# Lumina-Group/libzkp

Measured on AMD Instinct MI355X. Metric: proofs/sec (whole node) + ms/proof p50, 4096-proof mixed batch (range / equality / membership / improvement) per MI355X, higher is better.
Workload: dtype u32/u64 integer limbs (10x25.5-bit GF(2^255-19), BN254 Fq on 9x29-bit limbs in the MSM loops and 10x26-bit elsewhere, 8x32-bit Fr and scalars mod l, 2x64-bit f128)

## Files before the change

libzkp_amd/csrc/bn254_g.h:

```cpp
#pragma once
#include "bn254_fq.h"
#include "bn254_fq9.h"

namespace zkp {

struct fq2 { fq c0, c1; };

ZKP_HD inline fq f_add(const fq& a, const fq& b) { return fq_add(a, b); }
ZKP_HD inline fq f_sub(const fq& a, const fq& b) { return fq_sub(a, b); }
ZKP_HD inline fq f_mul(const fq& a, const fq& b) { return fq_mul(a, b); }
ZKP_HD inline fq f_sq(const fq& a) { return fq_sq(a); }
ZKP_HD inline fq f_neg(const fq& a) { return fq_neg(a); }
ZKP_HD inline fq f_dbl(const fq& a) { return fq_dbl(a); }
ZKP_HD inline bool f_is_zero(const fq& a) { return fq_is_zero(a); }
ZKP_HD inline fq f_select(bool c, const fq& a, const fq& b) { return fq_select(c, a, b); }
ZKP_HD inline void f_set_zero(fq& a) { a = fq_zero(); }
ZKP_HD inline void f_set_one(fq& a) { a = fq_one(); }
ZKP_HD inline fq f_inv(const fq& a) { return fq_inv(a); }

ZKP_HD inline fq2 f_add(const fq2& a, const fq2& b) { return fq2{fq_add(a.c0, b.c0), fq_add(a.c1, b.c1)}; }
ZKP_HD inline fq2 f_sub(const fq2& a, const fq2& b) { return fq2{fq_sub(a.c0, b.c0), fq_sub(a.c1, b.c1)}; }
ZKP_HD inline fq2 f_neg(const fq2& a) { return fq2{fq_neg(a.c0), fq_neg(a.c1)}; }
ZKP_HD inline fq2 f_dbl(const fq2& a) { return fq2{fq_dbl(a.c0), fq_dbl(a.c1)}; }
ZKP_HD inline fq2 f_mul(const fq2& a, const fq2& b) {
    const fq t0 = fq_mul(a.c0, b.c0), t1 = fq_mul(a.c1, b.c1);
    const fq t2 = fq_mul(fq_add_l(a.c0, a.c1), fq_add_l(b.c0, b.c1));
    return fq2{fq_reduce_weak(fq_sub_k4(t0, t1)), fq_reduce_weak(fq_sub_k8(t2, fq_add_l(t0, t1)))};
}
ZKP_HD inline fq2 f_sq(const fq2& a) {
    const fq t = fq_mul(a.c0, a.c1);
    return fq2{fq_reduce_weak(fq_mul(fq_add_l(a.c0, a.c1), fq_sub_k4(a.c0, a.c1))), fq_reduce_weak(fq_dbl_l(t))};
}
ZKP_HD inline bool f_is_zero(const fq2& a) { return fq_is_zero(a.c0) && fq_is_zero(a.c1); }
ZKP_HD inline fq2 f_select(bool c, const fq2& a, const fq2& b) { return fq2{fq_select(c, a.c0, b.c0), fq_select(c, a.c1, b.c1)}; }
ZKP_HD inline void f_set_zero(fq2& a) { a.c0 = fq_zero(); a.c1 = fq_zero(); }
ZKP_HD inline void f_set_one(fq2& a) { a.c0 = fq_one(); a.c1 = fq_zero(); }
ZKP_HD inline fq2 f_inv(const fq2& a) {
    const fq d = fq_inv(fq_add(fq_sq(a.c0), fq_sq(a.c1)));
    return fq2{fq_reduce_weak(fq_mul(a.c0, d)), fq_neg(fq_reduce_weak(fq_mul(a.c1, d)))};
}

template <class F> struct Aff { F x, y; };
template <class F> struct Jac { F X, Y, Z; };
using g1_aff = Aff<fq>; using g1_jac = Jac<fq>;
using g2_aff = Aff<fq2>; using g2_jac = Jac<fq2>;

template <class F> ZKP_HD inline Jac<F> jac_infinity() { Jac<F> r; f_set_one(r.X); f_set_one(r.Y); f_set_zero(r.Z); return r; }
template <class F> ZKP_HD inline Jac<F> jac_from_aff(const Aff<F>& p) { Jac<F> r; r.X = p.x; r.Y = p.y; f_set_one(r.Z); return r; }
template <class F> ZKP_HD inline bool jac_is_inf(const Jac<F>& p) { return f_is_zero(p.Z); }

template <class F> ZKP_HD inline Jac<F> jac_dbl(const Jac<F>& p) {
    const F A = f_sq(p.X), B = f_sq(p.Y), C = f_sq(B);
    const F D = f_dbl(f_sub(f_sub(f_sq(f_add(p.X, B)), A), C));
    const F E = f_add(f_dbl(A), A), Fq_ = f_sq(E);
    Jac<F> r;
    r.X = f_sub(Fq_, f_dbl(D));
    r.Y = f_sub(f_mul(E, f_sub(D, r.X)), f_dbl(f_dbl(f_dbl(C))));
    r.Z = f_dbl(f_mul(p.Y, p.Z));
    return r;
}

template <class F> ZKP_HD inline Jac<F> jac_madd(const Jac<F>& p, const Aff<F>& q) {
    if (jac_is_inf(p)) return jac_from_aff(q);
    const F Z1Z1 = f_sq(p.Z);
    const F U2 = f_mul(q.x, Z1Z1), S2 = f_mul(f_mul(q.y, p.Z), Z1Z1);
    const F H = f_sub(U2, p.X), rr = f_dbl(f_sub(S2, p.Y));
    if (f_is_zero(H)) return f_is_zero(rr) ? jac_dbl(p) : jac_infinity<F>();
    const F HH = f_sq(H), I = f_dbl(f_dbl(HH)), J = f_mul(H, I), V = f_mul(p.X, I);
    Jac<F> r;
    r.X = f_sub(f_sub(f_sq(rr), J), f_dbl(V));
    r.Y = f_sub(f_mul(rr, f_sub(V, r.X)), f_dbl(f_mul(p.Y, J)));
    r.Z = f_sub(f_sub(f_sq(f_add(p.Z, H)), Z1Z1), HH);
    return r;
}


ZKP_HD inline Jac<fq> g1_madd_lazy(const Jac<fq>& p, const Aff<fq>& q) {
    const fq Z1Z1 = fq_sq(p.Z);
    const fq U2 = fq_mul(q.x, Z1Z1), S2 = fq_mul(fq_mul(q.y, p.Z), Z1Z1);
    const fq H = fq_sub_k4(U2, p.X), sv = fq_sub_k4(S2, p.Y);
    const fq HH = fq_sq(H);
    const fq I = fq_dbl_l(fq_dbl_l(HH));
    const fq J = fq_mul(H, I), V = fq_mul(p.X, I);
    const fq ss = fq_sq(sv);
    Jac<fq> r;
    r.X = fq_reduce_weak(fq_sub_k8(fq_sub_k4(fq_dbl_l(fq_dbl_l(ss)), J), fq_dbl_l(V)));
    const fq t = fq_sub_k4(fq_mul(sv, fq_sub_k4(V, r.X)), fq_mul(p.Y, J));
    r.Y = fq_reduce_weak(fq_dbl_l(t));
    r.Z = fq_reduce_weak(fq_sub_k4(fq_sub_k4(fq_sq(fq_add_l(p.Z, H)), Z1Z1), HH));
    return r;
}

struct g1_xyzz { fq X, Y, ZZ, ZZZ; };
ZKP_HD inline g1_xyzz g1_mmadd_lazy(const g1_xyzz& p, const Aff<fq>& q) {
    const fq U2 = fq_mul(q.x, p.ZZ), S2 = fq_mul(q.y, p.ZZZ);
    const fq P = fq_sub_k4(U2, p.X), Rv = fq_sub_k4(S2, p.Y);
    const fq PP = fq_sq(P);
    const fq PPP = fq_mul(P, PP), Q = fq_mul(p.X, PP);
    const fq RR = fq_sq(Rv);
    g1_xyzz r;
    r.X = fq_reduce_weak(fq_sub_k8(fq_sub_k4(RR, PPP), fq_dbl_l(Q)));
    r.Y = fq_mul_add2(Rv, fq_sub_k4(Q, r.X), fq_sub_k4(fq_zero(), p.Y), PPP);
    r.ZZ = fq_mul(p.ZZ, PP);
    r.ZZZ = fq_mul(p.ZZZ, PPP);
    return r;
}
struct g1_xyzz9 { fq9 X, Y, ZZ, ZZZ; };
struct g1_aff9 { fq9 x, y; };
ZKP_HD inline g1_xyzz9 g1_mmadd9(const g1_xyzz9& p, const g1_aff9& q) {
    const fq9 U2 = fq9_mul(q.x, p.ZZ), S2 = fq9_mul(q.y, p.ZZZ);
    const fq9 P = fq9_sub_k<8>(U2, p.X), Rv = fq9_sub_k<4>(S2, p.Y);
    const fq9 PP = fq9_sq(P);
    const fq9 PPP = fq9_mul(P, PP), Q = fq9_mul(p.X, PP);
    const fq9 RR = fq9_sq(Rv);
    g1_xyzz9 r;
    r.X = fq9_sub2_k4(RR, PPP, Q);
    r.Y = fq9_mul_add2(Rv, fq9_sub_loose<8>(Q, r.X), fq9_neg_loose<4>(p.Y), PPP);
    r.ZZ = fq9_mul(p.ZZ, PP);
    r.ZZZ = fq9_mul(p.ZZZ, PPP);
    return r;
}
ZKP_HD inline g1_xyzz9 xyzz9_from_jac(const Jac<fq>& p) {
    const fq zz = fq_sq(p.Z);
    return g1_xyzz9{fq9_from_fq(p.X), fq9_from_fq(p.Y), fq9_from_fq(zz), fq9_from_fq(fq_mul(zz, p.Z))};
}
ZKP_HD inline Jac<fq> jac_from_xyzz9(const g1_xyzz9& p) { return Jac<fq>{fq9_to_fq(fq9_mul(p.X, p.ZZ)), fq9_to_fq(fq9_mul(p.Y, p.ZZZ)), fq9_to_fq(p.ZZ)}; }
ZKP_HD inline g1_xyzz xyzz_from_jac(const Jac<fq>& p) { const fq zz = fq_sq(p.Z); return g1_xyzz{p.X, p.Y, zz, fq_mul(zz, p.Z)}; }
ZKP_HD inline Jac<fq> jac_from_xyzz(const g1_xyzz& p) { return Jac<fq>{fq_reduce_weak(fq_mul(p.X, p.ZZ)), fq_reduce_weak(fq_mul(p.Y, p.ZZZ)), fq_reduce_weak(p.ZZ)}; }

struct fq2k { fq t0, t1, t2; };
struct fq2s { fq c0, m; };
ZKP_HD inline fq2k fq2_kara(const fq2& a, const fq2& b) { return fq2k{fq_mul(a.c0, b.c0), fq_mul(a.c1, b.c1), fq_mul(fq_add_l(a.c0, a.c1), fq_add_l(b.c0, b.c1))}; }
ZKP_HD inline fq2 fq2_join(const fq2k& k) { return fq2{fq_sub_k4(k.t0, k.t1), fq_sub_k8(k.t2, fq_add_l(k.t0, k.t1))}; }
ZKP_HD inline fq2s fq2_sq_l(const fq2& a) { return fq2s{fq_mul(fq_add_l(a.c0, a.c1), fq_sub_k4(a.c0, a.c1)), fq_mul(a.c0, a.c1)}; }
ZKP_HD inline Jac<fq2> g2_madd_lazy(const Jac<fq2>& p, const Aff<fq2>& q, bool negate) {
    const fq zero = fq_zero();
    const fq2 y2{fq_select(negate, fq_sub_k4(zero, q.y.c0), q.y.c0), fq_select(negate, fq_sub_k4(zero, q.y.c1), q.y.c1)};
    const fq2s zz = fq2_sq_l(p.Z);
    const fq2 Z1Z1{zz.c0, fq_dbl_l(zz.m)};
    const fq2 U2 = fq2_join(fq2_kara(q.x, Z1Z1));
    const fq2 S2 = fq2_join(fq2_kara(fq2_join(fq2_kara(y2, p.Z)), Z1Z1));
    const fq2 H{fq_reduce_weak(fq_sub_k4(U2.c0, p.X.c0)), fq_reduce_weak(fq_sub_k4(U2.c1, p.X.c1))};
    const fq2 sv{fq_reduce_weak(fq_sub_k4(S2.c0, p.Y.c0)), fq_reduce_weak(fq_sub_k4(S2.c1, p.Y.c1))};
    const fq2s hh = fq2_sq_l(H);
    const fq2 I{fq_dbl_l(fq_dbl_l(hh.c0)), fq_dbl_l(fq_dbl_l(fq_dbl_l(hh.m)))};
    const fq2k J = fq2_kara(H, I), V = fq2_kara(p.X, I);
    const fq2s ss = fq2_sq_l(sv);
    Jac<fq2> r;
    r.X.c0 = fq_reduce_weak(fq_sub_k16(fq_add_l(fq_dbl_l(fq_dbl_l(ss.c0)), fq_add_l(J.t1, fq_dbl_l(V.t1))), fq_add_l(J.t0, fq_dbl_l(V.t0))));
    r.X.c1 = fq_reduce_weak(fq_sub_k16(fq_add_l(fq_dbl_l(fq_dbl_l(fq_dbl_l(ss.m))), fq_add_l(fq_add_l(J.t0, J.t1), fq_dbl_l(fq_add_l(V.t0, V.t1)))),
                                       fq_add_l(J.t2, fq_dbl_l(V.t2))));
    const fq2 W{fq_sub_k8(V.t0, fq_add_l(V.t1, r.X.c0)), fq_sub_k16(V.t2, fq_add_l(fq_add_l(V.t0, V.t1), r.X.c1))};
    const fq2k P1 = fq2_kara(sv, W), P2 = fq2_kara(p.Y, fq2_join(J));
    r.Y.c0 = fq_reduce_weak(fq_dbl_l(fq_sub_k8(fq_add_l(P1.t0, P2.t1), fq_add_l(P1.t1, P2.t0))));
    r.Y.c1 = fq_reduce_weak(fq_dbl_l(fq_sub_k16(fq_add_l(P1.t2, fq_add_l(P2.t0, P2.t1)), fq_add_l(fq_add_l(P1.t0, P1.t1), P2.t2))));
    const fq2 zh{fq_add_l(p.Z.c0, H.c0), fq_add_l(p.Z.c1, H.c1)};
    const fq zq0 = fq_mul(fq_add_l(zh.c0, zh.c1), fq_sub_k8(zh.c0, zh.c1)), zqm = fq_mul(zh.c0, zh.c1);
    r.Z.c0 = fq_reduce_weak(fq_sub_k8(zq0, fq_add_l(zz.c0, hh.c0)));
    r.Z.c1 = fq_reduce_weak(fq_dbl_l(fq_sub_k8(zqm, fq_add_l(zz.m, hh.m))));
    return r;
}

struct fq2_9 { fq9 c0, c1; };
struct g2_xyzz9 { fq2_9 X, Y, ZZ, ZZZ; };
struct g2_aff9 { fq2_9 x, y; };
ZKP_HD inline fq2_9 fq2_9_mul(const fq2_9& a, const fq2_9& b, const fq9& nb1) {
    return fq2_9{fq9_mul_add2(a.c0, b.c0, a.c1, nb1), fq9_mul_add2(a.c0, b.c1, a.c1, b.c0)};
}
ZKP_HD inline fq2_9 fq2_9_sq(const fq2_9& a, const fq9& na1) { return fq2_9{fq9_mul_add2(a.c0, a.c0, a.c1, na1), fq9_mul(fq9_dbl_l(a.c0), a.c1)}; }
ZKP_HD inline g2_xyzz9 g2_mmadd9(const g2_xyzz9& p, const g2_aff9& q, bool negate) {
    const fq9 nZZ1 = fq9_neg_k<4>(p.ZZ.c1), nZZZ1 = fq9_neg_k<4>(p.ZZZ.c1);
    const fq2_9 U2 = fq2_9_mul(q.x, p.ZZ, nZZ1), S2 = fq2_9_mul(q.y, p.ZZZ, nZZZ1);
    const fq2_9 P{fq9_sub_k<16>(U2.c0, p.X.c0), fq9_sub_k<16>(U2.c1, p.X.c1)};
    const fq2_9 Rv{fq9_sgn_sub_k<8>(negate, S2.c0, p.Y.c0), fq9_sgn_sub_k<8>(negate, S2.c1, p.Y.c1)};
    const fq2_9 PP = fq2_9_sq(P, fq9_neg_k<32>(P.c1));
    const fq9 nPP1 = fq9_neg_k<8>(PP.c1);
    const fq2_9 PPP = fq2_9_mul(P, PP, nPP1), Q = fq2_9_mul(p.X, PP, nPP1);
    const fq9 nR1 = fq9_neg_k<16>(Rv.c1);
    const fq2_9 RR = fq2_9_sq(Rv, nR1);
    g2_xyzz9 r;
    r.X = fq2_9{fq9_sub2_k<8>(RR.c0, PPP.c0, Q.c0), fq9_sub2_k<8>(RR.c1, PPP.c1, Q.c1)};
    const fq2_9 W{fq9_sub_k<16>(Q.c0, r.X.c0), fq9_sub_k<16>(Q.c1, r.X.c1)};
    const fq9 nY0 = fq9_neg_k<4>(p.Y.c0), nY1 = fq9_neg_k<4>(p.Y.c1);
    r.Y = fq2_9{fq9_mul_add4(Rv.c0, W.c0, nR1, W.c1, nY0, PPP.c0, p.Y.c1, PPP.c1),
                fq9_mul_add4(Rv.c0, W.c1, Rv.c1, W.c0, nY0, PPP.c1, nY1, PPP.c0)};
    r.ZZ = fq2_9_mul(PP, p.ZZ, nZZ1);
    r.ZZZ = fq2_9_mul(PPP, p.ZZZ, nZZZ1);
    return r;
}
ZKP_HD inline fq2_9 fq2_9_from_fq2(const fq2& a) { return fq2_9{fq9_from_fq(a.c0), fq9_from_fq(a.c1)}; }
ZKP_HD inline fq2 fq2_9_to_fq2(const fq2_9& a) { return fq2{fq9_to_fq(a.c0), fq9_to_fq(a.c1)}; }
ZKP_HD inline g2_xyzz9 g2_xyzz9_from_jac(const Jac<fq2>& p) {
    const fq2 zz = f_sq(p.Z);
    return g2_xyzz9{fq2_9_from_fq2(p.X), fq2_9_from_fq2(p.Y), fq2_9_from_fq2(zz), fq2_9_from_fq2(f_mul(zz, p.Z))};
}
ZKP_HD inline Jac<fq2> jac_from_g2_xyzz9(const g2_xyzz9& p) {
    return Jac<fq2>{fq2_9_to_fq2(fq2_9_mul(p.X, p.ZZ, fq9_neg_k<4>(p.ZZ.c1))), fq2_9_to_fq2(fq2_9_mul(p.Y, p.ZZZ, fq9_neg_k<4>(p.ZZZ.c1))), fq2_9_to_fq2(p.ZZ)};
}

template <class F> ZKP_HD inline Jac<F> jac_add(const Jac<F>& p, const Jac<F>& q) {
    if (jac_is_inf(p)) return q;
    if (jac_is_inf(q)) return p;
    const F Z1Z1 = f_sq(p.Z), Z2Z2 = f_sq(q.Z);
    const F U1 = f_mul(p.X, Z2Z2), U2 = f_mul(q.X, Z1Z1);
    const F S1 = f_mul(f_mul(p.Y, q.Z), Z2Z2), S2 = f_mul(f_mul(q.Y, p.Z), Z1Z1);
    const F H = f_sub(U2, U1), rr = f_dbl(f_sub(S2, S1));
    if (f_is_zero(H)) return f_is_zero(rr) ? jac_dbl(p) : jac_infinity<F>();
    const F I = f_sq(f_dbl(H)), J = f_mul(H, I), V = f_mul(U1, I);
    Jac<F> r;
    r.X = f_sub(f_sub(f_sq(rr), J), f_dbl(V));
    r.Y = f_sub(f_mul(rr, f_sub(V, r.X)), f_dbl(f_mul(S1, J)));
    r.Z = f_mul(f_sub(f_sub(f_sq(f_add(p.Z, q.Z)), Z1Z1), Z2Z2), H);
    return r;
}
template <class F> ZKP_HD inline Aff<F> aff_neg(const Aff<F>& p) { return Aff<F>{p.x, f_neg(p.y)}; }
template <class F> ZKP_HD inline Jac<F> jac_neg(const Jac<F>& p) { return Jac<F>{p.X, f_neg(p.Y), p.Z}; }

template <class F> ZKP_HD inline Jac<F> jac_mul_raw(const Jac<F>& p, const uint32_t k[8]) {
    Jac<F> tbl[16];
    tbl[0] = jac_infinity<F>(); tbl[1] = p;
    for (int i = 2; i < 16; i++) tbl[i] = jac_add(tbl[i - 1], p);
    Jac<F> acc = jac_infinity<F>();
    for (int nib = 63; nib >= 0; nib--) {
        acc = jac_dbl(jac_dbl(jac_dbl(jac_dbl(acc))));
        const uint32_t d = (k[nib >> 3] >> ((nib & 7) * 4)) & 15u;
        if (d) acc = jac_add(acc, tbl[d]);
    }
    return acc;
}

template <int NA, int NB, int NO> ZKP_HD inline void mp_mul_lo(uint32_t* out, const uint32_t* a, const uint32_t* b) {
    uint64_t acc = 0, hi = 0;
    ZKP_UNROLL for (int k = 0; k < NO; k++) {
        ZKP_UNROLL for (int i = 0; i < NA; i++) {
            const int j = k - i;
            if (j < 0 || j >= NB) continue;
            const uint64_t t = (uint64_t)a[i] * b[j];
            acc += (uint32_t)t; hi += t >> 32;
        }
        out[k] = (uint32_t)acc;
        acc = (acc >> 32) + (uint32_t)hi; hi >>= 32;
    }
}
struct glv_half { uint32_t mag[4]; bool neg; };
ZKP_HD inline glv_half glv_from_160(const uint32_t w[5]) {
    glv_half h; h.neg = (w[4] >> 31) != 0;
    uint32_t c = h.neg ? 1u : 0u;
    ZKP_UNROLL for (int i = 0; i < 4; i++) { const uint32_t x = h.neg ? ~w[i] : w[i]; const uint32_t t = x + c; c = (c && t == 0) ? 1u : 0u; h.mag[i] = t; }
    return h;
}
ZKP_HD inline void fr_glv_split(const uint32_t k[8], glv_half& h1, glv_half& h2) {
    const uint32_t G1[3] = {0xc7e0b3d7u, 0xd91d232eu, 0x00000002u}, G2[5] = {0x391eb18du, 0x7a7bd9d4u, 0xa773d2cfu, 0x4ccef014u, 0x00000002u};
    const uint32_t A1[2] = {0x94d213e3u, 0x89d32568u}, A2[4] = {0x1221250bu, 0x0be4e154u, 0xeeb859fdu, 0x6f4d8248u};
    const uint32_t NB1[4] = {0x7d4f1128u, 0x8211bbebu, 0xeeb859fcu, 0x6f4d8248u}, B2[2] = {0x94d213e3u, 0x89d32568u};
    uint32_t t1[11], t2[13];
    mp_mul_lo<8, 3, 11>(t1, k, G1); mp_mul_lo<8, 5, 13>(t2, k, G2);
    const uint32_t* c1 = t1 + 8;
    const uint32_t* c2 = t2 + 8;
    uint32_t p11[5], p22[5], p12[5], p21[5];
    mp_mul_lo<3, 2, 5>(p11, c1, A1); mp_mul_lo<5, 4, 5>(p22, c2, A2); mp_mul_lo<3, 4, 5>(p12, c1, NB1); mp_mul_lo<5, 2, 5>(p21, c2, B2);
    uint32_t k1[5], k2[5]; int64_t b1 = 0, b2 = 0;
    ZKP_UNROLL for (int i = 0; i < 5; i++) {
        b1 += (int64_t)k[i] - (int64_t)p11[i] - (int64_t)p22[i]; k1[i] = (uint32_t)b1; b1 >>= 32;
        b2 += (int64_t)p12[i] - (int64_t)p21[i]; k2[i] = (uint32_t)b2; b2 >>= 32;
    }
    h1 = glv_from_160(k1); h2 = glv_from_160(k2);
}
ZKP_HD inline fq fq_glv_beta() {
    const uint32_t w[8] = {0x77fffffeu, 0x57634731u, 0xacdb5c4fu, 0xd4f263f1u, 0xa0d48bacu, 0x59e26bceu, 0x00000000u, 0x00000000u};
    return fq_from_raw(w);
}
template <class F> ZKP_HD inline Jac<F> jac_mul_u128_signed(const Jac<F>& p, const uint32_t mag[4], bool neg) {
    Jac<F> tbl[8];
    tbl[0] = p; tbl[1] = jac_dbl(p);
    for (int i = 2; i < 8; i++) tbl[i] = jac_add(tbl[i - 1], p);
    int dig[33]; int carry = 0;
    for (int i = 0; i < 32; i++) {
        int v = (int)((mag[i >> 3] >> ((i & 7) * 4)) & 15u) + carry;
        carry = v > 8 ? 1 : 0; if (carry) v -= 16;
        dig[i] = v;
    }
    dig[32] = carry;
    Jac<F> acc = jac_infinity<F>();
    for (int i = 32; i >= 0; i--) {
        if (i != 32) acc = jac_dbl(jac_dbl(jac_dbl(jac_dbl(acc))));
        const int d = dig[i];
        if (d > 0) acc = jac_add(acc, tbl[d - 1]);
        else if (d < 0) acc = jac_add(acc, jac_neg(tbl[-d - 1]));
    }
    return neg ? jac_neg(acc) : acc;
}

template <class F> ZKP_HD inline bool jac_to_aff(Aff<F>& out, const Jac<F>& p) {
    if (jac_is_inf(p)) return false;
    const F zi = f_inv(p.Z), zi2 = f_sq(zi);
    out.x = f_mul(p.X, zi2); out.y = f_mul(f_mul(p.Y, zi2), zi);
    return true;
}

ZKP_HD inline bool fq_raw_gt_half(const uint32_t w[8]) {
    const uint32_t half[8] = {0x6c3e7ea3u, 0x9e10460bu, 0xb438e546u, 0xcbc0b548u, 0x40c0ac2eu, 0xdc2822dbu, 0x7098d014u, 0x18322739u};
    for (int i = 7; i >= 0; i--) { if (w[i] > half[i]) return true; if (w[i] < half[i]) return false; }
    return false;
}
ZKP_HD inline void g1_serialize(uint32_t out[16], const g1_jac& p) {
    g1_aff a;
    if (!jac_to_aff(a, p)) { for (int i = 0; i < 16; i++) out[i] = 0; out[15] = 0x40000000u; return; }
    fq_to_raw(out, a.x); fq_to_raw(out + 8, a.y);
    if (fq_raw_gt_half(out + 8)) out[15] |= 0x80000000u;
}
ZKP_HD inline void g2_serialize(uint32_t out[32], const g2_jac& p) {
    g2_aff a;
    if (!jac_to_aff(a, p)) { for (int i = 0; i < 32; i++) out[i] = 0; out[31] = 0x40000000u; return; }
    fq_to_raw(out, a.x.c0); fq_to_raw(out + 8, a.x.c1); fq_to_raw(out + 16, a.y.c0); fq_to_raw(out + 24, a.y.c1);
    uint32_t nz = 0; for (int i = 0; i < 8; i++) nz |= out[24 + i];
    const bool larger = nz ? fq_raw_gt_half(out + 24) : fq_raw_gt_half(out + 16);
    if (larger) out[31] |= 0x80000000u;
}

}
```

libzkp_amd/csrc/bp_layout.h:

```cpp
#pragma once
#include <vector>
#include <utility>
#include <cstring>
#include "bp_steps.h"

namespace zkp {

inline void host_sponge(uint8_t* out, size_t outlen, const uint8_t* in, size_t inlen, size_t rate, uint8_t suffix) {
    uint64_t a[25]; memset(a, 0, sizeof a);
    uint8_t* b = reinterpret_cast<uint8_t*>(a);
    size_t pos = 0;
    for (size_t i = 0; i < inlen; i++) { b[pos++] ^= in[i]; if (pos == rate) { keccak_f1600(a); pos = 0; } }
    b[pos] ^= suffix; b[rate - 1] ^= 0x80;
    keccak_f1600(a);
    size_t done = 0;
    while (done < outlen) {
        size_t n = outlen - done < rate ? outlen - done : rate;
        memcpy(out + done, b, n); done += n;
        if (done < outlen) keccak_f1600(a);
    }
}

inline ge host_from_uniform(const uint8_t b[64]) { uint32_t w[16]; memcpy(w, b, 64); return ge_from_uniform_words(w); }

inline ge host_basepoint() {
    const uint32_t yw[8] = {0x66666658u, 0x66666666u, 0x66666666u, 0x66666666u, 0x66666666u, 0x66666666u, 0x66666666u, 0x66666666u};
    const uint32_t xw[8] = {0x8f25d51au, 0xc9562d60u, 0x9525a7b2u, 0x692cc760u, 0xfdd6dc5cu, 0xc0a4e231u, 0xcd6e53feu, 0x216936d3u};
    ge p; p.X = fe_fromwords(xw); p.Y = fe_fromwords(yw); p.Z = fe_one(); p.T = fe_mul(p.X, p.Y);
    return p;
}

inline void host_generators(ge out[NBASE]) {
    out[BASE_B] = host_basepoint();
    uint32_t enc[8]; ge_ristretto_encode(enc, out[BASE_B]);
    uint8_t h[64]; host_sponge(h, 64, reinterpret_cast<uint8_t*>(enc), 32, 72, 0x06);
    out[BASE_BB] = host_from_uniform(h);
    for (int which = 0; which < 2; which++) {
        uint8_t in[20]; memcpy(in, "GeneratorsChain", 15);
        in[15] = which ? 'H' : 'G'; in[16] = in[17] = in[18] = in[19] = 0;
        std::vector<uint8_t> stream(64 * BP_N);
        host_sponge(stream.data(), stream.size(), in, 20, 136, 0x1F);
        for (uint32_t i = 0; i < BP_N; i++) out[(which ? BASE_H : BASE_G) + i] = host_from_uniform(stream.data() + 64 * i);
    }
}

inline fe host_fe_invert(const fe& z) {
    fe t = fe_pow22523(z);
    t = fe_sq(fe_sq(fe_sq(t)));
    return fe_mul(t, fe_mul(fe_sq(z), z));
}

inline void host_build_table_for_base(uint32_t* dst, const ge& base) {
    std::vector<ge> pts(NWIN * NENT);
    ge pw = base;
    for (uint32_t w = 0; w < NWIN; w++) {
        ge acc = pw;
        for (uint32_t e = 0; e < NENT; e++) { pts[w * NENT + e] = acc; acc = ge_add(acc, pw); }
        for (uint32_t k = 0; k < WBITS; k++) pw = ge_dbl(pw);
    }
    const size_t n = pts.size();
    std::vector<fe> pre(n);
    fe run = fe_one();
    for (size_t i = 0; i < n; i++) { pre[i] = run; run = fe_mul(run, pts[i].Z); }
    fe inv = host_fe_invert(run);
    const fe d2 = fe_const_d2();
    for (size_t i = n; i-- > 0;) {
        const fe zi = fe_mul(inv, pre[i]);
        inv = fe_mul(inv, pts[i].Z);
        const fe x = fe_mul(pts[i].X, zi), y = fe_mul(pts[i].Y, zi);
        uint32_t w8[8];
        fe_towords(w8, fe_add(y, x)); const fe ypx = fe_fromwords(w8);
        fe_towords(w8, fe_sub(y, x)); const fe ymx = fe_fromwords(w8);
        fe_towords(w8, fe_mul(fe_mul(x, y), d2)); const fe xy2d = fe_fromwords(w8);
        uint32_t* q = dst + i * NIELS_W;
        for (int k = 0; k < 10; k++) { q[k] = ypx.v[k]; q[10 + k] = ymx.v[k]; q[20 + k] = xy2d.v[k]; }
    }
}

struct MsmLayout {
    std::vector<uint16_t> slot_base, chunk_begin, chunk_win0, chunk_nwin, target_chunk_begin;
    std::vector<uint8_t> slot_nwin;
    uint32_t nslots() const { return (uint32_t)slot_base.size(); }
    uint32_t nchunks() const { return (uint32_t)chunk_begin.size(); }
    uint32_t ntargets() const { return (uint32_t)target_chunk_begin.size() - 1; }
};
using SlotList = std::vector<std::pair<uint16_t, uint8_t>>;

inline MsmLayout make_layout(const std::vector<SlotList>& targets, uint32_t win_budget) {
    MsmLayout L;
    L.target_chunk_begin.push_back(0);
    for (const auto& t : targets) {
        uint32_t used = 0; bool open = false;
        for (const auto& s : t) {
            if (open && used + s.second > win_budget) { L.chunk_nwin.push_back((uint16_t)used); used = 0; open = false; }
            if (!open) { L.chunk_begin.push_back((uint16_t)L.slot_base.size()); L.chunk_win0.push_back(0); open = true; }
            L.slot_base.push_back(s.first); L.slot_nwin.push_back(s.second); used += s.second;
        }
        if (open) L.chunk_nwin.push_back((uint16_t)used);
        L.target_chunk_begin.push_back((uint16_t)L.chunk_begin.size());
    }
    return L;
}
inline MsmLayout make_layout_even(const std::vector<SlotList>& targets, uint32_t total_chunks) {
    MsmLayout L;
    uint64_t W = 0; for (const auto& t : targets) for (const auto& s : t) W += s.second;
    L.target_chunk_begin.push_back(0);
    for (const auto& t : targets) {
        uint32_t wt = 0; for (const auto& s : t) wt += s.second;
        uint32_t k = (uint32_t)((uint64_t)total_chunks * wt / (W ? W : 1));
        if (k < 1) k = 1;
        if (k > wt && wt) k = wt;
        const uint32_t slot0 = (uint32_t)L.slot_base.size();
        for (const auto& s : t) { L.slot_base.push_back(s.first); L.slot_nwin.push_back(s.second); }
        uint32_t slot = slot0, win = 0, done = 0;
        for (uint32_t c = 0; c < k; c++) {
            const uint32_t upto = (uint32_t)((uint64_t)wt * (c + 1) / k), n = upto - done;
            if (n == 0) continue;
            L.chunk_begin.push_back((uint16_t)slot); L.chunk_win0.push_back((uint16_t)win); L.chunk_nwin.push_back((uint16_t)n);
            uint32_t left = n;
            while (left) { const uint32_t room = L.slot_nwin[slot] - win, step = left < room ? left : room; win += step; left -= step; if (win == L.slot_nwin[slot]) { slot++; win = 0; } }
            done = upto;
        }
        L.target_chunk_begin.push_back((uint16_t)L.chunk_begin.size());
    }
    return L;
}
struct GatherShape { uint32_t nent, slot_ent, uneven, digw; };
inline bool make_gather_steps(const MsmLayout& L, const uint16_t* slot_scalar, const GatherShape& g, std::vector<uint32_t>& steps, std::vector<uint32_t>& chunk_step0) {
    steps.clear(); chunk_step0.clear();
    for (uint32_t c = 0; c < L.nchunks(); c++) {
        chunk_step0.push_back((uint32_t)(steps.size() / 2));
        uint32_t s = L.chunk_begin[c], w = L.chunk_win0[c];
        for (uint32_t left = L.chunk_nwin[c]; left > 0; left--) {
            const uint64_t first = (uint64_t)L.slot_base[s] * g.slot_ent + (uint64_t)(w + (g.uneven && w == 17u ? 1u : 0u)) * g.nent;
            const uint64_t word = (uint64_t)(slot_scalar ? slot_scalar[s] : s) * g.digw + w / 2;
            if (first + g.nent > 0xffffffffull || word > 0x7fffffffull) return false;
            steps.push_back((uint32_t)first); steps.push_back((uint32_t)(word << 1) | (w & 1u));
            if (++w == L.slot_nwin[s]) { s++; w = 0; }
        }
    }
    chunk_step0.push_back((uint32_t)(steps.size() / 2));
    for (int pad = 0; pad < 8; pad++) { steps.push_back(0); steps.push_back(0); }
    return true;
}

inline std::vector<SlotList> targets_phase1(uint32_t n = BP_N, uint8_t nw = NWIN, uint8_t nw64 = NWIN_U64) {
    const uint8_t NWIN = nw, NWIN_U64 = nw64;
    SlotList v = {{BASE_B, NWIN_U64}, {BASE_BB, NWIN}}, a = {{BASE_BB, NWIN}}, s = {{BASE_BB, NWIN}};
    for (uint32_t i = 0; i < n; i++) a.push_back({(uint16_t)(BASE_G + i), 1});
    for (uint32_t i = 0; i < n; i++) a.push_back({(uint16_t)(BASE_H + i), 1});
    for (uint32_t i = 0; i < n; i++) s.push_back({(uint16_t)(BASE_G + i), NWIN});
    for (uint32_t i = 0; i < n; i++) s.push_back({(uint16_t)(BASE_H + i), NWIN});
    return {v, a, s};
}
inline std::vector<SlotList> targets_phase2(uint8_t nw = NWIN) { SlotList t = {{BASE_B, nw}, {BASE_BB, nw}}; return {t, t}; }
inline std::vector<SlotList> targets_round(uint32_t r, uint32_t n = BP_N, uint8_t nw = NWIN) {
    const uint8_t NWIN = nw;
    uint32_t lg = 0; while ((1u << lg) < n) lg++;
    const uint32_t p = lg - 1 - r, k = 1u << p, half = n / 2;
    auto idx = [&](uint32_t rank, uint32_t bit) { return ((rank >> p) << (p + 1)) | (bit << p) | (rank & (k - 1)); };
    SlotList l = {{BASE_B, NWIN}}, rr = {{BASE_B, NWIN}};
    for (uint32_t q = 0; q < half; q++) l.push_back({(uint16_t)(BASE_G + idx(q, 1)), NWIN});
    for (uint32_t q = 0; q < half; q++) l.push_back({(uint16_t)(BASE_H + idx(q, 0)), NWIN});
    for (uint32_t q = 0; q < half; q++) rr.push_back({(uint16_t)(BASE_G + idx(q, 0)), NWIN});
    for (uint32_t q = 0; q < half; q++) rr.push_back({(uint16_t)(BASE_H + idx(q, 1)), NWIN});
    return {l, rr};
}
inline std::vector<SlotList> targets_ctask(uint8_t nw = NWIN, uint8_t nw64 = NWIN_U64) { return {SlotList{{BASE_B, nw64}, {BASE_BB, nw}}}; }
inline std::vector<SlotList> targets_verify(uint8_t nw = NWIN) {
    const uint8_t NWIN = nw;
    SlotList t = {{BASE_B, NWIN}, {BASE_BB, NWIN}};
    for (uint32_t i = 0; i < BP_N; i++) t.push_back({(uint16_t)(BASE_G + i), NWIN});
    for (uint32_t i = 0; i < BP_N; i++) t.push_back({(uint16_t)(BASE_H + i), NWIN});
    return {t};
}
inline MsmLayout layout_phase1(uint32_t budget, uint32_t n = BP_N) { return make_layout(targets_phase1(n), budget); }
inline MsmLayout layout_phase2(uint32_t budget) { return make_layout(targets_phase2(), budget); }
inline MsmLayout layout_round(uint32_t r, uint32_t budget, uint32_t n = BP_N) { return make_layout(targets_round(r, n), budget); }
inline MsmLayout layout_ctask(uint32_t budget) { return make_layout(targets_ctask(), budget); }

}
```

libzkp_amd/csrc/bp_steps.h:

```cpp
#pragma once
#include "fe25519.h"
#include "sc25519.h"
#include "ge25519.h"
#include "keccak.h"

namespace zkp {

constexpr uint32_t BP_N = 64;
constexpr uint32_t BASE_B = 0, BASE_BB = 1, BASE_G = 2, BASE_H = 66, NBASE = 130;
constexpr uint32_t WBITS = 10, NWIN = 26, NENT = 512, DIGW = 13, NWIN_U64 = 7, NIELS_W = 30, SUBTAB_W = NENT * NIELS_W;
constexpr uint32_t TAPE_SLOTS = 132;
constexpr uint32_t P1_V = 0, P1_A = 2, P1_NSLOTS = 260;
constexpr uint32_t P2_NSLOTS = 4;
constexpr uint32_t PR_NSLOTS = 130;
ZKP_HD constexpr uint32_t p1_s(uint32_t n) { return 3 + 2 * n; }
ZKP_HD constexpr uint32_t tape_slots(uint32_t n) { return 2 * n + 4; }
ZKP_HD constexpr uint32_t rp_bytes(uint32_t lg) { return 32 * (9 + 2 * lg); }
constexpr uint32_t GE_W = 40;
enum { SC_Y = 0, SC_Z, SC_X, SC_W, SC_U, SC_UINV, SC_T0, SC_T1, SC_T2, SC_NUM };
enum { KIND_RANGE_MIN = 0, KIND_RANGE_MAX, KIND_THRESHOLD, KIND_CONSISTENCY, KIND_BULLETPROOF, KIND_NUM };

struct BpView {
    uint32_t M;
    uint32_t n, lg;
    uint32_t wbits = 0;
    const uint64_t* v;
    const uint32_t* seed_ix;
    const uint32_t* proof_ix;
    const int32_t* bl_plus;
    const int32_t* bl_minus;
    const uint8_t* kind;
    const uint32_t* seeds;
    const uint64_t* proof_off;
    const uint64_t* commit_off;
    uint8_t* out;
    uint32_t* tape;
    uint32_t* gamma;
    uint32_t* d1;
    uint32_t* d2;
    uint32_t* dr;
    uint32_t* yinvpow;
    uint32_t* ypq;
    uint32_t* r0;
    uint32_t* r1;
    uint32_t* pp;
    uint32_t* ab;
    uint32_t* gh;
    uint32_t* scal;
    uint32_t* tstate;
    uint32_t* enc;
};

ZKP_HD inline sc ld_sc(const uint32_t* p, uint32_t idx, uint32_t row, uint32_t rows) {
    sc r; const uint32_t* q = p + (size_t)idx * 8 * rows + row;
    ZKP_UNROLL for (int k = 0; k < 8; k++) r.v[k] = q[(size_t)k * rows];
    return r;
}
ZKP_HD inline void st_sc(uint32_t* p, uint32_t idx, uint32_t row, uint32_t rows, const sc& s) {
    uint32_t* q = p + (size_t)idx * 8 * rows + row;
    ZKP_UNROLL for (int k = 0; k < 8; k++) q[(size_t)k * rows] = s.v[k];
}
ZKP_HD inline void st_digits_raw(uint32_t* d, uint32_t slot, uint32_t row, uint32_t rows, const sc& raw, uint32_t wbits = 0) {
    uint32_t* q = d + (size_t)slot * DIGW * rows + row;
    if (wbits == 16) {
        uint32_t pk[8]; sc_recode_signed65536(pk, raw);
        ZKP_UNROLL for (uint32_t k = 0; k < 8; k++) q[(size_t)k * rows] = pk[k];
        return;
    }
    if (wbits > 10) { sc_recode_signed_rt(q, rows, raw, wbits, sc_signed_ndigits(wbits, 254)); return; }
    uint32_t pk[DIGW]; sc_recode_signed1024(pk, raw);
    ZKP_UNROLL for (uint32_t k = 0; k < DIGW; k++) q[(size_t)k * rows] = pk[k];
}
ZKP_HD inline void st_digits(uint32_t* d, uint32_t slot, uint32_t row, uint32_t rows, const sc& mont, uint32_t wbits = 0) { st_digits_raw(d, slot, row, rows, sc_to_raw(mont), wbits); }
ZKP_HD inline int32_t ld_digit(const uint32_t* d, uint32_t srow, uint32_t w, uint32_t row, uint32_t rows) {
    return (int32_t)(int16_t)(d[((size_t)srow * DIGW + (w >> 1)) * rows + row] >> (16 * (w & 1u)));
}
ZKP_HD inline void put_bytes(uint8_t* dst, const uint32_t* w, int nwords) {
    for (int i = 0; i < nwords; i++) { dst[4 * i] = (uint8_t)w[i]; dst[4 * i + 1] = (uint8_t)(w[i] >> 8); dst[4 * i + 2] = (uint8_t)(w[i] >> 16); dst[4 * i + 3] = (uint8_t)(w[i] >> 24); }
}
ZKP_HD inline void ld_seed(uint32_t s[8], const BpView& V, uint32_t job) {
    const uint32_t* p = V.seeds + (size_t)V.seed_ix[job] * 8;
    ZKP_UNROLL for (int k = 0; k < 8; k++) s[k] = p[k];
}
ZKP_HD inline sc tape_blinding(const uint32_t seed[8], uint32_t i) {
    uint32_t w[16]; tape_draw64(w, seed, 0xFFFFFFFFu, i);
    sc raw; ZKP_UNROLL for (int k = 0; k < 8; k++) raw.v[k] = w[k];
    return sc_from_raw256(raw);
}

ZKP_HD inline void step_tape(const BpView& V, uint32_t slot, uint32_t job) {
    const uint32_t M = V.M, n = V.n, P1_S = p1_s(V.n);
    uint32_t seed[8]; ld_seed(seed, V, job);
    if (slot < tape_slots(n)) {
        uint32_t w[16]; tape_draw64(w, seed, V.proof_ix[job], slot);
        const sc x = sc_from_wide(w);
        st_sc(V.tape, slot, job, M, x);
        if (slot == 0) st_digits(V.d1, P1_A + 0, job, M, x, V.wbits);
        else if (slot == 1) st_digits(V.d1, P1_S + 0, job, M, x, V.wbits);
        else if (slot < 2 + n) st_digits(V.d1, P1_S + 1 + (slot - 2), job, M, x, V.wbits);
        else if (slot < 2 + 2 * n) st_digits(V.d1, P1_S + 1 + n + (slot - 2 - n), job, M, x, V.wbits);
        else if (slot == 2 + 2 * n) st_digits(V.d2, 1, job, M, x, V.wbits);
        else st_digits(V.d2, 3, job, M, x, V.wbits);
    } else {
        sc g = sc_zero();
        if (V.bl_plus[job] >= 0) g = tape_blinding(seed, (uint32_t)V.bl_plus[job]);
        if (V.bl_minus[job] >= 0) g = sc_sub(g, tape_blinding(seed, (uint32_t)V.bl_minus[job]));
        st_sc(V.gamma, 0, job, M, g);
        st_digits(V.d1, P1_V + 1, job, M, g, V.wbits);
        const uint64_t v = V.v[job];
        st_digits_raw(V.d1, P1_V + 0, job, M, sc_words((uint32_t)v, (uint32_t)(v >> 32), 0, 0, 0, 0, 0, 0), V.wbits);
        for (uint32_t i = 0; i < n; i++) {
            const uint32_t bit = (uint32_t)(v >> i) & 1u;
            V.d1[(size_t)(P1_A + 1 + i) * DIGW * M + job] = bit;
            V.d1[(size_t)(P1_A + 1 + n + i) * DIGW * M + job] = bit ? 0u : 0xFFFFu;
        }
    }
}

ZKP_HD inline ge_niels ld_niels(const uint32_t* p) {
    ge_niels n;
    ZKP_UNROLL for (int k = 0; k < 10; k++) { n.ypx.v[k] = p[k]; n.ymx.v[k] = p[10 + k]; n.xy2d.v[k] = p[20 + k]; }
    return n;
}
ZKP_HD inline ge msm_accumulate_digit(const ge& acc, int32_t d, const uint32_t* subtab) {
    const uint32_t mag = (uint32_t)(d < 0 ? -d : d);
    ge_niels n = ld_niels(subtab + (size_t)(mag - 1) * NIELS_W);
    n = ge_niels_select(d < 0, ge_niels_neg(n), n);
    return ge_madd(acc, n);
}
ZKP_HD inline void st_ge(uint32_t* p, uint32_t idx, uint32_t row, uint32_t rows, const ge& g) {
    uint32_t* q = p + (size_t)idx * GE_W * rows + row;
    ZKP_UNROLL for (int k = 0; k < 10; k++) {
        q[(size_t)k * rows] = g.X.v[k]; q[(size_t)(10 + k) * rows] = g.Y.v[k];
        q[(size_t)(20 + k) * rows] = g.Z.v[k]; q[(size_t)(30 + k) * rows] = g.T.v[k];
    }
}
ZKP_HD inline ge ld_ge(const uint32_t* p, uint32_t idx, uint32_t row, uint32_t rows) {
    ge g; const uint32_t* q = p + (size_t)idx * GE_W * rows + row;
    ZKP_UNROLL for (int k = 0; k < 10; k++) {
        g.X.v[k] = q[(size_t)k * rows]; g.Y.v[k] = q[(size_t)(10 + k) * rows];
        g.Z.v[k] = q[(size_t)(20 + k) * rows]; g.T.v[k] = q[(size_t)(30 + k) * rows];
    }
    return g;
}
struct MsmView {
    uint32_t rows, nslots, nchunks;
    const uint32_t* table;
    const uint32_t* digits;
    const uint16_t* slot_base;
    const uint16_t* slot_scalar;
    const uint8_t* slot_nwin;
    const uint16_t* chunk_begin;
    const uint16_t* chunk_win0;
    const uint16_t* chunk_nwin;
    uint32_t* partial;
    const uint32_t* acc_init;
    uint32_t nwin = 0, nent = 0, digw = 0;
    uint32_t slot_ent = 0, uneven = 0;
    const uint32_t* steps = nullptr; const uint32_t* chunk_step0 = nullptr;
};
ZKP_HD inline void msm_chunk_ref(const MsmView& m, uint32_t chunk, uint32_t row) {
    ge acc = ge_identity();
    uint32_t s = m.chunk_begin[chunk], w = m.chunk_win0[chunk];
    for (uint32_t left = m.chunk_nwin[chunk]; left > 0; left--) {
        const uint32_t srow = m.slot_scalar ? m.slot_scalar[s] : s;
        const int32_t d = ld_digit(m.digits, srow, w, row, m.rows);
        if (d != 0) acc = msm_accumulate_digit(acc, d, m.table + ((size_t)m.slot_base[s] * NWIN + w) * SUBTAB_W);
        if (++w == m.slot_nwin[s]) { s++; w = 0; }
    }
    st_ge(m.partial, chunk, row, m.rows, acc);
}
struct ReduceView {
    uint32_t rows, ntargets;
    const uint32_t* partial;
    const uint16_t* target_chunk_begin;
    uint32_t* enc;
    const uint64_t* out_off;
    uint8_t* out;
    const uint32_t* corr;
    const uint16_t* target_chunk_end = nullptr;
};
ZKP_HD inline uint32_t reduce_chunk_end(const ReduceView& r, uint32_t target) { return r.target_chunk_end ? r.target_chunk_end[target] : r.target_chunk_begin[target + 1]; }
ZKP_HD inline void reduce_encode_thread(const ReduceView& r, uint32_t target, uint32_t row) {
    const uint32_t c0 = r.target_chunk_begin[target], c1 = reduce_chunk_end(r, target);
    ge acc = ld_ge(r.partial, c0, row, r.rows);
    for (uint32_t c = c0 + 1; c < c1; c++) acc = ge_add(acc, ld_ge(r.partial, c, row, r.rows));
    sc e; ge_ristretto_encode(e.v, acc);
    st_sc(r.enc, target, row, r.rows, e);
    if (r.out_off != nullptr && target == 0) put_bytes(r.out + r.out_off[row], e.v, 8);
}

ZKP_HD inline void strobe_save(const BpView& V, uint32_t job, const Strobe& s) {
    for (int i = 0; i < 50; i++) V.tstate[(size_t)i * V.M + job] = s.base[i * s.stride];
    V.tstate[(size_t)50 * V.M + job] = s.pos; V.tstate[(size_t)51 * V.M + job] = s.pos_begin;
}
ZKP_HD inline void strobe_load(const BpView& V, uint32_t job, Strobe& s) {
    for (int i = 0; i < 50; i++) s.base[i * s.stride] = V.tstate[(size_t)i * V.M + job];
    s.pos = V.tstate[(size_t)50 * V.M + job]; s.pos_begin = V.tstate[(size_t)51 * V.M + job];
}
ZKP_HD inline sc merlin_challenge_scalar(Strobe& s, const char* label, uint32_t label_len) {
    uint32_t w[16]; merlin_challenge_words(s, label, label_len, w, 16);
    return sc_from_wide(w);
}
ZKP_HD inline void merlin_append_scalar(Strobe& s, const char* label, uint32_t label_len, const sc& raw) { merlin_append_words(s, label, label_len, raw.v, 8); }

ZKP_HD inline void step_transcript1(const BpView& V, uint32_t job, Strobe& s) {
    const uint32_t M = V.M;
    switch (V.kind[job]) {
        case KIND_RANGE_MIN: merlin_init(s, "libzkp_range_min", 16); break;
        case KIND_RANGE_MAX: merlin_init(s, "libzkp_range_max", 16); break;
        case KIND_THRESHOLD: merlin_init(s, "libzkp_threshold", 16); break;
        case KIND_CONSISTENCY: merlin_init(s, "libzkp_consistency", 18); break;
        default: merlin_init(s, "libzkp_bulletproof", 18); break;
    }
    merlin_append_bytes(s, "dom-sep", 7, "rangeproof v1", 13);
    merlin_append_u64(s, "n", 1, V.n);
    merlin_append_u64(s, "m", 1, 1);
    const sc Ve = ld_sc(V.enc, 0, job, M), Ae = ld_sc(V.enc, 1, job, M), Se = ld_sc(V.enc, 2, job, M);
    merlin_append_words(s, "V", 1, Ve.v, 8);
    merlin_append_words(s, "A", 1, Ae.v, 8);
    merlin_append_words(s, "S", 1, Se.v, 8);
    const sc y = merlin_challenge_scalar(s, "y", 1);
    const sc z = merlin_challenge_scalar(s, "z", 1);
    strobe_save(V, job, s);
    st_sc(V.scal, SC_Y, job, M, y);
    st_sc(V.scal, SC_Z, job, M, z);
    const sc yinv = sc_invert(y);
    for (uint32_t h = 0; h < 2; h++) {
        const sc base = h ? yinv : y;
        sc p = sc_one();
        for (uint32_t b = 0; b < 8; b++) { st_sc(V.ypq, 16 * h + b, job, M, p); p = sc_mul(p, base); }
        sc q = sc_one();
        for (uint32_t a = 0; a < 8; a++) { st_sc(V.ypq, 16 * h + 8 + a, job, M, q); q = sc_mul(q, p); }
    }
    uint8_t* pr = V.out + V.proof_off[job];
    put_bytes(pr, Ae.v, 8); put_bytes(pr + 32, Se.v, 8);
    put_bytes(V.out + V.commit_off[job], Ve.v, 8);
}

ZKP_HD inline void step_poly(const BpView& V, uint32_t i, uint32_t job) {
    const uint32_t M = V.M;
    const sc yi = sc_mul(ld_sc(V.ypq, 8 + (i >> 3), job, M), ld_sc(V.ypq, i & 7u, job, M));
    st_sc(V.yinvpow, i, job, M, sc_mul(ld_sc(V.ypq, 24 + (i >> 3), job, M), ld_sc(V.ypq, 16 + (i & 7u), job, M)));
    const sc z = ld_sc(V.scal, SC_Z, job, M);
    const sc zz = sc_mul(z, z);
    const uint32_t bit = (uint32_t)(V.v[job] >> i) & 1u;
    const sc one = sc_one();
    const sc l0 = bit ? sc_sub(one, z) : sc_neg(z);
    const sc arz = bit ? z : sc_sub(z, one);
    const sc two_i = sc_from_u64(1ull << i);
    const sc r0 = sc_add(sc_mul(yi, arz), sc_mul(zz, two_i));
    const sc l1 = ld_sc(V.tape, 2 + i, job, M);
    const sc r1 = sc_mul(yi, ld_sc(V.tape, 2 + V.n + i, job, M));
    st_sc(V.r0, i, job, M, r0); st_sc(V.r1, i, job, M, r1);
    st_sc(V.pp, i, job, M, sc_mul(l0, r0));
    st_sc(V.pp, 64 + i, job, M, sc_mul(sc_add(l0, l1), sc_add(r0, r1)));
    st_sc(V.pp, 128 + i, job, M, sc_mul(l1, r1));
}
struct ScTriple { sc a, b, c; };
ZKP_HD inline ScTriple triple_add(const ScTriple& x, const ScTriple& y) { return ScTriple{sc_add(x.a, y.a), sc_add(x.b, y.b), sc_add(x.c, y.c)}; }
ZKP_HD inline ScTriple step_poly_sum_part(const BpView& V, uint32_t part, uint32_t job) {
    const uint32_t M = V.M;
    ScTriple t{sc_zero(), sc_zero(), sc_zero()};
    for (uint32_t i = part; i < V.n; i += 8) {
        t.a = sc_add(t.a, ld_sc(V.pp, i, job, M));
        t.b = sc_add(t.b, ld_sc(V.pp, 64 + i, job, M));
        t.c = sc_add(t.c, ld_sc(V.pp, 128 + i, job, M));
    }
    return t;
}
ZKP_HD inline void step_poly_sum_finish(const BpView& V, uint32_t job, const ScTriple& t) {
    const uint32_t M = V.M;
    const sc t0 = t.a, t2 = t.c, t1 = sc_sub(sc_sub(t.b, t0), t2);
    st_sc(V.scal, SC_T0, job, M, t0); st_sc(V.scal, SC_T1, job, M, t1); st_sc(V.scal, SC_T2, job, M, t2);
    st_digits(V.d2, 0, job, M, t1, V.wbits);
    st_digits(V.d2, 2, job, M, t2, V.wbits);
}
ZKP_HD inline void step_poly_sum(const BpView& V, uint32_t job) {
    ScTriple t = step_poly_sum_part(V, 0, job);
    for (uint32_t p = 1; p < 8; p++) t = triple_add(t, step_poly_sum_part(V, p, job));
    step_poly_sum_finish(V, job, t);
}
ZKP_HD inline void step_transcript2(const BpView& V, uint32_t job, Strobe& s) {
    const uint32_t M = V.M;
    strobe_load(V, job, s);
    const sc T1e = ld_sc(V.enc, 0, job, M), T2e = ld_sc(V.enc, 1, job, M);
    merlin_append_words(s, "T_1", 3, T1e.v, 8);
    merlin_append_words(s, "T_2", 3, T2e.v, 8);
    const sc x = merlin_challenge_scalar(s, "x", 1);
    const sc xx = sc_mul(x, x);
    const sc z = ld_sc(V.scal, SC_Z, job, M), zz = sc_mul(z, z);
    const sc t0 = ld_sc(V.scal, SC_T0, job, M), t1 = ld_sc(V.scal, SC_T1, job, M), t2 = ld_sc(V.scal, SC_T2, job, M);
    const sc t_x = sc_add(sc_add(t0, sc_mul(t1, x)), sc_mul(t2, xx));
    const sc t1_bl = ld_sc(V.tape, 2 + 2 * V.n, job, M), t2_bl = ld_sc(V.tape, 3 + 2 * V.n, job, M);
    const sc t_x_bl = sc_add(sc_add(sc_mul(zz, ld_sc(V.gamma, 0, job, M)), sc_mul(t1_bl, x)), sc_mul(t2_bl, xx));
    const sc e_bl = sc_add(ld_sc(V.tape, 0, job, M), sc_mul(ld_sc(V.tape, 1, job, M), x));
    const sc r_tx = sc_to_raw(t_x), r_txb = sc_to_raw(t_x_bl), r_eb = sc_to_raw(e_bl);
    merlin_append_scalar(s, "t_x", 3, r_tx);
    merlin_append_scalar(s, "t_x_blinding", 12, r_txb);
    merlin_append_scalar(s, "e_blinding", 10, r_eb);
    const sc w = merlin_challenge_scalar(s, "w", 1);
    merlin_append_bytes(s, "dom-sep", 7, "ipp v1", 6);
    merlin_append_u64(s, "n", 1, V.n);
    strobe_save(V, job, s);
    st_sc(V.scal, SC_X, job, M, x); st_sc(V.scal, SC_W, job, M, w);
    uint8_t* pr = V.out + V.proof_off[job];
    put_bytes(pr + 64, T1e.v, 8); put_bytes(pr + 96, T2e.v, 8);
    put_bytes(pr + 128, r_tx.v, 8); put_bytes(pr + 160, r_txb.v, 8); put_bytes(pr + 192, r_eb.v, 8);
}
ZKP_HD inline void step_lr_init(const BpView& V, uint32_t i, uint32_t job) {
    const uint32_t M = V.M;
    const sc z = ld_sc(V.scal, SC_Z, job, M), x = ld_sc(V.scal, SC_X, job, M);
    const uint32_t bit = (uint32_t)(V.v[job] >> i) & 1u;
    const sc l0 = bit ? sc_sub(sc_one(), z) : sc_neg(z);
    const sc a = sc_add(l0, sc_mul(ld_sc(V.tape, 2 + i, job, M), x));
    const sc b = sc_add(ld_sc(V.r0, i, job, M), sc_mul(ld_sc(V.r1, i, job, M), x));
    st_sc(V.ab, i, job, M, a); st_sc(V.ab, 64 + i, job, M, b);
}

ZKP_HD inline void step_round_prep(const BpView& V, uint32_t r, uint32_t i, uint32_t job) {
    const uint32_t M = V.M, p = V.lg - 1 - r, k = 1u << p, half = V.n >> 1;
    const uint32_t* abp = V.ab + (size_t)(r & 1) * (2 * 64 * 8) * M;
    uint32_t* abn = V.ab + (size_t)((r + 1) & 1) * (2 * 64 * 8) * M;
    sc u = sc_one(), uinv = sc_one();
    if (r > 0) { u = ld_sc(V.scal, SC_U, job, M); uinv = ld_sc(V.scal, SC_UINV, job, M); }
    auto cur_a = [&](uint32_t x) -> sc {
        if (r == 0) return ld_sc(abp, x, job, M);
        return sc_add(sc_mul(ld_sc(abp, x, job, M), u), sc_mul(ld_sc(abp, x + 2 * k, job, M), uinv));
    };
    auto cur_b = [&](uint32_t x) -> sc {
        if (r == 0) return ld_sc(abp, 64 + x, job, M);
        return sc_add(sc_mul(ld_sc(abp, 64 + x, job, M), uinv), sc_mul(ld_sc(abp, 64 + x + 2 * k, job, M), u));
    };
    sc g, h;
    if (r == 0) { g = sc_one(); h = ld_sc(V.yinvpow, i, job, M); }
    else {
        const bool hi = (i >> (p + 1)) & 1u;
        g = sc_mul(ld_sc(V.gh, i, job, M), hi ? u : uinv);
        h = sc_mul(ld_sc(V.gh, 64 + i, job, M), hi ? uinv : u);
    }
    st_sc(V.gh, i, job, M, g); st_sc(V.gh, 64 + i, job, M, h);
    const uint32_t x = (i & (2 * k - 1)) ^ k;
    const sc ax = cur_a(x), bx = cur_b(x);
    if (i < 2 * k) { st_sc(abn, x, job, M, ax); st_sc(abn, 64 + x, job, M, bx); }
    const uint32_t bit = (i >> p) & 1u, rank = ((i >> (p + 1)) << p) | (i & (k - 1));
    st_digits(V.dr, bit ? 1 + rank : V.n + 2 + rank, job, M, sc_mul(ax, g), V.wbits);
    st_digits(V.dr, bit ? V.n + 2 + half + rank : 1 + half + rank, job, M, sc_mul(bx, h), V.wbits);
    if (i < k) {
        const sc ai = cur_a(i), bi = cur_b(i);
        st_sc(V.pp, i, job, M, sc_mul(ai, bx));
        st_sc(V.pp, 32 + i, job, M, sc_mul(ax, bi));
    }
}
ZKP_HD inline void step_round_sum(const BpView& V, uint32_t r, uint32_t job) {
    const uint32_t M = V.M, k = (V.n >> 1) >> r;
    sc cL = sc_zero(), cR = sc_zero();
    for (uint32_t j = 0; j < k; j++) { cL = sc_add(cL, ld_sc(V.pp, j, job, M)); cR = sc_add(cR, ld_sc(V.pp, 32 + j, job, M)); }
    const sc w = ld_sc(V.scal, SC_W, job, M);
    st_digits(V.dr, 0, job, M, sc_mul(cL, w), V.wbits);
    st_digits(V.dr, V.n + 1, job, M, sc_mul(cR, w), V.wbits);
}
ZKP_HD inline void step_transcript_round(const BpView& V, uint32_t r, uint32_t job, Strobe& s) {
    const uint32_t M = V.M;
    strobe_load(V, job, s);
    const sc Le = ld_sc(V.enc, 0, job, M), Re = ld_sc(V.enc, 1, job, M);
    merlin_append_words(s, "L", 1, Le.v, 8);
    merlin_append_words(s, "R", 1, Re.v, 8);
    const sc u = merlin_challenge_scalar(s, "u", 1);
    const sc uinv = sc_invert(u);
    uint8_t* pr = V.out + V.proof_off[job];
    put_bytes(pr + 224 + 64 * r, Le.v, 8); put_bytes(pr + 256 + 64 * r, Re.v, 8);
    if (r + 1 < V.lg) {
        strobe_save(V, job, s);
        st_sc(V.scal, SC_U, job, M, u); st_sc(V.scal, SC_UINV, job, M, uinv);
    } else {
        const uint32_t* abp = V.ab + (size_t)(V.lg & 1u) * (2 * 64 * 8) * M;
        const sc a = sc_add(sc_mul(ld_sc(abp, 0, job, M), u), sc_mul(ld_sc(abp, 1, job, M), uinv));
        const sc b = sc_add(sc_mul(ld_sc(abp, 64, job, M), uinv), sc_mul(ld_sc(abp, 65, job, M), u));
        const sc ra = sc_to_raw(a), rb = sc_to_raw(b);
        put_bytes(pr + 224 + 64 * V.lg, ra.v, 8); put_bytes(pr + 256 + 64 * V.lg, rb.v, 8);
    }
}

struct CtView {
    uint32_t C;
    const uint64_t* v; const uint32_t* seed_ix; const uint32_t* bl_ix; const uint32_t* seeds;
    uint32_t* digits;
    uint32_t wbits = 0;
};
ZKP_HD inline void step_ctask(const CtView& T, uint32_t c) {
    uint32_t seed[8]; const uint32_t* p = T.seeds + (size_t)T.seed_ix[c] * 8;
    ZKP_UNROLL for (int k = 0; k < 8; k++) seed[k] = p[k];
    const uint64_t v = T.v[c];
    st_digits_raw(T.digits, 0, c, T.C, sc_words((uint32_t)v, (uint32_t)(v >> 32), 0, 0, 0, 0, 0, 0), T.wbits);
    st_digits(T.digits, 1, c, T.C, tape_blinding(seed, T.bl_ix[c]), T.wbits);
}

struct JobBuf {
    uint64_t* v; uint32_t* seed_ix; uint32_t* proof_ix; int32_t* bl_plus; int32_t* bl_minus; uint8_t* kind;
    uint64_t* proof_off; uint64_t* commit_off;
    uint64_t* ct_v; uint32_t* ct_seed_ix; uint32_t* ct_bl_ix; uint64_t* ct_off;
};
constexpr uint32_t RANGE_PROOF_BYTES = 1478, RP_BYTES = 672;
enum { ZKP_ST_OK = 0, ZKP_ST_INVALID_INPUT = 1 };
ZKP_HD inline void put_le(uint8_t* p, uint64_t x, int n) { for (int i = 0; i < n; i++) p[i] = (uint8_t)(x >> (8 * i)); }
ZKP_HD constexpr uint32_t range_body_bytes(uint32_t lg) { return 20 + 2 * (4 + rp_bytes(lg)) + 64; }
ZKP_HD constexpr uint32_t range_envelope_bytes(uint32_t lg) { return 10 + range_body_bytes(lg) + 32; }
ZKP_HD inline void step_build_range(const JobBuf& J, uint32_t op, const uint64_t* value, const uint64_t* mn, const uint64_t* mx, uint32_t lg,
                                    uint8_t* out, uint64_t stride, uint32_t* out_len, int32_t* status) {
    const uint64_t val = value[op], lo = mn[op], hi = mx[op];
    const uint64_t max_diff = lg >= 6 ? ~0ull : (1ull << (1u << lg)) - 1;
    const bool ok = lo <= hi && val >= lo && val <= hi
                    && val - lo <= max_diff && hi - val <= max_diff;
    const uint32_t RP_BYTES = rp_bytes(lg), body = range_body_bytes(lg);
    status[op] = ok ? ZKP_ST_OK : ZKP_ST_INVALID_INPUT;
    out_len[op] = ok ? range_envelope_bytes(lg) : 0;
    const uint64_t base = (uint64_t)op * stride;
    for (uint32_t j = 0; j < 2; j++) {
        const uint32_t job = 2 * op + j;
        J.v[job] = ok ? (j == 0 ? val - lo : hi - val) : 0;
        J.seed_ix[job] = op; J.proof_ix[job] = j;
        J.bl_plus[job] = j == 0 ? 0 : -1; J.bl_minus[job] = j == 0 ? -1 : 0;
        J.kind[job] = (uint8_t)(j == 0 ? KIND_RANGE_MIN : KIND_RANGE_MAX);
        J.proof_off[job] = base + 34 + (uint64_t)j * (4 + RP_BYTES);
        J.commit_off[job] = base + 10 + 20 + 2 * (4 + RP_BYTES) + 32 * j;
    }
    J.ct_v[op] = ok ? val : 0; J.ct_seed_ix[op] = op; J.ct_bl_ix[op] = 0;
    J.ct_off[op] = base + 10 + body;
    uint8_t* o = out + base;
    o[0] = 2; o[1] = 1; put_le(o + 2, body, 4); put_le(o + 6, 32, 4);
    put_le(o + 10, lo, 8); put_le(o + 18, hi, 8); put_le(o + 26, 1u << lg, 4);
    put_le(o + 30, RP_BYTES, 4); put_le(o + 34 + RP_BYTES, RP_BYTES, 4);
}

}
```

libzkp_amd/csrc/g16_impl.inc:

```

namespace {

struct G16Key {
    bool loaded = false;
    uint32_t n_inst = 0, n_wit = 0, nv = 0, n_rows = 0, m = 0, logm = 0;
    G16Circuit C{};
    std::vector<void*> allocs;
    uint32_t *table_g1 = nullptr, *table_g2 = nullptr;
    G16Radix rx = g16_radix(G16_WBITS_DEFAULT);
    int shared_tables = -1;
    uint64_t table_bytes = 0;
    struct Chunking { DevLayout lay; const uint32_t* corr = nullptr; const uint16_t* scal = nullptr; };
    std::vector<SlotList> targets_g1, targets_g2;
    std::vector<uint16_t> hscal_g1, hscal_g2;
    std::map<uint64_t, Chunking> lays_g1, lays_g2;
    uint64_t win_g1 = 0, win_g2 = 0;
    const uint32_t *init_g1 = nullptr, *init_g2 = nullptr;
    G16Vk vk{}; bool vk_ready = false;
    uint64_t vk_table_bytes = 0;
    bool verifier_only() const { return vk_ready && !loaded; }
    const uint32_t *vm_kconst = nullptr, *vm_lines = nullptr;
};
struct G16Run {
    void* buf = nullptr; size_t cap = 0; hipStream_t side = nullptr, side2 = nullptr; hipEvent_t ev[4] = {nullptr, nullptr, nullptr, nullptr};
    hipEvent_t last = nullptr; bool used = false;
};
struct G16State {
    G16Key key[2];
    uint32_t* mimc_dev = nullptr;
    G16Run run[2][2];
    bool attr_set = false;
    G16VmTables vm;
};
G16State& g16s() {
    if (!dev().g16) dev().g16 = new G16State();
    return *dev().g16;
}

template <class Tv> int dev_upload(G16Key& K, Tv** dst, const std::vector<typename std::remove_const<Tv>::type>& src) {
    typename std::remove_const<Tv>::type* p = nullptr;
    HIP_TRY(hipMalloc(&p, src.size() * sizeof(src[0]) + 16));
    if (!src.empty()) HIP_TRY(hipMemcpy(p, src.data(), src.size() * sizeof(src[0]), hipMemcpyHostToDevice));
    K.allocs.push_back(p); *dst = p;
    return 0;
}

int upload_circuit(G16Key& K, const HostR1CS& cs) {
    const HostCircuitTables T = build_circuit_tables(cs);
    K.n_inst = T.n_inst; K.n_wit = T.n_wit; K.nv = T.nv; K.n_rows = T.n_rows; K.m = T.m; K.logm = T.logm;
    G16Circuit& C = K.C;
    C.n_rows = T.n_rows; C.m = T.m; C.logm = T.logm;
    int rc;
    if ((rc = dev_upload(K, &C.a_ptr, T.ptr[0])) || (rc = dev_upload(K, &C.a_col, T.col[0])) || (rc = dev_upload(K, &C.a_coef, T.coef[0]))) return rc;
    if ((rc = dev_upload(K, &C.b_ptr, T.ptr[1])) || (rc = dev_upload(K, &C.b_col, T.col[1])) || (rc = dev_upload(K, &C.b_coef, T.coef[1]))) return rc;
    if ((rc = dev_upload(K, &C.c_ptr, T.ptr[2])) || (rc = dev_upload(K, &C.c_col, T.col[2])) || (rc = dev_upload(K, &C.c_coef, T.coef[2]))) return rc;
    if ((rc = dev_upload(K, &C.tw, T.tw)) || (rc = dev_upload(K, &C.tw_inv, T.tw_inv)) || (rc = dev_upload(K, &C.coset, T.coset)) ||
        (rc = dev_upload(K, &C.coset_inv, T.coset_inv)) || (rc = dev_upload(K, &C.zinv, T.zinv))) return rc;
    return 0;
}


g2_aff host_g2_generator() {
    static const char* dec[4] = {"10857046999023057135944570762232829481370756359578518086990519993285655852781",
                                 "11559732032986387107991004021392285783925812861821192530917403151452391805634",
                                 "8495653923123431417604973247489272438418190587263600148770280649306958101930",
                                 "4082367875863433681332203403145435568316851327593401208105741076214120093531"};
    fq c[4];
    for (int k = 0; k < 4; k++) {
        fq acc = fq_zero(); const fq ten = fq_from_u64(10);
        for (const char* q = dec[k]; *q; q++) acc = fq_add(fq_mul(acc, ten), fq_from_u64((uint64_t)(*q - '0')));
        c[k] = acc;
    }
    return g2_aff{fq2{c[0], c[1]}, fq2{c[2], c[3]}};
}
g1_aff host_g1_generator() { return g1_aff{fq_from_u64(1), fq_from_u64(2)}; }
struct MsmOffsets { g1_jac o1; g2_jac o2; };
const MsmOffsets& msm_offsets() {
    static const MsmOffsets off = [] {
        uint8_t h[32]; const char* tag = "libzkp-amd msm offset"; sha256_host(h, (const uint8_t*)tag, strlen(tag));
        uint32_t k[8]; memcpy(k, h, 32); k[7] &= 0x0fffffffu;
        return MsmOffsets{jac_mul_raw(jac_from_aff(host_g1_generator()), k), jac_mul_raw(jac_from_aff(host_g2_generator()), k)};
    }();
    return off;
}
template <class J> void append_words(std::vector<uint32_t>& v, const J& p) { const uint32_t* w = reinterpret_cast<const uint32_t*>(&p); for (size_t i = 0; i < sizeof(J) / 4; i++) v.push_back(w[i]); }
template <class J> J host_neg_multiple(const J& o, uint32_t k) {
    J acc = o; for (uint32_t i = 1; i < k; i++) acc = jac_add(acc, o);
    return jac_neg(acc);
}
void append_offset(std::vector<uint32_t>& v, bool g2, uint32_t k) {
    const MsmOffsets& o = msm_offsets();
    if (!g2) append_words(v, k ? host_neg_multiple(o.o1, k) : o.o1); else append_words(v, k ? host_neg_multiple(o.o2, k) : o.o2);
}
int upload_offset_point(G16Key& K, bool g2, const uint32_t** d_init) { std::vector<uint32_t> init; append_offset(init, g2, 0); return dev_upload(K, d_init, init); }
uint32_t choose_chunks(uint64_t windows, uint32_t ntargets, uint32_t rows, uint32_t resident, uint32_t tb) {
    const uint32_t groups = (rows + tb - 1) / tb;
    uint32_t hi = (uint32_t)(windows / 8); if (hi > 2048) hi = 2048; if (hi < ntargets) hi = ntargets;
    uint32_t best = ntargets; double best_cost = 1e300;
    for (uint32_t c = ntargets; c <= hi; c++) {
        const double rounds = std::ceil((double)c * groups / resident);
        const double cost = rounds * (std::ceil((double)windows / c) + 2.5) + 0.25 * c / 8.0;
        if (cost < best_cost) { best_cost = cost; best = c; }
    }
    return best;
}
int get_chunking(G16Key& K, bool g2, int part, uint32_t rows, const G16Key::Chunking** out) {
    const uint32_t resident = (uint32_t)dev().num_cu * g16_msm_blocks_per_cu(g2);
    if (part == G16_PART_ALL && !g2) return fail(ZKP_HIP_E_ARGUMENT, "G16_PART_ALL is the G2 launch");
    const std::vector<SlotList> targets = g16_part_targets(g2 ? K.targets_g2 : K.targets_g1, part);
    uint32_t c = choose_chunks(g16_windows(targets), (uint32_t)targets.size(), rows, resident, g16_msm_rows_per_block(g2));
    if (g_budget_request >= 10000) c = g_budget_request - 10000;
    auto& cache = g2 ? K.lays_g2 : K.lays_g1;
    const uint64_t key = (uint64_t)part << 32 | c;
    auto it = cache.find(key);
    if (it == cache.end()) {
        const G16Chunks P = g16_plan_chunks(targets, g2 ? K.hscal_g2 : K.hscal_g1, part, c);
        G16Key::Chunking ch; int rc;
        const GatherShape shape{K.rx.nent, K.rx.slot_ent, K.rx.uneven ? 1u : 0u, K.rx.digw};
        if ((rc = upload_layout(ch.lay, P.L, &shape, P.scal.data()))) return rc;
        std::vector<uint32_t> corr;
        for (uint32_t k : P.offsets) append_offset(corr, g2, k);
        if ((rc = dev_upload(K, &ch.corr, corr))) return rc;
        if ((rc = dev_upload(K, &ch.scal, P.scal))) return rc;
        it = cache.emplace(key, ch).first;
    }
    *out = &it->second;
    return 0;
}


uint64_t key_table_bytes(size_t n1, size_t n2, uint32_t wbits, bool uneven = false) {
    const G16Radix rx = g16_radix(wbits, uneven);
    return ((uint64_t)n1 * g16_table_entry_words(false, true) + (uint64_t)n2 * g16_table_entry_words(true, true)) * 4ull * rx.slot_ent;
}
int choose_radix(size_t n1, size_t n2, uint32_t* wbits_out, bool* uneven_out) {
    *uneven_out = false;
    const int forced = env_int("ZKP_HIP_G16_WBITS", 0);
    if (forced) {
        if (forced < (int)G16_WBITS_MIN || forced > (int)G16_WBITS_MAX) return fail(ZKP_HIP_E_ARGUMENT, "ZKP_HIP_G16_WBITS must be 8..15");
        *wbits_out = (uint32_t)forced; *uneven_out = forced == 14 && env_int("ZKP_HIP_G16_UNEVEN", 1) != 0; return 0;
    }
    size_t free_b = 0, total_b = 0;
    HIP_TRY(hipMemGetInfo(&free_b, &total_b));
    const int budget_mb = env_int("ZKP_HIP_G16_TABLE_BUDGET_MB", 0);
    const uint64_t reserve = 8ull << 30;
    const uint64_t fits = free_b > reserve ? (uint64_t)((free_b - reserve) * 0.45) : 0;
    uint64_t budget = budget_mb > 0 ? (uint64_t)budget_mb << 20 : fits;
    uint32_t first = G16_WBITS_KNEE;
    if (budget_mb > 0) {
        first = G16_WBITS_DEFAULT;
        if (G16_WBITS_DEFAULT == 14 && env_int("ZKP_HIP_G16_UNEVEN", 1) != 0 && key_table_bytes(n1, n2, 14, true) <= budget) { *wbits_out = 14; *uneven_out = true; return 0; }
    }
    for (uint32_t w = first; w >= G16_WBITS_MIN; w--)
        if (key_table_bytes(n1, n2, w) <= budget) { *wbits_out = w; return 0; }
    char msg[256];
    snprintf(msg, sizeof msg, "not enough device memory for the proving key's window tables: %llu MB at the smallest radix (2^%u), budget %llu MB (%llu MB free)",
             (unsigned long long)(key_table_bytes(n1, n2, G16_WBITS_MIN) >> 20), G16_WBITS_MIN, (unsigned long long)(budget >> 20), (unsigned long long)(free_b >> 20));
    return fail(ZKP_HIP_E_RUNTIME, msg);
}
struct SharedTables { int hip_dev, kind; uint8_t digest[32]; uint32_t wbits; bool share_ab; uint32_t *g1, *g2; int refs; };
struct TableRegistry { std::mutex mu; std::vector<SharedTables> v; std::map<int, std::mutex> build_mu; };
TableRegistry& table_registry() { static TableRegistry* r = new TableRegistry(); return *r; }
std::mutex& table_build_mutex(int hip_dev) { TableRegistry& R = table_registry(); std::lock_guard<std::mutex> lk(R.mu); return R.build_mu[hip_dev]; }
bool acquire_tables(G16Key& K, const SharedTables& want, bool any_radix) {
    TableRegistry& R = table_registry();
    std::lock_guard<std::mutex> lk(R.mu);
    for (size_t i = 0; i < R.v.size(); i++) {
        SharedTables& e = R.v[i];
        if (e.refs <= 0 || e.hip_dev != want.hip_dev || e.kind != want.kind || e.share_ab != want.share_ab || memcmp(e.digest, want.digest, 32) || (!any_radix && e.wbits != want.wbits)) continue;
        e.refs++; K.shared_tables = (int)i; K.table_g1 = e.g1; K.table_g2 = e.g2; K.rx = g16_radix(e.wbits & 0xffu, (e.wbits >> 8) != 0);
        return true;
    }
    return false;
}
void register_tables(G16Key& K, SharedTables e) {
    TableRegistry& R = table_registry();
    std::lock_guard<std::mutex> lk(R.mu);
    e.refs = 1; R.v.push_back(e);
    K.shared_tables = (int)R.v.size() - 1; K.table_g1 = e.g1; K.table_g2 = e.g2;
}
template <uint32_t AW, class Pt>
int build_tables(G16Key& K, const std::vector<Pt>& bases, uint32_t** table, bool msm_form, const G16Radix& rx, bool owned = true) {
    std::vector<uint32_t> flat; flat.reserve(bases.size() * AW);
    for (auto& b : bases) { const uint32_t* w = reinterpret_cast<const uint32_t*>(&b); for (uint32_t k = 0; k < AW; k++) flat.push_back(w[k]); }
    uint32_t* d_bases = nullptr; int rc;
    if ((rc = dev_upload(K, &d_bases, flat))) return rc;
    const size_t words = bases.size() * (size_t)rx.slot_ent * g16_table_entry_words(AW == 40, msm_form);
    uint32_t* tab = nullptr;
    if (hipMalloc(&tab, words * 4 + 64) != hipSuccess) {
        (void)hipGetLastError();
        char msg[200]; snprintf(msg, sizeof msg, "out of device memory allocating %llu MB of key tables (radix 2^%u)", (unsigned long long)((words * 4) >> 20), rx.wbits);
        return fail(ZKP_HIP_E_RUNTIME, msg);
    }
    if (owned) K.allocs.push_back(tab);
    g16_launch_build_table(AW == 40, d_bases, (uint32_t)bases.size(), tab, dev().stream, msm_form, rx);
    HIP_TRY(hipGetLastError());
    HIP_TRY(hipStreamSynchronize(dev().stream));
    *table = tab;
    return 0;
}

void release_key(G16Key& K) {
    (void)hipDeviceSynchronize();
    if (K.shared_tables >= 0) {
        TableRegistry& R = table_registry();
        std::lock_guard<std::mutex> lk(R.mu);
        SharedTables& e = R.v[(size_t)K.shared_tables];
        if (--e.refs == 0) { (void)hipFree(e.g1); (void)hipFree(e.g2); e.g1 = e.g2 = nullptr; }
    }
    for (void* p : K.allocs) (void)hipFree(p);
    for (auto& e : K.lays_g1) free_layout(e.second.lay);
    for (auto& e : K.lays_g2) free_layout(e.second.lay);
    K = G16Key();
}
int load_key_body(int kind, const uint8_t* pk, uint64_t len);
int no_proving_key(const G16Key& K) {
    return fail(ZKP_HIP_E_ARGUMENT, K.verifier_only() ? "only a verifying key is loaded for this circuit: proving needs the proving key (zkp_hip_groth16_load_key)"
                                                      : "no proving key loaded for this circuit (zkp_hip_groth16_load_key)");
}
int load_key_locked(int kind, const uint8_t* pk, uint64_t len) {
    if (kind != G16_EQUALITY && kind != G16_MEMBERSHIP) return fail(ZKP_HIP_E_ARGUMENT, "unknown circuit kind");
    G16Key& K = g16s().key[kind];
    if (K.loaded || K.shared_tables >= 0 || !K.allocs.empty()) release_key(K);
    int rc;
    try { rc = load_key_body(kind, pk, len); }
    catch (...) { release_key(K); throw; }
    if (rc) { const std::string keep = t_err; release_key(K); t_err = keep; }
    return rc;
}
int install_verifying_key(G16Key& K, const G16VkBlob& B) {
    int rc;
    K.vk_ready = false;
    std::vector<g1_aff> ic_pts; for (auto& e : B.abc) ic_pts.push_back(e.p);
    ic_pts.push_back(B.alpha_g1.p);
    std::vector<uint32_t> icw; for (auto& p : ic_pts) append_words(icw, p);
    const uint32_t* d_ic = nullptr;
    if ((rc = dev_upload(K, &d_ic, icw))) return rc;
    uint32_t* d_ic_tab = nullptr;
    const G16Radix vrx = g16_radix(G16V_WBITS);
    if ((rc = build_tables<20>(K, ic_pts, &d_ic_tab, false, vrx))) return rc;
    K.vk_table_bytes = (uint64_t)ic_pts.size() * vrx.slot_ent * g16_table_entry_words(false, false) * 4ull;
    K.vk.gamma = B.gamma_g2.p; K.vk.delta = B.delta_g2.p; K.vk.beta = B.beta_g2.p; K.vk.n_ic = (uint32_t)B.abc.size(); K.vk.ic = d_ic; K.vk.ic_table = d_ic_tab;
    K.vk.ml_alpha_beta = miller_loop(B.beta_g2.p, aff_neg(B.alpha_g1.p));
    std::vector<uint32_t> kc(6 * 20), lines;
    g16_vm_key_constants(B.beta_g2.p, aff_neg(B.alpha_g1.p), B.gamma_g2.p, B.delta_g2.p, kc.data(), lines);
    if ((rc = dev_upload(K, &K.vm_kconst, kc)) || (rc = dev_upload(K, &K.vm_lines, lines))) return rc;
    K.vk_ready = true;
    return 0;
}
int ensure_mimc_dev() {
    if (g16s().mimc_dev) return 0;
    ensure_mimc_constants();
    std::vector<uint32_t> mc; for (auto& c : g_mimc_host) put_fr(mc, c);
    HIP_TRY(hipMalloc(&g16s().mimc_dev, mc.size() * 4)); HIP_TRY(hipMemcpy(g16s().mimc_dev, mc.data(), mc.size() * 4, hipMemcpyHostToDevice));
    return 0;
}
int load_key_body(int kind, const uint8_t* pk, uint64_t len) {
    G16Key& K = g16s().key[kind];
    const HostR1CS cs = kind == G16_EQUALITY ? build_equality_r1cs() : build_membership_r1cs();
    int rc;
    KeyReader R{pk, len};
    G16VkBlob B; G16PkBlob Q;
    const int format = g16_read_key_prefix(R, B);
    if (format == G16_BLOB_MALFORMED)
        return fail(ZKP_HIP_E_ARGUMENT, "malformed proving key or verifying key (expected ark-serialize uncompressed ProvingKey<Bn254>, or its VerifyingKey<Bn254> alone)");
    if (format == G16_BLOB_VERIFYING_KEY) {
        if (const char* why = g16_check_verifying_key(B, cs.n_inst)) return fail(ZKP_HIP_E_ARGUMENT, why);
        return install_verifying_key(K, B);
    }
    if (const char* why = g16_read_proving_key(R, B, g16_key_shape(cs), Q)) return fail(ZKP_HIP_E_ARGUMENT, why);
    const bool share_ab = env_int("ZKP_HIP_G16_SHARE_AB", 1) != 0;
    G16KeyPlan P;
    if (const char* why = g16_plan_key(P, B, Q, cs, share_ab)) return fail(ZKP_HIP_E_UNSUPPORTED, why);
    SharedTables want{}; want.hip_dev = dev().hip_dev; want.kind = kind; want.share_ab = share_ab; sha256_host(want.digest, pk, len);
    std::lock_guard<std::mutex> build_lock(table_build_mutex(want.hip_dev));
    if (env_int("ZKP_HIP_G16_WBITS", 0) != 0 || !acquire_tables(K, want, true)) {
        uint32_t wb = 0; bool uneven = false;
        if ((rc = choose_radix(P.radix_points_g1, P.radix_points_g2, &wb, &uneven))) return rc;
        K.rx = g16_radix(wb, uneven); want.wbits = K.rx.wbits | K.rx.uneven << 8;
        if (!acquire_tables(K, want, false)) {
            if ((rc = build_tables<20>(K, P.bases_g1, &want.g1, true, K.rx, false))) return rc;
            if ((rc = build_tables<40>(K, P.bases_g2, &want.g2, true, K.rx, false))) { (void)hipFree(want.g1); return rc; }
            register_tables(K, want);
        }
    }
    K.table_bytes = key_table_bytes(P.bases_g1.size(), P.bases_g2.size(), K.rx.wbits, K.rx.uneven);
    if ((rc = upload_circuit(K, cs)) || (rc = ensure_mimc_dev())) return rc;
    K.targets_g1 = g16_plan_targets(P.cls_g1, K.rx); K.targets_g2 = g16_plan_targets(P.cls_g2, K.rx);
    K.win_g1 = g16_windows(K.targets_g1); K.win_g2 = g16_windows(K.targets_g2);
    K.hscal_g1 = P.row_g1; K.hscal_g2 = P.row_g2;
    if ((rc = upload_offset_point(K, false, &K.init_g1)) || (rc = upload_offset_point(K, true, &K.init_g2))) return rc;
    if (!g16_check_verifying_key(B, K.n_inst) && (rc = install_verifying_key(K, B))) return rc;
    K.loaded = true;
    return 0;
}


fr tape_fr(const uint32_t seed[8], uint32_t idx, uint32_t slot) { uint32_t w[16]; tape_draw64(w, seed, idx, slot); return fp_from_wide<FrParams>(w); }

MsmView g16_msm_view(const G16Radix& rx, const DevLayout& D, const uint16_t* slot_scalar, const uint32_t* table, const uint32_t* acc_init, uint32_t rows, const uint32_t* digits, uint32_t* partial) {
    MsmView m; m.nwin = rx.nwin; m.nent = rx.nent; m.digw = rx.digw; m.slot_ent = rx.slot_ent; m.uneven = rx.uneven; m.rows = rows; m.nslots = D.nslots; m.nchunks = D.nchunks; m.table = table; m.digits = digits;
    m.slot_base = D.slot_base; m.slot_scalar = slot_scalar; m.slot_nwin = D.slot_nwin; m.chunk_begin = D.chunk_begin; m.chunk_win0 = D.chunk_win0; m.chunk_nwin = D.chunk_nwin; m.partial = partial; m.acc_init = acc_init;
    m.steps = D.steps; m.chunk_step0 = D.chunk_step0;
    return m;
}

int gpu_scalar_mults(bool g2, const std::vector<fr>& scalars, std::vector<uint8_t>& out_bytes) {
    const uint32_t rows = (uint32_t)scalars.size(), AW = g2 ? 40 : 20, JW = g2 ? G2_JAC_W : G1_JAC_W, PB = g2 ? 128 : 64;
    std::vector<uint32_t> base;
    if (!g2) append_words(base, host_g1_generator()); else append_words(base, host_g2_generator());
    std::vector<uint32_t> offs; append_offset(offs, g2, 0); append_offset(offs, g2, 1);
    const G16Radix rx = g16_radix(10);
    std::vector<uint32_t> dig((size_t)rx.digw * rows);
    for (uint32_t i = 0; i < rows; i++) {
        sc raw; fp_to_raw(raw.v, scalars[i]); uint32_t pk[G16_DIGW_MAX]; g16_recode(pk, raw, rx);
        for (uint32_t k = 0; k < rx.digw; k++) dig[(size_t)k * rows + i] = pk[k];
    }
    uint32_t *d_base = nullptr, *d_tab = nullptr, *d_dig = nullptr, *d_part = nullptr, *d_offs = nullptr, *d_sums = nullptr; uint8_t* d_out = nullptr;
    DevScope mem;
    HIP_TRY(mem.alloc(&d_base, AW * 4)); HIP_TRY(mem.alloc(&d_tab, (size_t)rx.slot_ent * g16_table_entry_words(g2, true) * 4 + 64)); HIP_TRY(mem.alloc(&d_dig, dig.size() * 4));
    HIP_TRY(mem.alloc(&d_part, (size_t)JW * 4 * rows)); HIP_TRY(mem.alloc(&d_sums, (size_t)JW * 4 * rows)); HIP_TRY(mem.alloc(&d_offs, offs.size() * 4));
    HIP_TRY(hipMemcpy(d_offs, offs.data(), offs.size() * 4, hipMemcpyHostToDevice)); HIP_TRY(mem.alloc(&d_out, (size_t)PB * rows));
    HIP_TRY(hipMemcpy(d_base, base.data(), AW * 4, hipMemcpyHostToDevice));
    HIP_TRY(hipMemcpy(d_dig, dig.data(), dig.size() * 4, hipMemcpyHostToDevice));
    struct OneSlot { DevLayout d; ~OneSlot() { free_layout(d); } } lay;
    const GatherShape shape{rx.nent, rx.slot_ent, rx.uneven ? 1u : 0u, rx.digw};
    if (int rc = upload_layout(lay.d, make_layout_even({SlotList{{0, (uint8_t)rx.nwin}}}, 1), &shape)) return rc;
    g16_launch_build_table(g2, d_base, 1, d_tab, dev().stream, true, rx);
    g16_launch_msm(g2, g16_msm_view(rx, lay.d, nullptr, d_tab, d_offs, rows, d_dig, d_part), dev().stream);
    ReduceView R{}; R.rows = rows; R.ntargets = 1; R.partial = d_part; R.target_chunk_begin = lay.d.target_chunk_begin; R.corr = d_offs + JW;
    g16_launch_sum(g2, R, d_sums, dev().stream);
    g16_launch_serialize(g2, d_sums, rows, d_out, dev().stream);
    out_bytes.resize((size_t)PB * rows);
    HIP_TRY(hipMemcpyAsync(out_bytes.data(), d_out, out_bytes.size(), hipMemcpyDeviceToHost, dev().stream));
    HIP_TRY(hipStreamSynchronize(dev().stream));
    return 0;
}

int generate_key_locked(int kind, const uint8_t* setup_seed, std::vector<uint8_t>& pk, std::vector<uint8_t>& vk) {
    if (kind != G16_EQUALITY && kind != G16_MEMBERSHIP) return fail(ZKP_HIP_E_ARGUMENT, "unknown circuit kind");
    const HostR1CS cs = kind == G16_EQUALITY ? build_equality_r1cs() : build_membership_r1cs();
    const HostCircuitTables T = build_circuit_tables(cs);
    uint32_t seed[8];
    if (setup_seed) memcpy(seed, setup_seed, 32);
    else { std::vector<uint8_t> f; int rc0 = fresh_seeds(f, 1); if (rc0) return rc0; memcpy(seed, f.data(), 32); }
    const char* tagname = kind == G16_EQUALITY ? "equality_mimc" : "membership_mimc";
    uint8_t th[32]; sha256_host(th, (const uint8_t*)tagname, strlen(tagname));
    const uint32_t tag = (uint32_t)th[0] | ((uint32_t)th[1] << 8) | ((uint32_t)th[2] << 16);
    fr tw[5];
    for (uint32_t k = 0; k < 5; k++) { tw[k] = tape_fr(seed, 0x47313601u, 8 * tag + k); if (fp_is_zero(tw[k])) tw[k] = fp_one<FrParams>(); }
    const fr alpha = tw[0], beta = tw[1], gamma = tw[2], delta = tw[3], tau = tw[4];
    const uint32_t m = T.m, nv = T.nv;
    const fr one = fp_one<FrParams>();
    fr taum = one; for (uint32_t i = 0; i < m; i++) taum = fp_mul(taum, tau);
    const fr zt = fp_sub(taum, one), minv = fp_inv(fp_from_u64<FrParams>(m));
    const fr w = fr9_to_fr<FrParams>(ld_fr9_c(T.tw.data(), 1));
    std::vector<fr> lag(m);
    fr wj = one;
    for (uint32_t j = 0; j < m; j++) { lag[j] = fp_mul(fp_mul(fp_mul(zt, minv), wj), fp_inv(fp_sub(tau, wj))); wj = fp_mul(wj, w); }
    std::vector<fr> At(nv, fp_zero<FrParams>()), Bt = At, Ct = At;
    std::vector<fr>* dst[3] = {&At, &Bt, &Ct};
    for (int q = 0; q < 3; q++)
        for (uint32_t j = 0; j < T.n_rows; j++)
            for (uint32_t e = T.ptr[q][j]; e < T.ptr[q][j + 1]; e++)
                (*dst[q])[T.col[q][e]] = fp_add((*dst[q])[T.col[q][e]], fp_mul(ld_fr_c(T.coef[q].data(), e), lag[j]));
    for (uint32_t i = 0; i < T.n_inst; i++) At[i] = fp_add(At[i], lag[T.n_rows + i]);
    const fr ginv = fp_inv(gamma), dinv = fp_inv(delta);
    auto mix = [&](uint32_t k) { return fp_add(fp_add(fp_mul(beta, At[k]), fp_mul(alpha, Bt[k])), Ct[k]); };
    std::vector<fr> s1 = {alpha, beta, delta}, s2 = {beta, gamma, delta};
    for (uint32_t i = 0; i < T.n_inst; i++) s1.push_back(fp_mul(mix(i), ginv));
    for (uint32_t k = 0; k < nv; k++) s1.push_back(At[k]);
    for (uint32_t k = 0; k < nv; k++) s1.push_back(Bt[k]);
    { fr tp = fp_mul(zt, dinv); for (uint32_t i = 0; i + 1 < m; i++) { s1.push_back(tp); tp = fp_mul(tp, tau); } }
    for (uint32_t k = T.n_inst; k < nv; k++) s1.push_back(fp_mul(mix(k), dinv));
    for (uint32_t k = 0; k < nv; k++) s2.push_back(Bt[k]);
    std::vector<uint8_t> b1, b2; int rc;
    if ((rc = gpu_scalar_mults(false, s1, b1)) || (rc = gpu_scalar_mults(true, s2, b2))) return rc;
    auto g1at = [&](size_t i) { return b1.data() + 64 * i; };
    auto g2at = [&](size_t i) { return b2.data() + 128 * i; };
    auto put = [](std::vector<uint8_t>& v, const uint8_t* p, size_t n) { v.insert(v.end(), p, p + n); };
    auto put_len = [](std::vector<uint8_t>& v, uint64_t n) { for (int i = 0; i < 8; i++) v.push_back((uint8_t)(n >> (8 * i))); };
    size_t o_abc = 3, o_a = o_abc + T.n_inst, o_b = o_a + nv, o_h = o_b + nv, o_l = o_h + (m - 1);
    vk.clear();
    put(vk, g1at(0), 64); put(vk, g2at(0), 128); put(vk, g2at(1), 128); put(vk, g2at(2), 128);
    put_len(vk, T.n_inst); put(vk, g1at(o_abc), 64ull * T.n_inst);
    pk = vk;
    put(pk, g1at(1), 64); put(pk, g1at(2), 64);
    put_len(pk, nv); put(pk, g1at(o_a), 64ull * nv);
    put_len(pk, nv); put(pk, g1at(o_b), 64ull * nv);
    put_len(pk, nv); put(pk, g2at(3), 128ull * nv);
    put_len(pk, m - 1); put(pk, g1at(o_h), 64ull * (m - 1));
    put_len(pk, T.n_wit); put(pk, g1at(o_l), 64ull * T.n_wit);
    return load_key_locked(kind, pk.data(), pk.size());
}

int launch_msm_key(bool g2, const G16Radix& rx, const G16Key::Chunking& ch, const uint32_t* table, const uint32_t* acc_init, uint32_t rows, const uint32_t* digits, uint32_t* partial, hipStream_t st) {
    const DevLayout& D = ch.lay;
    const MsmView m = g16_msm_view(rx, D, ch.scal, table, acc_init, rows, digits, partial);
    Device::KProf& K = dev().prof[g2 ? 2 : 1];
    hipEvent_t e1 = nullptr;
    int rc = prof_begin(K, st, &e1);
    if (rc) return rc;
    ZKP_TRACED(g2 ? "k_msm_gather<G2Msm>" : "k_msm_gather<G1Msm>", st, g16_launch_msm(g2, m, st));
    prof_end(K, st, e1, D.adds_per_row * rows);
    return 0;
}


int run_g16(int kind, uint32_t rows, const uint64_t* d_value, const uint64_t* d_set_vals, const uint32_t* d_set_len, const uint8_t* d_seeds,
            uint8_t* d_out, uint64_t stride, hipStream_t st, uint32_t lane = 0) {
    G16Key& K = g16s().key[kind];
    if (!K.loaded) return no_proving_key(K);
    const uint32_t nsc = g16_nscalars(K.nv, K.m);
    const G16Key::Chunking *c1 = nullptr, *c1c = nullptr, *c2 = nullptr;
    int rc;
    if ((rc = get_chunking(K, false, G16_PART_AB, rows, &c1)) || (rc = get_chunking(K, true, G16_PART_ALL, rows, &c2))) return rc;
    if ((rc = get_chunking(K, false, G16_PART_C, rows, &c1c))) return rc;
    size_t off = 0;
    auto sz = [&](size_t bytes) { size_t o = off; off += align_up(bytes); return o; };
    const size_t W = (size_t)32 * rows;
    const size_t o_z = sz(W * K.nv), o_sd = sz((size_t)K.rx.digw * 4 * rows * nsc), o_rs = sz(W * 2), o_p1 = sz((size_t)c1->lay.nchunks * G1_JAC_W * 4 * rows),
                 o_p1c = sz((size_t)c1c->lay.nchunks * G1_JAC_W * 4 * rows), o_p2 = sz((size_t)c2->lay.nchunks * G2_JAC_W * 4 * rows),
                 o_s1 = sz((size_t)3 * G1_JAC_W * 4 * rows), o_s2 = sz((size_t)G2_JAC_W * 4 * rows), o_t1 = sz((size_t)G16_CPARTS * G1_JAC_W * 4 * rows),
                 o_qe = sz((size_t)2 * 9 * K.m * 4 * rows);
    G16Run& RW = g16s().run[kind][lane & 1u];
    if (off > RW.cap) {
        if (RW.buf) { HIP_TRY(hipDeviceSynchronize()); HIP_TRY(hipFree(RW.buf)); RW.buf = nullptr; RW.cap = 0; }
        HIP_TRY(hipMalloc(&RW.buf, off)); RW.cap = off;
    }
    uint8_t* base = (uint8_t*)RW.buf;
    G16View V{}; V.rx = K.rx; V.rows = rows; V.kind = (uint32_t)kind; V.n_inst = K.n_inst; V.n_wit = K.n_wit; V.nv = K.nv; V.m = K.m;
    V.value = d_value; V.set_vals = d_set_vals; V.set_len = d_set_len; V.seeds = reinterpret_cast<const uint32_t*>(d_seeds); V.mimc_c = g16s().mimc_dev;
    V.z = (uint32_t*)(base + o_z); V.sdig = (uint32_t*)(base + o_sd); V.rs = (uint32_t*)(base + o_rs); V.out = d_out; V.stride = stride;
    V.qap_evals = (uint32_t*)(base + o_qe);
    uint32_t *p1 = (uint32_t*)(base + o_p1), *p1c = (uint32_t*)(base + o_p1c), *p2 = (uint32_t*)(base + o_p2), *s1 = (uint32_t*)(base + o_s1), *s2 = (uint32_t*)(base + o_s2), *t1 = (uint32_t*)(base + o_t1);
    if (!RW.last) {
        for (auto& e : RW.ev) HIP_TRY(hipEventCreateWithFlags(&e, hipEventDisableTiming));
        HIP_TRY(hipEventCreateWithFlags(&RW.last, hipEventDisableTiming));
    }
    G16Run& R0 = g16s().run[kind][0];
    if (!R0.side) {
        static const int side_level = env_int("ZKP_HIP_G16_SIDE_PRIORITY", 2), side2_level = env_int("ZKP_HIP_G16_SIDE2_PRIORITY", 0);
        HIP_TRY(hipStreamCreateWithPriority(&R0.side, hipStreamNonBlocking, stream_priority(side_level)));
        HIP_TRY(hipStreamCreateWithPriority(&R0.side2, hipStreamNonBlocking, stream_priority(side2_level)));
    }
    hipStream_t const side = R0.side, side2 = R0.side2;
    hipEvent_t ev_wit = RW.ev[0], ev_ab = RW.ev[1], ev_c = RW.ev[2], ev_cp = RW.ev[3];
    ReduceView R2{}; R2.rows = rows; R2.ntargets = 1; R2.partial = p2; R2.target_chunk_begin = c2->lay.target_chunk_begin; R2.corr = c2->corr;
    if (RW.used) HIP_TRY(hipStreamWaitEvent(st, RW.last, 0));
    ZKP_TRACED("k_g16_witness", st, g16_launch_witness(V, st));
    ZKP_TRACED("k_g16_zdigits", st, g16_launch_zdigits(V, st));
    HIP_TRY(hipEventRecord(ev_wit, st));
    HIP_TRY(hipStreamWaitEvent(side, ev_wit, 0));
    { TraceMark tm_("k_g16_qap", side); HIP_TRY(g16_launch_qap(V, K.C, side)); }
    if ((rc = launch_msm_key(false, K.rx, *c1c, K.table_g1, K.init_g1, rows, V.sdig, p1c, side))) return rc;
    ReduceView Rc{}; Rc.rows = rows; Rc.ntargets = 1; Rc.partial = p1c; Rc.target_chunk_begin = c1c->lay.target_chunk_begin; Rc.corr = c1c->corr;
    ZKP_TRACED("k_sum_t<G1Msm>", side, g16_launch_sum(false, Rc, s1 + (size_t)2 * G1_JAC_W * rows, side));
    HIP_TRY(hipEventRecord(ev_c, side));
    if ((rc = launch_msm_key(false, K.rx, *c1, K.table_g1, K.init_g1, rows, V.sdig, p1, st))) return rc;
    ReduceView Rab{}; Rab.rows = rows; Rab.ntargets = 2; Rab.partial = p1; Rab.target_chunk_begin = c1->lay.target_chunk_begin; Rab.corr = c1->corr;
    if (c1->lay.ntargets == 3) Rab.target_chunk_end = c1->lay.target_chunk_begin + 2;
    HIP_TRY(hipEventRecord(ev_ab, st));
    HIP_TRY(hipStreamWaitEvent(side2, ev_ab, 0));
    ZKP_TRACED("k_sum_t<G1Msm>", side2, g16_launch_sum(false, Rab, s1, side2));
    ZKP_TRACED("k_g16_cparts", side2, g16_launch_cparts(V, s1, t1, side2));
    HIP_TRY(hipEventRecord(ev_cp, side2));
    if ((rc = launch_msm_key(true, K.rx, *c2, K.table_g2, K.init_g2, rows, V.sdig, p2, st))) return rc;
    ZKP_TRACED("k_sum_t<G2Msm>", st, g16_launch_sum(true, R2, s2, st));
    HIP_TRY(hipStreamWaitEvent(st, ev_c, 0));
    HIP_TRY(hipStreamWaitEvent(st, ev_cp, 0));
    ZKP_TRACED("k_g16_final", st, g16_launch_final(V, s1, s2, t1, st));
    HIP_TRY(hipGetLastError());
    HIP_TRY(hipEventRecord(RW.last, st)); RW.used = true;
    return 0;
}

int prove_g16_host(int kind, uint64_t n, const uint64_t* values, const uint64_t* sets_flat, const uint32_t* set_counts, const std::vector<uint8_t>& valid,
                   const uint8_t* seeds, uint8_t* out, uint64_t stride, uint32_t* out_len, int32_t* status) {
    if (g16s().key[kind].verifier_only()) return no_proving_key(g16s().key[kind]);
    std::vector<uint64_t> v, sv; std::vector<uint32_t> sl, idx; std::vector<uint8_t> sd;
    size_t pos = 0; int any = 0;
    memset(out, 0, stride * n);
    for (uint64_t i = 0; i < n; i++) {
        const uint32_t cnt = set_counts ? set_counts[i] : 0;
        if (valid[i]) {
            idx.push_back((uint32_t)i); v.push_back(values[i]);
            sd.insert(sd.end(), seeds + 32 * i, seeds + 32 * i + 32);
            if (kind == G16_MEMBERSHIP) { sl.push_back(cnt); for (uint32_t k = 0; k < G16_MAX_SET; k++) sv.push_back(k < cnt ? sets_flat[pos + k] : 0); }
            const uint32_t plen = kind == G16_EQUALITY ? EQUALITY_ENVELOPE_BYTES : (uint32_t)membership_envelope_bytes(cnt);
            if (plen > stride) return fail(ZKP_HIP_E_ARGUMENT, "stride too small for the proof envelope");
            out_len[i] = plen; status[i] = ZKP_HIP_OK;
        } else { out_len[i] = 0; status[i] = ZKP_HIP_INVALID_INPUT; any = 1; }
        pos += cnt;
    }
    const uint32_t rows = (uint32_t)idx.size();
    if (rows == 0) return any;
    hipStream_t st = dev().stream;
    uint64_t *d_v = nullptr, *d_sv = nullptr; uint32_t* d_sl = nullptr; uint8_t *d_sd = nullptr, *d_out = nullptr;
    DevScope mem;
    HIP_TRY(mem.alloc(&d_v, 8ull * rows)); HIP_TRY(mem.alloc(&d_sd, 32ull * rows)); HIP_TRY(mem.alloc(&d_out, stride * rows));
    HIP_TRY(hipMemcpyAsync(d_v, v.data(), 8ull * rows, hipMemcpyHostToDevice, st));
    HIP_TRY(hipMemcpyAsync(d_sd, sd.data(), 32ull * rows, hipMemcpyHostToDevice, st));
    HIP_TRY(hipMemsetAsync(d_out, 0, stride * rows, st));
    if (kind == G16_MEMBERSHIP) {
        HIP_TRY(mem.alloc(&d_sv, 8ull * sv.size())); HIP_TRY(mem.alloc(&d_sl, 4ull * rows));
        HIP_TRY(hipMemcpyAsync(d_sv, sv.data(), 8ull * sv.size(), hipMemcpyHostToDevice, st));
        HIP_TRY(hipMemcpyAsync(d_sl, sl.data(), 4ull * rows, hipMemcpyHostToDevice, st));
    }
    int rc = run_g16(kind, rows, d_v, d_sv, d_sl, d_sd, d_out, stride, st);
    std::vector<uint8_t> tmp;
    if (rc == 0) {
        tmp.resize(stride * rows);
        HIP_TRY(hipMemcpyAsync(tmp.data(), d_out, stride * rows, hipMemcpyDeviceToHost, st));
        HIP_TRY(hipStreamSynchronize(st));
        for (uint32_t k = 0; k < rows; k++) memcpy(out + (uint64_t)idx[k] * stride, tmp.data() + (uint64_t)k * stride, stride);
    }
    if (rc) return rc;
    return any;
}

void g16_release_all() {
    G16State* S = dev().g16;
    if (!S) return;
    for (auto& circuit : S->run) for (auto& W : circuit) {
        if (W.side) { (void)hipStreamDestroy(W.side); (void)hipStreamDestroy(W.side2); }
        if (W.last) { for (auto e : W.ev) (void)hipEventDestroy(e); (void)hipEventDestroy(W.last); }
        if (W.buf) (void)hipFree(W.buf);
    }
    for (auto& K : S->key) release_key(K);
    if (S->mimc_dev) (void)hipFree(S->mimc_dev);
    g16_vm_free(S->vm);
    delete S; dev().g16 = nullptr;
}

int verify_g16_device(int kind, G16Key& K, const uint8_t* d_in, uint64_t stride, const uint32_t* d_len, uint32_t n, uint8_t* d_ok, uint8_t* ok, bool use_vm, DevScope& mem) {
    hipStream_t st = dev().stream;
    if (use_vm) {
        uint8_t* d_scratch = nullptr; uint32_t* d_special = nullptr; uint32_t special = 0;
        HIP_TRY(mem.alloc(&d_scratch, g16_vm_scratch_bytes(n))); HIP_TRY(mem.alloc(&d_special, 4));
        HIP_TRY(hipMemsetAsync(d_special, 0, 4, st));
        g16_launch_verify_vm(kind, d_in, stride, d_len, n, K.vk, g16s().vm, K.vm_kconst, K.vm_lines, d_scratch, d_ok, d_special, st);
        HIP_TRY(hipGetLastError());
        if (ok) HIP_TRY(hipMemcpyAsync(ok, d_ok, n, hipMemcpyDeviceToHost, st));
        HIP_TRY(hipMemcpyAsync(&special, d_special, 4, hipMemcpyDeviceToHost, st));
        HIP_TRY(hipStreamSynchronize(st));
        if (!special) return 0;
    }
    uint8_t* d_scratch2 = nullptr;
    HIP_TRY(mem.alloc(&d_scratch2, g16_verify_scratch_bytes(n)));
    g16_launch_verify(kind, d_in, stride, d_len, n, K.vk, d_scratch2, d_ok, st);
    HIP_TRY(hipGetLastError());
    if (ok) HIP_TRY(hipMemcpyAsync(ok, d_ok, n, hipMemcpyDeviceToHost, st));
    HIP_TRY(hipStreamSynchronize(st));
    return 0;
}

struct G16VerifyTally {
    Device& d; std::chrono::steady_clock::time_point t0 = std::chrono::steady_clock::now();
    uint64_t segment_checks = 0, envelopes = 0;
    explicit G16VerifyTally(Device& dv) : d(dv) {}
    ~G16VerifyTally() {
        Device::HostCounter& C = d.counter(ZKP_HIP_COUNTER_G16_VERIFY);
        C.a += segment_checks; C.b += envelopes;
        C.ms += std::chrono::duration<double, std::milli>(std::chrono::steady_clock::now() - t0).count();
    }
};

int localise_g16(int kind, G16Key& K, const uint8_t* d_in, uint64_t stride, const uint32_t* d_len, uint32_t n, uint8_t* d_rlc, uint8_t* d_ok, uint8_t* ok,
                 const uint32_t counters[4], DevScope& mem, G16VerifyTally& tally, bool* done) {
    *done = false;
    if (env_int("ZKP_HIP_G16_LOCALISE", 1) == 0) return 0;
    hipStream_t st = dev().stream;
    if (counters[0] == 0 && counters[1] == 0 && std::all_of(ok, ok + n, [](uint8_t v) { return v == 0; })) { *done = true; return 0; }
    const int forced = env_int("ZKP_HIP_G16_LOCALISE_SEGMENT", 0);
    const G16Segments g = g16_loc_segments(n, forced > 0 ? (uint32_t)forced : 0u);
    const uint32_t n_ic = K.vk.n_ic;
    uint8_t* d_loc = nullptr;
    HIP_TRY(mem.alloc(&d_loc, g16_loc_scratch_bytes(g.count, n_ic)));
    std::vector<uint8_t> suspect(g.count);
    g16_launch_localise(kind, d_in, stride, d_len, n, g, K.vk, g16s().vm, K.vm_kconst, K.vm_lines, d_rlc, d_ok, d_loc, st);
    HIP_TRY(hipGetLastError());
    HIP_TRY(hipMemcpyAsync(suspect.data(), d_loc, g.count, hipMemcpyDeviceToHost, st));
    HIP_TRY(hipStreamSynchronize(st));
    tally.segment_checks += g.count;
    std::vector<uint32_t> off((size_t)g.count + 1);
    const uint32_t m = g16_loc_offsets(g, n, suspect.data(), off.data());
    if (g16_loc_whole_batch(m, n)) return 0;
    *done = true;
    if (m == 0) return 0;
    uint8_t *d_in2 = nullptr, *d_ok2 = nullptr; uint32_t* d_len2 = nullptr;
    uint32_t* d_off = reinterpret_cast<uint32_t*>(d_loc + g16_loc_offsets_offset(g.count, n_ic));
    HIP_TRY(mem.alloc(&d_in2, stride * m)); HIP_TRY(mem.alloc(&d_len2, 4ull * m)); HIP_TRY(mem.alloc(&d_ok2, m));
    HIP_TRY(hipMemcpyAsync(d_off, off.data(), 4 * off.size(), hipMemcpyHostToDevice, st));
    g16_launch_compact(d_in, stride, d_len, n, g, d_loc, d_off, d_in2, d_len2, st);
    HIP_TRY(hipGetLastError());
    tally.envelopes += m;
    int rc = verify_g16_device(kind, K, d_in2, stride, d_len2, m, d_ok2, nullptr, true, mem);
    if (rc) return rc;
    g16_launch_scatter(n, g, d_loc, d_off, d_ok2, d_ok, st);
    HIP_TRY(hipGetLastError());
    HIP_TRY(hipMemcpyAsync(ok, d_ok, n, hipMemcpyDeviceToHost, st));
    HIP_TRY(hipStreamSynchronize(st));
    return 0;
}

int g16_rlc_min() { static const int v = env_int("ZKP_HIP_G16_BATCH_VERIFY_MIN", 8193); return v; }

int verify_g16_core(int kind, uint64_t n, const uint8_t* d_in, uint64_t stride, const uint32_t* d_len, uint8_t* d_ok, uint8_t* ok, DevScope& mem) {
    G16Key& K = g16s().key[kind];
    if (!K.vk_ready) return fail(ZKP_HIP_E_ARGUMENT, "no (usable) key loaded for this circuit (zkp_hip_groth16_load_key)");
    hipStream_t st = dev().stream;
    static const int use_vm = env_int("ZKP_HIP_G16_VERIFY_VM", 1);
    std::unique_ptr<G16VerifyTally> tally;
    if (use_vm) {
        G16VmTables& T = g16s().vm;
        if (!T.ready) {
            const int urc = g16_vm_upload(T);
            if (urc == -2) return fail(ZKP_HIP_E_RUNTIME, "hipFuncSetAttribute: the device refused the 160 KB dynamic LDS that the Groth16 verifier's Fq2 machine needs");
            if (urc) return fail(ZKP_HIP_E_RUNTIME, "could not place the verifier's tables in device memory");
        }
        const int rlc_min = g16_rlc_min();
        if (rlc_min > 0 && n >= (uint64_t)rlc_min && !getenv("ZKP_HIP_NO_BATCH_VERIFY")) {
            const uint32_t n_ic = K.vk.n_ic;
            uint8_t* d_rlc = nullptr;
            HIP_TRY(mem.alloc(&d_rlc, g16_rlc_scratch_bytes((uint32_t)n, n_ic)));
            std::vector<uint8_t> rnd; { int rcs = fresh_seeds(rnd, (n + 1) / 2); if (rcs) return rcs; }
            for (uint64_t j = 0; j < n; j++) { bool z = true; for (int k = 0; k < 16; k++) z = z && rnd[16 * j + k] == 0; if (z) rnd[16 * j] = 1; }
            uint32_t counters[4] = {0, 0, 0, 0};
            HIP_TRY(hipMemcpyAsync(d_rlc + g16_rlc_rho_offset((uint32_t)n, n_ic), rnd.data(), 16 * n, hipMemcpyHostToDevice, st));
            HIP_TRY(hipMemsetAsync(d_rlc + g16_rlc_counters_offset((uint32_t)n, n_ic), 0, sizeof counters, st));
            g16_launch_verify_rlc(kind, d_in, stride, d_len, (uint32_t)n, K.vk, T, K.vm_kconst, K.vm_lines, d_rlc, d_ok, st);
            HIP_TRY(hipGetLastError());
            HIP_TRY(hipMemcpyAsync(counters, d_rlc + g16_rlc_counters_offset((uint32_t)n, n_ic), sizeof counters, hipMemcpyDeviceToHost, st));
            HIP_TRY(hipMemcpyAsync(ok, d_ok, n, hipMemcpyDeviceToHost, st));
            HIP_TRY(hipStreamSynchronize(st));
            if (counters[0] == 0 && counters[1] == 0 && counters[2] == 0 && counters[3] == 1) return 0;
            if (getenv("ZKP_HIP_G16_BATCH_VERIFY_ONLY")) {
                char msg[160]; snprintf(msg, sizeof msg, "the batch check did not stand (special %u, outside the subgroup %u, anomalies %u, product is one: %u)", counters[0], counters[1], counters[2], counters[3]);
                return fail(ZKP_HIP_E_RUNTIME, msg);
            }
            tally.reset(new G16VerifyTally(dev()));
            bool done = false;
            const int rc = localise_g16(kind, K, d_in, stride, d_len, (uint32_t)n, d_rlc, d_ok, ok, counters, mem, *tally, &done);
            if (rc) return rc;
            if (done) return 0;
            tally->envelopes += n;
        }
    }
    return verify_g16_device(kind, K, d_in, stride, d_len, (uint32_t)n, d_ok, ok, use_vm != 0, mem);
}

uint64_t g16_min_slice() { const int v = g16_rlc_min(); return v > 0 ? (uint64_t)v : 8193u; }
bool g16_shard_holds_vk(Device* d, int kind) { std::lock_guard<std::mutex> lk(d->mu); return d->g16 && d->g16->key[kind].vk_ready; }

int verify_g16_host(int kind, uint64_t n, const uint8_t* proofs, uint64_t stride, const uint32_t* lens, uint8_t* ok) {
    if (!g16s().key[kind].vk_ready) return fail(ZKP_HIP_E_ARGUMENT, "no (usable) key loaded for this circuit (zkp_hip_groth16_load_key)");
    EnvelopeUpload up;
    Quiesce quiesce;
    int rc = up.open(n, proofs, stride, lens);
    if (rc || (rc = verify_g16_core(kind, n, up.d_in, stride, up.d_len, up.d_ok, ok, up.mem))) return rc;
    quiesce.armed = false;
    return 0;
}
int verify_g16_call(int kind, uint64_t n, const uint8_t* proofs, uint64_t stride, const uint32_t* lens, uint8_t* ok) {
    return verify_call(n,
        [&](const std::vector<Device*>& shards, VerifyFanout& F) {
            for (Device* d : shards) F.holds.push_back(g16_shard_holds_vk(d, kind));
            F.min_jobs = g16_min_slice();
            return 0;
        },
        [&](uint64_t lo, uint64_t m) { return verify_g16_host(kind, m, proofs + stride * lo, stride, lens + lo, ok + lo); });
}

}

extern "C" {

static int load_key_all_shards(int kind, const uint8_t* pk, uint64_t len, Device* skip) {
    std::vector<Device*> todo;
    {
        Device* d0 = nullptr; int rc = find_shard(0, &d0);
        if (rc) return rc;
        Registry& R = registry(); std::lock_guard<std::mutex> lk(R.mu);
        for (Device* d : R.shards) if (d != skip) todo.push_back(d);
    }
    return for_each_device(todo, [&](size_t) { return load_key_locked(kind, pk, len); });
}

int zkp_hip_groth16_load_key(int kind, const uint8_t* pk, uint64_t len) try {
    if (!pk) return fail(ZKP_HIP_E_ARGUMENT, "null proving key");
    return load_key_all_shards(kind, pk, len, nullptr);
} ZKP_API_CATCH_INT

int zkp_hip_groth16_key_info(int kind, uint32_t* wbits, uint32_t* uneven, uint64_t* table_bytes) try {
    if (kind != G16_EQUALITY && kind != G16_MEMBERSHIP && kind != ZKP_HIP_TABLES_BP_GENERATORS) return fail(ZKP_HIP_E_ARGUMENT, "unknown circuit kind");
    Bind bind; int rc = bind.open();
    if (rc) return rc;
    if (kind == ZKP_HIP_TABLES_BP_GENERATORS) {
        const EdgGeom& g = dev().edg;
        if (wbits) *wbits = g.wbits;
        if (uneven) *uneven = 0;
        if (table_bytes) *table_bytes = dev().d_edg_table ? (uint64_t)edg_table_words(g) * 4 : 0;
        return 0;
    }
    const G16Key& K = g16s().key[kind];
    if (K.verifier_only()) {
        if (wbits) *wbits = G16V_WBITS;
        if (uneven) *uneven = 0;
        if (table_bytes) *table_bytes = K.vk_table_bytes;
        return 0;
    }
    if (!K.loaded) return fail(ZKP_HIP_E_ARGUMENT, "no proving key loaded for this circuit (zkp_hip_groth16_load_key)");
    if (wbits) *wbits = K.rx.wbits;
    if (uneven) *uneven = K.rx.uneven ? 1u : 0u;
    if (table_bytes) *table_bytes = K.table_bytes;
    return 0;
} ZKP_API_CATCH_INT

int zkp_hip_groth16_generate_key(int kind, const uint8_t* setup_seed, uint8_t* pk_out, uint64_t pk_cap, uint64_t* pk_len,
                                 uint8_t* vk_out, uint64_t vk_cap, uint64_t* vk_len) try {
    std::vector<uint8_t> pk, vk;
    Device* here = nullptr;
    {
        Bind bind; int rc = bind.open();
        if (rc) return rc;
        here = &dev();
        if ((rc = generate_key_locked(kind, setup_seed, pk, vk))) return rc;
    }
    int rc = load_key_all_shards(kind, pk.data(), pk.size(), here);
    if (rc) return rc;
    if (pk_len) *pk_len = pk.size();
    if (vk_len) *vk_len = vk.size();
    if (pk_out) { if (pk_cap < pk.size()) return fail(ZKP_HIP_E_ARGUMENT, "pk buffer too small"); memcpy(pk_out, pk.data(), pk.size()); }
    if (vk_out) { if (vk_cap < vk.size()) return fail(ZKP_HIP_E_ARGUMENT, "vk buffer too small"); memcpy(vk_out, vk.data(), vk.size()); }
    return 0;
} ZKP_API_CATCH_INT

int zkp_hip_verify_equality_batch(uint64_t n, const uint8_t* proofs, uint64_t stride, const uint32_t* lens, uint8_t* ok) try {
    if (n == 0) return 0;
    const int rc = verifier_args(n, {proofs, lens, ok}, stride);
    return rc ? rc : verify_g16_call(G16_EQUALITY, n, proofs, stride, lens, ok);
} ZKP_API_CATCH_INT
int zkp_hip_verify_membership_batch(uint64_t n, const uint8_t* proofs, uint64_t stride, const uint32_t* lens, uint8_t* ok) try {
    if (n == 0) return 0;
    const int rc = verifier_args(n, {proofs, lens, ok}, stride);
    return rc ? rc : verify_g16_call(G16_MEMBERSHIP, n, proofs, stride, lens, ok);
} ZKP_API_CATCH_INT

int zkp_hip_snark_commit_value_batch(uint64_t n, const uint64_t* values, uint8_t* out) try {
    if (n == 0) return 0;
    Bind bind; int rc = host_args(n, {values, out});
    if (rc || (rc = bind.open())) return rc;
    if ((rc = ensure_mimc_dev())) return rc;
    uint64_t* d_v = nullptr; uint8_t* d_o = nullptr;
    DevScope mem;
    HIP_TRY(mem.alloc(&d_v, 8 * n)); HIP_TRY(mem.alloc(&d_o, 32 * n));
    HIP_TRY(hipMemcpyAsync(d_v, values, 8 * n, hipMemcpyHostToDevice, dev().stream));
    g16_launch_mimc(d_v, (uint32_t)n, g16s().mimc_dev, d_o, dev().stream);
    HIP_TRY(hipMemcpyAsync(out, d_o, 32 * n, hipMemcpyDeviceToHost, dev().stream));
    HIP_TRY(hipStreamSynchronize(dev().stream));
    return 0;
} ZKP_API_CATCH_INT

int zkp_hip_prove_equality_batch(uint64_t n, const uint64_t* val1, const uint64_t* val2, const uint8_t* seeds,
                                 uint8_t* out, uint64_t stride, uint32_t* out_len, int32_t* status) try {
    if (n == 0) return 0;
    std::vector<uint8_t> fresh;
    int rc = prover_args(fresh, seeds, n, {val1, val2, out, out_len, status}, nullptr, stride, EQUALITY_ENVELOPE_BYTES, "stride must be >= 298");
    if (rc) return rc;
    std::vector<uint8_t> valid(n);
    for (uint64_t i = 0; i < n; i++) valid[i] = equality_ok(val1[i], val2[i]);
    Bind bind;
    if ((rc = bind.open())) return rc;
    return prove_g16_host(G16_EQUALITY, n, val1, nullptr, nullptr, valid, seeds, out, stride, out_len, status);
} ZKP_API_CATCH_INT

int zkp_hip_prove_membership_batch(uint64_t n, const uint64_t* values, const uint64_t* sets, const uint32_t* set_counts, const uint8_t* seeds,
                                   uint8_t* out, uint64_t stride, uint32_t* out_len, int32_t* status) try {
    if (n == 0) return 0;
    std::vector<uint8_t> fresh;
    int rc = prover_args(fresh, seeds, n, {values, sets, set_counts, out, out_len, status}, set_counts);
    if (rc) return rc;
    std::vector<uint8_t> valid(n);
    for (uint64_t i = 0, pos = 0; i < n; pos += set_counts[i++]) valid[i] = membership_ok(values[i], sets + pos, set_counts[i]);
    Bind bind;
    if ((rc = bind.open())) return rc;
    return prove_g16_host(G16_MEMBERSHIP, n, values, sets, set_counts, valid, seeds, out, stride, out_len, status);
} ZKP_API_CATCH_INT

}
```

libzkp_amd/csrc/g16_kernels.hip:

```cpp
#include "g16_launch.h"
#include "msm_kernel.h"

struct G1Msm {
    static constexpr uint32_t ACC_W = G1_JAC_W, DIG_PER_WORD = 2;
    static __device__ __forceinline__ int32_t digit(uint32_t word, uint32_t w) { return (int32_t)(int16_t)(word >> (16 * (w & 1u))); }
    using Acc = g1_jac;
    static __device__ __forceinline__ Acc identity() { return jac_infinity<fq>(); }
    static constexpr uint32_t GATHER_WAVES = 3; static constexpr int GATHER_PREFETCH = 2;
    static constexpr uint32_t GATHER_W = 16, GATHER_STRIDE = 16, GATHER_PRIO = 0;
    using GAcc = g1_xyzz9;
    static __device__ __forceinline__ GAcc to_gather(const g1_jac& a) { return xyzz9_from_jac(a); }
    static __device__ __forceinline__ g1_jac from_gather(const GAcc& a) { return jac_from_xyzz9(a); }
    static __device__ __forceinline__ GAcc accumulate_entry(const GAcc& acc, int32_t d, const uint32_t* e) {
        g1_aff9 q{fq9_unpack8(e), fq9_unpack8(e + 8)};
        q.y = fq9_select(d < 0, fq9_neg_k<4>(q.y), q.y);
        return g1_mmadd9(acc, q);
    }
    static __device__ __forceinline__ void store(uint32_t* p, uint32_t idx, uint32_t row, uint32_t rows, const Acc& a) { st_g1_jac(p, idx, row, rows, a); }
    static __device__ __forceinline__ Acc load(const uint32_t* p, uint32_t idx, uint32_t row, uint32_t rows) { return ld_g1_jac(p, idx, row, rows); }
    static __device__ __forceinline__ Acc add(const Acc& a, const Acc& b) { return jac_add(a, b); }
};
struct G2Msm {
    static constexpr uint32_t ACC_W = G2_JAC_W, DIG_PER_WORD = 2;
    static __device__ __forceinline__ int32_t digit(uint32_t word, uint32_t w) { return (int32_t)(int16_t)(word >> (16 * (w & 1u))); }
    using Acc = g2_jac;
    static __device__ __forceinline__ Acc identity() { return jac_infinity<fq2>(); }
    static constexpr uint32_t GATHER_WAVES = 2; static constexpr int GATHER_PREFETCH = -1;
    static constexpr uint32_t GATHER_W = 32, GATHER_STRIDE = 32, GATHER_PRIO = 0;
    using GAcc = g2_xyzz9;
    static __device__ __forceinline__ GAcc to_gather(const g2_jac& a) { return g2_xyzz9_from_jac(a); }
    static __device__ __forceinline__ g2_jac from_gather(const GAcc& a) { return jac_from_g2_xyzz9(a); }
    static __device__ __forceinline__ GAcc accumulate_entry(const GAcc& acc, int32_t d, const uint32_t* e) {
        const g2_aff9 q{fq2_9{fq9_unpack8(e), fq9_unpack8(e + 8)}, fq2_9{fq9_unpack8(e + 16), fq9_unpack8(e + 24)}};
        return g2_mmadd9(acc, q, d < 0);
    }
    static __device__ __forceinline__ void store(uint32_t* p, uint32_t idx, uint32_t row, uint32_t rows, const Acc& a) { st_g2_jac(p, idx, row, rows, a); }
    static __device__ __forceinline__ Acc load(const uint32_t* p, uint32_t idx, uint32_t row, uint32_t rows) { return ld_g2_jac(p, idx, row, rows); }
    static __device__ __forceinline__ Acc add(const Acc& a, const Acc& b) { return jac_add(a, b); }
};


__global__ void __launch_bounds__(TW) k_g16_witness(G16View V) {
    ZKP_RAISE_PRIO();
    const uint32_t row = blockIdx.x * TW + threadIdx.x;
    if (row < V.rows) step_g16_witness(V, row);
}
__global__ void __launch_bounds__(TB) k_g16_zdigits(G16View V) {
    ZKP_RAISE_PRIO();
    const uint32_t row = blockIdx.x * TB + threadIdx.x;
    if (row < V.rows) step_g16_zdigits(V, blockIdx.y, row);
}
struct DevSync { __device__ __forceinline__ void operator()() const { __syncthreads(); } };
static constexpr int QAP_TB_MAX = 256;
__global__ void __launch_bounds__(QAP_TB_MAX) k_g16_qap(G16View V, G16Circuit C) {
    extern __shared__ uint32_t g16_lds[];
    G16Lds L; L.base = g16_lds; L.m = C.m;
    g16_qap_proof(V, C, L, V.qap_evals + (size_t)blockIdx.x * 2 * 9 * C.m, blockIdx.x, threadIdx.x, blockDim.x, DevSync());
}
__global__ void __launch_bounds__(TW) k_g16_cparts(G16View V, const uint32_t* sum_g1, uint32_t* tmp_g1) {
    ZKP_RAISE_PRIO();
    const uint32_t row = blockIdx.x * TW + threadIdx.x;
    if (row < V.rows) step_g16_cparts(V, sum_g1, tmp_g1, blockIdx.y, row);
}
__global__ void __launch_bounds__(TW) k_g16_final(G16View V, const uint32_t* sum_g1, const uint32_t* sum_g2, const uint32_t* tmp_g1) {
    ZKP_RAISE_PRIO();
    const uint32_t row = blockIdx.x * TW + threadIdx.x;
    if (row < V.rows) step_g16_final(V, sum_g1, sum_g2, tmp_g1, blockIdx.y, row);
}
__global__ void __launch_bounds__(TW) k_mimc_commit(const uint64_t* values, uint32_t n, const uint32_t* mimc_c, uint8_t* out) {
    const uint32_t i = blockIdx.x * TW + threadIdx.x;
    if (i >= n) return;
    G16View V{}; V.mimc_c = mimc_c; V.z = nullptr;
    const fr h = g16_mimc_chain(V, 0, fp_from_u64<FrParams>(values[i]), 0);
    uint32_t w[8]; fp_to_raw(w, h);
    g16_put_bytes(out + 32ull * i, w, 8);
}
constexpr uint32_t G16_TABLE_SEG = 512;
template <class F, uint32_t AFF_W>
__global__ void __launch_bounds__(TW, 2) k_g16_build_table(const uint32_t* bases, uint32_t nslots, uint32_t* table, uint32_t fmt9, G16Radix rx) {
    const uint32_t seg_len = rx.nent < G16_TABLE_SEG ? rx.nent : G16_TABLE_SEG, nseg = rx.nent / seg_len, slot_seg = rx.slot_ent / seg_len;
    const uint32_t t = blockIdx.x * TW + threadIdx.x;
    if (t >= nslots * slot_seg) return;
    const uint32_t slot = t / slot_seg, sg = t % slot_seg;
    uint32_t win = sg / nseg, seg = sg % nseg;
    if (rx.uneven && sg >= 16u * nseg) { win = sg < 18u * nseg ? 16u : 17u; seg = sg - (win == 16u ? 16u : 18u) * nseg; }
    constexpr uint32_t FW = AFF_W / 2, BATCH = 8;
    Aff<F> base;
    {
        const uint32_t* b = bases + (size_t)slot * AFF_W;
        uint32_t* bx = reinterpret_cast<uint32_t*>(&base.x); uint32_t* by = reinterpret_cast<uint32_t*>(&base.y);
        for (uint32_t k = 0; k < FW; k++) { bx[k] = b[k]; by[k] = b[FW + k]; }
    }
    Jac<F> q = jac_from_aff(base);
    for (uint32_t i = 0; i < g16_win_bit(rx, win); i++) q = jac_dbl(q);
    Jac<F> acc = q;
    {
        const uint32_t first = seg * seg_len + 1;
        int top = 31; while (top > 0 && !((first >> top) & 1u)) top--;
        for (int b = top - 1; b >= 0; b--) { acc = jac_dbl(acc); if ((first >> b) & 1u) acc = jac_add(acc, q); }
    }
    constexpr uint32_t NC = AFF_W / 10;
    const uint32_t OW = fmt9 ? 8 * NC : AFF_W;
    uint32_t* dst = table + ((size_t)slot * rx.slot_ent + g16_win_off(rx, win) + (size_t)seg * seg_len) * OW;
    for (uint32_t e0 = 0; e0 < seg_len; e0 += BATCH) {
        Jac<F> pts[BATCH]; F zp[BATCH];
        for (uint32_t k = 0; k < BATCH; k++) {
            pts[k] = acc; acc = jac_add(acc, q);
            zp[k] = k ? f_mul(zp[k - 1], pts[k].Z) : pts[k].Z;
        }
        F inv = f_inv(zp[BATCH - 1]);
        for (int k = BATCH - 1; k >= 0; k--) {
            const F zi = k ? f_mul(inv, zp[k - 1]) : inv;
            if (k) inv = f_mul(inv, pts[k].Z);
            const F zi2 = f_sq(zi);
            Aff<F> a; a.x = f_mul(pts[k].X, zi2); a.y = f_mul(pts[k].Y, f_mul(zi2, zi));
            const uint32_t* ax = reinterpret_cast<const uint32_t*>(&a.x); const uint32_t* ay = reinterpret_cast<const uint32_t*>(&a.y);
            uint32_t* o = dst + (size_t)(e0 + k) * OW;
            if (fmt9) {
                const fq* c = reinterpret_cast<const fq*>(&a);
                for (uint32_t t2 = 0; t2 < NC; t2++) fq9_pack8(o + 8 * t2, fq9_from_fq(c[t2]));
                continue;
            }
            for (uint32_t j = 0; j < FW; j++) { o[j] = ax[j]; o[FW + j] = ay[j]; }
        }
    }
}



__global__ void __launch_bounds__(TW) k_g16_serialize(bool g2, const uint32_t* jac, uint32_t rows, uint8_t* out) {
    const uint32_t row = blockIdx.x * TW + threadIdx.x;
    if (row >= rows) return;
    if (!g2) { uint32_t w[16]; g1_serialize(w, ld_g1_jac(jac, 0, row, rows)); g16_put_bytes(out + 64ull * row, w, 16); }
    else { uint32_t w[32]; g2_serialize(w, ld_g2_jac(jac, 0, row, rows)); g16_put_bytes(out + 128ull * row, w, 32); }
}

template __global__ void k_msm_gather<G1Msm>(MsmView, uint32_t, uint32_t);
template __global__ void k_msm_gather<G2Msm>(MsmView, uint32_t, uint32_t);
static constexpr uint32_t G16_SUM_ROWS = 8, G16_SUM_TB = 256;
template __global__ void k_sum_t<G1Msm, G16_SUM_ROWS, G16_SUM_TB>(ReduceView, uint32_t*);
template __global__ void k_sum_t<G2Msm, G16_SUM_ROWS, G16_SUM_TB>(ReduceView, uint32_t*);
template __global__ void k_g16_build_table<fq, 20>(const uint32_t*, uint32_t, uint32_t*, uint32_t, G16Radix);
template __global__ void k_g16_build_table<fq2, 40>(const uint32_t*, uint32_t, uint32_t*, uint32_t, G16Radix);

void g16_launch_witness(const G16View& V, hipStream_t st) { k_g16_witness<<<(V.rows + TW - 1) / TW, TW, 0, st>>>(V); }
void g16_launch_zdigits(const G16View& V, hipStream_t st) { k_g16_zdigits<<<dim3((V.rows + TB - 1) / TB, V.nv), TB, 0, st>>>(V); }
hipError_t g16_launch_qap(const G16View& V, const G16Circuit& C, hipStream_t st) {
    const size_t lds = (size_t)9 * C.m * 4;
    const uint32_t tb = C.m / 4;
    if (tb < 64 || tb > (uint32_t)QAP_TB_MAX || (tb & 63u)) return hipErrorInvalidValue;
    k_g16_qap<<<V.rows, tb, lds, st>>>(V, C);
    return hipSuccess;
}
void g16_launch_cparts(const G16View& V, const uint32_t* sum_g1, uint32_t* tmp_g1, hipStream_t st) {
    k_g16_cparts<<<dim3((V.rows + TW - 1) / TW, G16_CPARTS), TW, 0, st>>>(V, sum_g1, tmp_g1);
}
void g16_launch_final(const G16View& V, const uint32_t* sum_g1, const uint32_t* sum_g2, const uint32_t* tmp_g1, hipStream_t st) {
    k_g16_final<<<dim3((V.rows + TW - 1) / TW, 3), TW, 0, st>>>(V, sum_g1, sum_g2, tmp_g1);
}
void g16_launch_mimc(const uint64_t* values, uint32_t n, const uint32_t* mimc_c, uint8_t* out, hipStream_t st) { k_mimc_commit<<<(n + TW - 1) / TW, TW, 0, st>>>(values, n, mimc_c, out); }
void g16_launch_build_table(bool g2, const uint32_t* bases, uint32_t nslots, uint32_t* table, hipStream_t st, bool msm_form, const G16Radix& rx) {
    const uint32_t seg_len = rx.nent < G16_TABLE_SEG ? rx.nent : G16_TABLE_SEG;
    const uint32_t threads = nslots * (rx.slot_ent / seg_len);
    if (!g2) k_g16_build_table<fq, 20><<<(threads + TW - 1) / TW, TW, 0, st>>>(bases, nslots, table, msm_form ? 1u : 0u, rx);
    else k_g16_build_table<fq2, 40><<<(threads + TW - 1) / TW, TW, 0, st>>>(bases, nslots, table, msm_form ? 1u : 0u, rx);
}
uint32_t g16_table_entry_words(bool g2, bool msm_form) { return msm_form ? (g2 ? G2Msm::GATHER_W : G1Msm::GATHER_W) : (g2 ? 40u : 20u); }
uint32_t g16_msm_rows_per_block(bool) { return 256u; }
uint32_t g16_msm_blocks_per_cu(bool g2) { return g2 ? G2Msm::GATHER_WAVES : G1Msm::GATHER_WAVES; }
void g16_launch_msm(bool g2, const MsmView& m, hipStream_t st) {
    const uint32_t ngroups = (m.rows + 255u) / 256u, nblocks = m.nchunks * ngroups, grid = ((nblocks + 7) / 8) * 8;
    if constexpr (gather_lds_bytes<G2Msm>() > 0 || gather_lds_bytes<G1Msm>() > 0) {
        if (gather_lds_bytes<G1Msm>()) (void)hipFuncSetAttribute(reinterpret_cast<const void*>(k_msm_gather<G1Msm>), hipFuncAttributeMaxDynamicSharedMemorySize, (int)gather_lds_bytes<G1Msm>());
        if (gather_lds_bytes<G2Msm>()) (void)hipFuncSetAttribute(reinterpret_cast<const void*>(k_msm_gather<G2Msm>), hipFuncAttributeMaxDynamicSharedMemorySize, (int)gather_lds_bytes<G2Msm>());
    }
    if (!g2) k_msm_gather<G1Msm><<<grid, 256, gather_lds_bytes<G1Msm>(), st>>>(m, ngroups, nblocks);
    else k_msm_gather<G2Msm><<<grid, 256, gather_lds_bytes<G2Msm>(), st>>>(m, ngroups, nblocks);
}
void g16_launch_sum(bool g2, const ReduceView& R, uint32_t* sums, hipStream_t st) {
    const dim3 grid((R.rows + G16_SUM_ROWS - 1) / G16_SUM_ROWS, R.ntargets);
    if (!g2) k_sum_t<G1Msm, G16_SUM_ROWS, G16_SUM_TB><<<grid, G16_SUM_TB, 0, st>>>(R, sums);
    else k_sum_t<G2Msm, G16_SUM_ROWS, G16_SUM_TB><<<grid, G16_SUM_TB, 0, st>>>(R, sums);
}
void g16_launch_serialize(bool g2, const uint32_t* jac, uint32_t rows, uint8_t* out, hipStream_t st) { k_g16_serialize<<<(rows + TW - 1) / TW, TW, 0, st>>>(g2, jac, rows, out); }
```

libzkp_amd/csrc/g16_launch.h:

```cpp
#pragma once
#include <hip/hip_runtime.h>
#include "g16_steps.h"
#include "bp_steps.h"

void g16_launch_witness(const zkp::G16View& V, hipStream_t st);
void g16_launch_zdigits(const zkp::G16View& V, hipStream_t st);
hipError_t g16_launch_qap(const zkp::G16View& V, const zkp::G16Circuit& C, hipStream_t st);
void g16_launch_cparts(const zkp::G16View& V, const uint32_t* sum_g1, uint32_t* tmp_g1, hipStream_t st);
void g16_launch_final(const zkp::G16View& V, const uint32_t* sum_g1, const uint32_t* sum_g2, const uint32_t* tmp_g1, hipStream_t st);
void g16_launch_mimc(const uint64_t* values, uint32_t n, const uint32_t* mimc_c, uint8_t* out, hipStream_t st);
void g16_launch_build_table(bool g2, const uint32_t* bases, uint32_t nslots, uint32_t* table, hipStream_t st, bool msm_form, const zkp::G16Radix& rx);
uint32_t g16_table_entry_words(bool g2, bool msm_form);
uint32_t g16_msm_rows_per_block(bool g2);
uint32_t g16_msm_blocks_per_cu(bool g2);
void g16_launch_msm(bool g2, const zkp::MsmView& m, hipStream_t st);
void g16_launch_sum(bool g2, const zkp::ReduceView& R, uint32_t* sums, hipStream_t st);
void g16_launch_serialize(bool g2, const uint32_t* jac, uint32_t rows, uint8_t* out, hipStream_t st);
```

libzkp_amd/csrc/g16_share.h:

```cpp
#pragma once
#include <cstdint>
#include <vector>
#include "bp_layout.h"
#include "g16_circuit.h"
#include "g16_keyblob.h"

namespace zkp {

inline bool g16_shared_point(const G1Pt& a, const G1Pt& b) { return !a.inf && !b.inf && fq_eq(a.p.x, b.p.x) && fq_eq(a.p.y, b.p.y); }

struct G16AbSlots { SlotList a, s, b; };
inline G16AbSlots g16_ab_slots(const std::vector<G1Pt>& aq, const std::vector<G1Pt>& b1q, const std::vector<uint8_t>& cls, bool share) {
    G16AbSlots out;
    const size_t n = aq.size() < b1q.size() ? aq.size() : b1q.size();
    for (size_t k = 0; k < aq.size(); k++) {
        if (aq[k].inf) continue;
        if (share && k < n && g16_shared_point(aq[k], b1q[k])) out.s.push_back({(uint16_t)k, cls[k]});
        else out.a.push_back({(uint16_t)k, cls[k]});
    }
    for (size_t k = 0; k < b1q.size(); k++) {
        if (b1q[k].inf || (share && k < n && g16_shared_point(aq[k], b1q[k]))) continue;
        out.b.push_back({(uint16_t)k, cls[k]});
    }
    return out;
}

inline std::vector<SlotList> g16_ab_targets(const SlotList& a, const SlotList& s, const SlotList& b) {
    if (s.empty()) return {a, b};
    return {a, s, b};
}
struct G16AbRanges { uint16_t begin[2], end[2]; };
inline G16AbRanges g16_ab_ranges(const MsmLayout& L) {
    const auto& t = L.target_chunk_begin;
    if (L.ntargets() == 3) return {{t[0], t[1]}, {t[2], t[3]}};
    return {{t[0], t[1]}, {t[1], t[2]}};
}

inline G16KeyShape g16_key_shape(const HostR1CS& cs) { return {cs.n_inst + cs.n_wit, 1u << g16_domain_log2(cs), cs.n_wit, cs.n_inst}; }

struct G16KeyPlan {
    std::vector<g1_aff> bases_g1; std::vector<g2_aff> bases_g2;
    std::vector<uint16_t> row_g1, row_g2;
    std::vector<SlotList> cls_g1, cls_g2;
    size_t radix_points_g1 = 0, radix_points_g2 = 0;
};
inline const char* g16_plan_key(G16KeyPlan& P, const G16VkBlob& vk, const G16PkBlob& pk, const HostR1CS& cs, bool share_ab) {
    const G16KeyShape sh = g16_key_shape(cs);
    if (sh.nv + sh.m + 3 > 65535 || 3ull * sh.nv + sh.m + 8 > 65535) return "circuit too large for 16-bit slot indices";
    const uint32_t SC_H = sh.nv, SC_R = sh.nv + sh.m - 1, SC_S = SC_R + 1, SC_NRS = SC_R + 2, SC_ONE = SC_R + 3;
    std::vector<uint8_t> cls(cs.inst_nwin); cls.insert(cls.end(), cs.wit_nwin.begin(), cs.wit_nwin.end());
    P = G16KeyPlan(); P.cls_g1.resize(4); P.cls_g2.resize(1);
    auto add1 = [&](int list, const G1Pt& pt, uint32_t row, uint8_t c) {
        if (pt.inf) return;
        P.cls_g1[list].push_back({(uint16_t)P.bases_g1.size(), c}); P.bases_g1.push_back(pt.p); P.row_g1.push_back((uint16_t)row);
    };
    auto add2 = [&](const G2Pt& pt, uint32_t row, uint8_t c) {
        if (pt.inf) return;
        P.cls_g2[0].push_back({(uint16_t)P.bases_g2.size(), c}); P.bases_g2.push_back(pt.p); P.row_g2.push_back((uint16_t)row);
    };
    const G16AbSlots ab = g16_ab_slots(pk.a_query, pk.b_g1_query, cls, share_ab);
    for (auto& sl : ab.a) add1(0, pk.a_query[sl.first], sl.first, sl.second);
    add1(0, pk.delta_g1, SC_R, G16_NW_FULL); add1(0, vk.alpha_g1, SC_ONE, 1);
    for (auto& sl : ab.s) add1(1, pk.a_query[sl.first], sl.first, sl.second);
    for (auto& sl : ab.b) add1(2, pk.b_g1_query[sl.first], sl.first, sl.second);
    add1(2, pk.delta_g1, SC_S, G16_NW_FULL); add1(2, pk.beta_g1, SC_ONE, 1);
    for (uint32_t k = 0; k < sh.n_wit; k++) add1(3, pk.l_query[k], sh.n_inst + k, cls[sh.n_inst + k]);
    for (uint32_t i = 0; i + 1 < sh.m; i++) add1(3, pk.h_query[i], SC_H + i, G16_NW_FULL);
    add1(3, pk.delta_g1, SC_NRS, G16_NW_FULL);
    for (uint32_t k = 0; k < sh.nv; k++) add2(pk.b_g2_query[k], k, cls[k]);
    add2(vk.delta_g2, SC_S, G16_NW_FULL); add2(vk.beta_g2, SC_ONE, 1);
    P.radix_points_g1 = pk.a_query.size() + pk.b_g1_query.size() - ab.s.size() + pk.l_query.size() + pk.h_query.size() + 5;
    P.radix_points_g2 = pk.b_g2_query.size() + 2;
    return nullptr;
}
inline std::vector<SlotList> g16_plan_targets(const std::vector<SlotList>& cls, const G16Radix& rx) {
    std::vector<SlotList> out = cls;
    for (auto& t : out) for (auto& sl : t) sl.second = g16_class_nwin(sl.second, rx);
    return out;
}
inline uint64_t g16_windows(const std::vector<SlotList>& targets) { uint64_t w = 0; for (auto& t : targets) for (auto& sl : t) w += sl.second; return w; }

enum { G16_PART_ALL = 0, G16_PART_AB = 1, G16_PART_C = 2 };
inline std::vector<SlotList> g16_part_targets(const std::vector<SlotList>& all, int part) {
    if (part == G16_PART_ALL) return all;
    if (part == G16_PART_AB) return g16_ab_targets(all[0], all[1], all[2]);
    return std::vector<SlotList>(all.begin() + 3, all.end());
}
struct G16Chunks { MsmLayout L; std::vector<uint16_t> scal; std::vector<uint32_t> offsets; };
inline G16Chunks g16_plan_chunks(const std::vector<SlotList>& targets, const std::vector<uint16_t>& row, int part, uint32_t chunks) {
    G16Chunks C; C.L = make_layout_even(targets, chunks);
    for (uint16_t b : C.L.slot_base) C.scal.push_back(row[b]);
    if (part == G16_PART_AB) { const G16AbRanges ab = g16_ab_ranges(C.L); for (int t = 0; t < 2; t++) C.offsets.push_back((uint32_t)ab.end[t] - ab.begin[t]); }
    else for (uint32_t t = 0; t < C.L.ntargets(); t++) C.offsets.push_back((uint32_t)C.L.target_chunk_begin[t + 1] - C.L.target_chunk_begin[t]);
    return C;
}

}
```

libzkp_amd/csrc/msm_kernel.h:

```cpp
#pragma once
#include <hip/hip_runtime.h>
#include "bp_steps.h"

using namespace zkp;
static constexpr int TW = 64;
static constexpr int TB = 256;


template <class T> constexpr size_t gather_lds_bytes() { return T::GATHER_PREFETCH < 0 ? (size_t)4 * 2 * (T::GATHER_W / 4) * 64 * 16 : 0; }
template <class T>
__global__ void __launch_bounds__(256, T::GATHER_WAVES) k_msm_gather(MsmView m, uint32_t ngroups, uint32_t nblocks) {
    constexpr uint32_t V4 = T::GATHER_W / 4;
    constexpr uint32_t SV4 = T::GATHER_STRIDE / 4;
    const uint32_t tid = threadIdx.x;
    const uint32_t per_xcd = (nblocks + 7) / 8;
    const uint32_t linear = (blockIdx.x & 7u) * per_xcd + (blockIdx.x >> 3);
    if (linear >= nblocks) return;
    const uint32_t chunk = linear / ngroups, group = linear % ngroups;
    const uint32_t row = group * 256u + tid;
    const bool active = row < m.rows;
    const uint32_t st0 = m.chunk_step0[chunk], left = m.chunk_step0[chunk + 1] - st0;
    const uint2* const steps = reinterpret_cast<const uint2*>(m.steps) + st0;
    typename T::GAcc acc = T::to_gather(m.acc_init ? T::load(m.acc_init, 0, 0, 1) : T::identity());
    const uint4* const table4 = reinterpret_cast<const uint4*>(m.table);
    auto digit_word = [&](const uint2 ds) -> uint32_t { return active ? m.digits[(size_t)(ds.y >> 1) * m.rows + row] : 0u; };
    auto entry_of = [&](const uint2 ds, int32_t d) -> const uint4* { return table4 + ((uint64_t)ds.x + (uint32_t)((d < 0 ? -d : d) - 1)) * SV4; };
    if (left == 0) { if (active) T::store(m.partial, chunk, row, m.rows, T::from_gather(acc)); return; }
    if constexpr (T::GATHER_PREFETCH < 0) {
#if defined(__HIP_DEVICE_COMPILE__)
        extern __shared__ uint4 gather_lds[];
        const uint32_t wave = tid >> 6, lane = tid & 63u;
        uint4* const wbuf = gather_lds + (size_t)wave * (2u * V4 * 64u);
        auto dma = [&](uint32_t buf, const uint2 ds, int32_t dd) {
            if (dd == 0) return;
            const uint4* src = entry_of(ds, dd);
            ZKP_UNROLL for (uint32_t k = 0; k < V4; k++) __builtin_amdgcn_global_load_lds(src + k, wbuf + (buf * V4 + k) * 64u, 16, 0, 0);
        };
        uint32_t cb = 0;
        int32_t d = T::digit(digit_word(steps[0]), steps[0].y & 1u);
        uint32_t q0 = left > 1 ? digit_word(steps[1]) : 0u, q1 = left > 2 ? digit_word(steps[2]) : 0u;
        dma(0, steps[0], d);
        for (uint32_t i = 0; i < left; i++) {
            int32_t dn = 0;
            asm volatile("s_waitcnt vmcnt(0)" ::: "memory");
            uint4 e[V4];
            if (d != 0) { ZKP_UNROLL for (uint32_t k = 0; k < V4; k++) e[k] = wbuf[(cb * V4 + k) * 64u + lane]; }
            if (i + 1 < left) { const uint2 ds = steps[i + 1]; dn = T::digit(q0, ds.y & 1u); dma(cb ^ 1u, ds, dn); }
            const uint32_t qn = i + 3 < left ? digit_word(steps[i + 3]) : 0u;
            if (d != 0) acc = T::accumulate_entry(acc, d, reinterpret_cast<const uint32_t*>(e));
            cb ^= 1u; d = dn; q0 = q1; q1 = qn;
        }
        if (active) T::store(m.partial, chunk, row, m.rows, T::from_gather(acc));
        return;
#endif
    } else {
        constexpr int LEAD = T::GATHER_PREFETCH;
        uint4 e[LEAD + 1][V4]; int32_t dd[LEAD + 1];
        auto fetch = [&](uint4* dst, const uint2 ds, int32_t d) {
            if (d == 0) return;
            const uint4* src = entry_of(ds, d);
            ZKP_UNROLL for (uint32_t k = 0; k < V4; k++) dst[k] = src[k];
        };
        uint32_t qpre[LEAD + 2];
        ZKP_UNROLL for (int k = 0; k < LEAD + 2; k++) qpre[k] = (uint32_t)k < left ? digit_word(steps[k]) : 0u;
        ZKP_UNROLL for (int k = 0; k < LEAD; k++) {
            dd[k] = 0;
            if ((uint32_t)k < left) { const uint2 ds = steps[k]; dd[k] = T::digit(qpre[k], ds.y & 1u); fetch(e[k], ds, dd[k]); }
        }
        uint32_t q0 = qpre[LEAD], q1 = qpre[LEAD + 1];
        if constexpr (T::GATHER_PRIO > 0) __builtin_amdgcn_s_setprio(T::GATHER_PRIO);
        for (uint32_t i = 0; i < left; i++) {
            dd[LEAD] = 0;
            if (i + LEAD < left) { const uint2 ds = steps[i + LEAD]; dd[LEAD] = T::digit(q0, ds.y & 1u); fetch(e[LEAD], ds, dd[LEAD]); }
            const uint32_t qn = i + LEAD + 2 < left ? digit_word(steps[i + LEAD + 2]) : 0u;
            if (dd[0] != 0) acc = T::accumulate_entry(acc, dd[0], reinterpret_cast<const uint32_t*>(e[0]));
            ZKP_UNROLL for (int k = 0; k < LEAD; k++) { ZKP_UNROLL for (uint32_t v = 0; v < V4; v++) e[k][v] = e[k + 1][v]; dd[k] = dd[k + 1]; }
            q0 = q1; q1 = qn;
        }
    }
    if (active) T::store(m.partial, chunk, row, m.rows, T::from_gather(acc));
}

template <class T, uint32_t ROWS, uint32_t NTHREADS, uint32_t MIN_WAVES = 1>
__global__ void __launch_bounds__(NTHREADS, MIN_WAVES) k_sum_t(ReduceView R, uint32_t* sums) {
    ZKP_RAISE_PRIO();
    constexpr uint32_t SLICES = NTHREADS / ROWS;
    static_assert(NTHREADS % ROWS == 0 && (SLICES & (SLICES - 1)) == 0, "slices per row: a power of two");
    __shared__ uint32_t lds[T::ACC_W * (NTHREADS / 2)];
    const uint32_t rl = threadIdx.x % ROWS, slice = threadIdx.x / ROWS;
    const uint32_t row = blockIdx.x * ROWS + rl, target = blockIdx.y;
    const bool active = row < R.rows;
    const uint32_t c0 = R.target_chunk_begin[target], c1 = reduce_chunk_end(R, target);
    typename T::Acc acc = T::identity();
    bool have = false;
    if (active) {
        for (uint32_t c = c0 + slice; c < c1; c += SLICES) {
            const typename T::Acc p = T::load(R.partial, c, row, R.rows);
            acc = have ? T::add(acc, p) : p;
            have = true;
        }
    }
    for (uint32_t stride = SLICES / 2; stride >= 1; stride >>= 1) {
        if (slice >= stride && slice < 2 * stride) T::store(lds, 0, (slice - stride) * ROWS + rl, NTHREADS / 2, acc);
        __syncthreads();
        if (slice < stride) acc = T::add(acc, T::load(lds, 0, slice * ROWS + rl, NTHREADS / 2));
        __syncthreads();
    }
    if (slice == 0 && active) {
        if (R.corr) acc = T::add(acc, T::load(R.corr, target, 0, 1));
        T::store(sums, target, row, R.rows, acc);
    }
}
```

Before: 346,100.

## Merge four chunk waves per workgroup in Groth16 MSM gather via LDS tree add

```diff
diff --git a/libzkp_amd/csrc/bn254_g.h b/libzkp_amd/csrc/bn254_g.h
--- a/libzkp_amd/csrc/bn254_g.h
+++ b/libzkp_amd/csrc/bn254_g.h
@@ -119,6 +119,27 @@
     r.ZZ = fq9_mul(p.ZZ, PP);
     r.ZZZ = fq9_mul(p.ZZZ, PPP);
     return r;
+}
+template <class Src> ZKP_HD inline g1_xyzz9 g1_add9_from(const g1_xyzz9& p, Src&& q) {
+    const fq9 zz2 = q(2);
+    const fq9 U1 = fq9_mul(p.X, zz2), zz12 = fq9_mul(p.ZZ, zz2);
+    const fq9 U2 = fq9_mul(q(0), p.ZZ);
+    const fq9 zzz2 = q(3);
+    const fq9 S1 = fq9_mul(p.Y, zzz2), zzz12 = fq9_mul(p.ZZZ, zzz2);
+    const fq9 S2 = fq9_mul(q(1), p.ZZZ);
+    const fq9 P = fq9_sub_k<2>(U2, U1), Rv = fq9_sub_k<2>(S2, S1);
+    const fq9 PP = fq9_sq(P);
+    const fq9 PPP = fq9_mul(P, PP), Q = fq9_mul(U1, PP);
+    const fq9 RR = fq9_sq(Rv);
+    g1_xyzz9 r;
+    r.X = fq9_sub2_k4(RR, PPP, Q);
+    r.Y = fq9_mul_add2(Rv, fq9_sub_loose<8>(Q, r.X), fq9_neg_loose<4>(S1), PPP);
+    r.ZZ = fq9_mul(zz12, PP);
+    r.ZZZ = fq9_mul(zzz12, PPP);
+    return r;
+}
+ZKP_HD inline g1_xyzz9 g1_add9(const g1_xyzz9& p, const g1_xyzz9& q) {
+    return g1_add9_from(p, [&](int k) -> const fq9& { return k == 0 ? q.X : k == 1 ? q.Y : k == 2 ? q.ZZ : q.ZZZ; });
 }
 ZKP_HD inline g1_xyzz9 xyzz9_from_jac(const Jac<fq>& p) {
     const fq zz = fq_sq(p.Z);
@@ -188,6 +209,40 @@
     r.ZZZ = fq2_9_mul(PPP, p.ZZZ, nZZZ1);
     return r;
 }
+template <class Src> ZKP_HD inline g2_xyzz9 g2_add9_from(const g2_xyzz9& p, Src&& q) {
+    fq2_9 U1, U2, S1, S2, zz12, zzz12;
+    {
+        const fq2_9 zz2{q(4), q(5)};
+        const fq9 nZZ2 = fq9_neg_k<4>(zz2.c1);
+        U1 = fq2_9_mul(p.X, zz2, nZZ2); zz12 = fq2_9_mul(p.ZZ, zz2, nZZ2);
+    }
+    { const fq2_9 x2{q(0), q(1)}; U2 = fq2_9_mul(x2, p.ZZ, fq9_neg_k<4>(p.ZZ.c1)); }
+    {
+        const fq2_9 zzz2{q(6), q(7)};
+        const fq9 nZZZ2 = fq9_neg_k<4>(zzz2.c1);
+        S1 = fq2_9_mul(p.Y, zzz2, nZZZ2); zzz12 = fq2_9_mul(p.ZZZ, zzz2, nZZZ2);
+    }
+    { const fq2_9 y2{q(2), q(3)}; S2 = fq2_9_mul(y2, p.ZZZ, fq9_neg_k<4>(p.ZZZ.c1)); }
+    const fq2_9 P{fq9_sub_k<2>(U2.c0, U1.c0), fq9_sub_k<2>(U2.c1, U1.c1)};
+    const fq2_9 Rv{fq9_sub_k<2>(S2.c0, S1.c0), fq9_sub_k<2>(S2.c1, S1.c1)};
+    const fq2_9 PP = fq2_9_sq(P, fq9_neg_k<4>(P.c1));
+    const fq9 nPP1 = fq9_neg_k<2>(PP.c1);
+    const fq2_9 PPP = fq2_9_mul(P, PP, nPP1), Q = fq2_9_mul(U1, PP, nPP1);
+    const fq9 nR1 = fq9_neg_k<4>(Rv.c1);
+    const fq2_9 RR = fq2_9_sq(Rv, nR1);
+    g2_xyzz9 r;
+    r.X = fq2_9{fq9_sub2_k<4>(RR.c0, PPP.c0, Q.c0), fq9_sub2_k<4>(RR.c1, PPP.c1, Q.c1)};
+    const fq2_9 W{fq9_sub_k<8>(Q.c0, r.X.c0), fq9_sub_k<8>(Q.c1, r.X.c1)};
+    const fq9 nS0 = fq9_neg_k<2>(S1.c0), nS1 = fq9_neg_k<2>(S1.c1);
+    r.Y = fq2_9{fq9_mul_add4(Rv.c0, W.c0, nR1, W.c1, nS0, PPP.c0, S1.c1, PPP.c1),
+                fq9_mul_add4(Rv.c0, W.c1, Rv.c1, W.c0, nS0, PPP.c1, nS1, PPP.c0)};
+    r.ZZ = fq2_9_mul(zz12, PP, nPP1);
+    r.ZZZ = fq2_9_mul(zzz12, PPP, fq9_neg_k<2>(PPP.c1));
+    return r;
+}
+ZKP_HD inline g2_xyzz9 g2_add9(const g2_xyzz9& p, const g2_xyzz9& q) {
+    return g2_add9_from(p, [&](int k) -> const fq9& { return k == 0 ? q.X.c0 : k == 1 ? q.X.c1 : k == 2 ? q.Y.c0 : k == 3 ? q.Y.c1 : k == 4 ? q.ZZ.c0 : k == 5 ? q.ZZ.c1 : k == 6 ? q.ZZZ.c0 : q.ZZZ.c1; });
+}
 ZKP_HD inline fq2_9 fq2_9_from_fq2(const fq2& a) { return fq2_9{fq9_from_fq(a.c0), fq9_from_fq(a.c1)}; }
 ZKP_HD inline fq2 fq2_9_to_fq2(const fq2_9& a) { return fq2{fq9_to_fq(a.c0), fq9_to_fq(a.c1)}; }
 ZKP_HD inline g2_xyzz9 g2_xyzz9_from_jac(const Jac<fq2>& p) {
diff --git a/libzkp_amd/csrc/bp_layout.h b/libzkp_amd/csrc/bp_layout.h
--- a/libzkp_amd/csrc/bp_layout.h
+++ b/libzkp_amd/csrc/bp_layout.h
@@ -101,7 +101,7 @@
     }
     return L;
 }
-inline MsmLayout make_layout_even(const std::vector<SlotList>& targets, uint32_t total_chunks) {
+inline MsmLayout make_layout_even(const std::vector<SlotList>& targets, uint32_t total_chunks, uint32_t gran = 1) {
     MsmLayout L;
     uint64_t W = 0; for (const auto& t : targets) for (const auto& s : t) W += s.second;
     L.target_chunk_begin.push_back(0);
@@ -110,12 +110,13 @@
         uint32_t k = (uint32_t)((uint64_t)total_chunks * wt / (W ? W : 1));
         if (k < 1) k = 1;
         if (k > wt && wt) k = wt;
+        if (gran > 1) k = (k + gran - 1) / gran * gran;
         const uint32_t slot0 = (uint32_t)L.slot_base.size();
         for (const auto& s : t) { L.slot_base.push_back(s.first); L.slot_nwin.push_back(s.second); }
         uint32_t slot = slot0, win = 0, done = 0;
         for (uint32_t c = 0; c < k; c++) {
             const uint32_t upto = (uint32_t)((uint64_t)wt * (c + 1) / k), n = upto - done;
-            if (n == 0) continue;
+            if (n == 0 && gran == 1) continue;
             L.chunk_begin.push_back((uint16_t)slot); L.chunk_win0.push_back((uint16_t)win); L.chunk_nwin.push_back((uint16_t)n);
             uint32_t left = n;
             while (left) { const uint32_t room = L.slot_nwin[slot] - win, step = left < room ? left : room; win += step; left -= step; if (win == L.slot_nwin[slot]) { slot++; win = 0; } }
diff --git a/libzkp_amd/csrc/bp_steps.h b/libzkp_amd/csrc/bp_steps.h
--- a/libzkp_amd/csrc/bp_steps.h
+++ b/libzkp_amd/csrc/bp_steps.h
@@ -158,6 +158,7 @@
     uint32_t nwin = 0, nent = 0, digw = 0;
     uint32_t slot_ent = 0, uneven = 0;
     const uint32_t* steps = nullptr; const uint32_t* chunk_step0 = nullptr;
+    uint32_t merge = 0;
 };
 ZKP_HD inline void msm_chunk_ref(const MsmView& m, uint32_t chunk, uint32_t row) {
     ge acc = ge_identity();
@@ -179,6 +180,7 @@
     uint8_t* out;
     const uint32_t* corr;
     const uint16_t* target_chunk_end = nullptr;
+    uint32_t few_partials = 0;
 };
 ZKP_HD inline uint32_t reduce_chunk_end(const ReduceView& r, uint32_t target) { return r.target_chunk_end ? r.target_chunk_end[target] : r.target_chunk_begin[target + 1]; }
 ZKP_HD inline void reduce_encode_thread(const ReduceView& r, uint32_t target, uint32_t row) {
diff --git a/libzkp_amd/csrc/g16_impl.inc b/libzkp_amd/csrc/g16_impl.inc
--- a/libzkp_amd/csrc/g16_impl.inc
+++ b/libzkp_amd/csrc/g16_impl.inc
@@ -16,6 +16,7 @@
     std::map<uint64_t, Chunking> lays_g1, lays_g2;
     uint64_t win_g1 = 0, win_g2 = 0;
     const uint32_t *init_g1 = nullptr, *init_g2 = nullptr;
+    uint32_t merge = G16_MERGE;
     G16Vk vk{}; bool vk_ready = false;
     uint64_t vk_table_bytes = 0;
     bool verifier_only() const { return vk_ready && !loaded; }
@@ -92,14 +93,19 @@
     const MsmOffsets& o = msm_offsets();
     if (!g2) append_words(v, k ? host_neg_multiple(o.o1, k) : o.o1); else append_words(v, k ? host_neg_multiple(o.o2, k) : o.o2);
 }
-int upload_offset_point(G16Key& K, bool g2, const uint32_t** d_init) { std::vector<uint32_t> init; append_offset(init, g2, 0); return dev_upload(K, d_init, init); }
-uint32_t choose_chunks(uint64_t windows, uint32_t ntargets, uint32_t rows, uint32_t resident, uint32_t tb) {
-    const uint32_t groups = (rows + tb - 1) / tb;
-    uint32_t hi = (uint32_t)(windows / 8); if (hi > 2048) hi = 2048; if (hi < ntargets) hi = ntargets;
-    uint32_t best = ntargets; double best_cost = 1e300;
-    for (uint32_t c = ntargets; c <= hi; c++) {
-        const double rounds = std::ceil((double)c * groups / resident);
-        const double cost = rounds * (std::ceil((double)windows / c) + 2.5) + 0.25 * c / 8.0;
+template <class J> void append_multiples(std::vector<uint32_t>& v, const J& o, uint32_t n) { J acc = o; for (uint32_t i = 0; i < n; i++) { append_words(v, acc); acc = i ? jac_add(acc, o) : jac_dbl(o); } }
+int upload_offset_point(G16Key& K, bool g2, const uint32_t** d_init) {
+    std::vector<uint32_t> init;
+    if (!g2) append_multiples(init, msm_offsets().o1, G16_MERGE); else append_multiples(init, msm_offsets().o2, G16_MERGE);
+    return dev_upload(K, d_init, init);
+}
+uint32_t choose_chunks(uint64_t windows, uint32_t ntargets, uint32_t rows, uint32_t resident, uint32_t tb, uint32_t merge = 0) {
+    const uint32_t groups = (rows + tb - 1) / tb, step = merge ? merge : 1u, lo = ntargets * step;
+    uint32_t hi = (uint32_t)(windows / 8); if (hi > 2048) hi = 2048; if (hi < lo) hi = lo;
+    uint32_t best = lo; double best_cost = 1e300;
+    for (uint32_t c = lo; c <= hi; c += step) {
+        const double rounds = std::ceil((double)(c / step) * groups / resident);
+        const double cost = rounds * (std::ceil((double)windows / c) + 2.5 + (merge ? 3.0 : 0.0)) + 0.25 * (c / step) / 8.0;
         if (cost < best_cost) { best_cost = cost; best = c; }
     }
     return best;
@@ -108,18 +114,19 @@
     const uint32_t resident = (uint32_t)dev().num_cu * g16_msm_blocks_per_cu(g2);
     if (part == G16_PART_ALL && !g2) return fail(ZKP_HIP_E_ARGUMENT, "G16_PART_ALL is the G2 launch");
     const std::vector<SlotList> targets = g16_part_targets(g2 ? K.targets_g2 : K.targets_g1, part);
-    uint32_t c = choose_chunks(g16_windows(targets), (uint32_t)targets.size(), rows, resident, g16_msm_rows_per_block(g2));
+    uint32_t c = choose_chunks(g16_windows(targets), (uint32_t)targets.size(), rows, resident, g16_msm_rows_per_block(g2, K.merge), K.merge);
     if (g_budget_request >= 10000) c = g_budget_request - 10000;
     auto& cache = g2 ? K.lays_g2 : K.lays_g1;
     const uint64_t key = (uint64_t)part << 32 | c;
     auto it = cache.find(key);
     if (it == cache.end()) {
-        const G16Chunks P = g16_plan_chunks(targets, g2 ? K.hscal_g2 : K.hscal_g1, part, c);
+        G16Chunks P = g16_plan_chunks(targets, g2 ? K.hscal_g2 : K.hscal_g1, part, c, K.merge);
         G16Key::Chunking ch; int rc;
         const GatherShape shape{K.rx.nent, K.rx.slot_ent, K.rx.uneven ? 1u : 0u, K.rx.digw};
+        P.L.target_chunk_begin = P.reduce_begin;
         if ((rc = upload_layout(ch.lay, P.L, &shape, P.scal.data()))) return rc;
         std::vector<uint32_t> corr;
-        for (uint32_t k : P.offsets) append_offset(corr, g2, k);
+        for (uint32_t t = 0; t < P.offsets.size(); t++) append_offset(corr, g2, g16_offset_points(P, K.merge, t));
         if ((rc = dev_upload(K, &ch.corr, corr))) return rc;
         if ((rc = dev_upload(K, &ch.scal, P.scal))) return rc;
         it = cache.emplace(key, ch).first;
@@ -289,6 +296,7 @@
     K.targets_g1 = g16_plan_targets(P.cls_g1, K.rx); K.targets_g2 = g16_plan_targets(P.cls_g2, K.rx);
     K.win_g1 = g16_windows(K.targets_g1); K.win_g2 = g16_windows(K.targets_g2);
     K.hscal_g1 = P.row_g1; K.hscal_g2 = P.row_g2;
+    K.merge = env_int("ZKP_HIP_G16_MERGE", (int)G16_MERGE) == 0 ? 0u : G16_MERGE;
     if ((rc = upload_offset_point(K, false, &K.init_g1)) || (rc = upload_offset_point(K, true, &K.init_g2))) return rc;
     if (!g16_check_verifying_key(B, K.n_inst) && (rc = install_verifying_key(K, B))) return rc;
     K.loaded = true;
@@ -394,9 +402,10 @@
     return load_key_locked(kind, pk.data(), pk.size());
 }
 
-int launch_msm_key(bool g2, const G16Radix& rx, const G16Key::Chunking& ch, const uint32_t* table, const uint32_t* acc_init, uint32_t rows, const uint32_t* digits, uint32_t* partial, hipStream_t st) {
+int launch_msm_key(bool g2, const G16Radix& rx, const G16Key::Chunking& ch, const uint32_t* table, const uint32_t* acc_init, uint32_t rows, const uint32_t* digits, uint32_t* partial, hipStream_t st, uint32_t merge) {
     const DevLayout& D = ch.lay;
-    const MsmView m = g16_msm_view(rx, D, ch.scal, table, acc_init, rows, digits, partial);
+    MsmView m = g16_msm_view(rx, D, ch.scal, table, acc_init, rows, digits, partial);
+    m.merge = merge;
     Device::KProf& K = dev().prof[g2 ? 2 : 1];
     hipEvent_t e1 = nullptr;
     int rc = prof_begin(K, st, &e1);
@@ -419,8 +428,9 @@
     size_t off = 0;
     auto sz = [&](size_t bytes) { size_t o = off; off += align_up(bytes); return o; };
     const size_t W = (size_t)32 * rows;
-    const size_t o_z = sz(W * K.nv), o_sd = sz((size_t)K.rx.digw * 4 * rows * nsc), o_rs = sz(W * 2), o_p1 = sz((size_t)c1->lay.nchunks * G1_JAC_W * 4 * rows),
-                 o_p1c = sz((size_t)c1c->lay.nchunks * G1_JAC_W * 4 * rows), o_p2 = sz((size_t)c2->lay.nchunks * G2_JAC_W * 4 * rows),
+    const uint32_t per = K.merge ? K.merge : 1u;
+    const size_t o_z = sz(W * K.nv), o_sd = sz((size_t)K.rx.digw * 4 * rows * nsc), o_rs = sz(W * 2), o_p1 = sz((size_t)(c1->lay.nchunks / per) * G1_JAC_W * 4 * rows),
+                 o_p1c = sz((size_t)(c1c->lay.nchunks / per) * G1_JAC_W * 4 * rows), o_p2 = sz((size_t)(c2->lay.nchunks / per) * G2_JAC_W * 4 * rows),
                  o_s1 = sz((size_t)3 * G1_JAC_W * 4 * rows), o_s2 = sz((size_t)G2_JAC_W * 4 * rows), o_t1 = sz((size_t)G16_CPARTS * G1_JAC_W * 4 * rows),
                  o_qe = sz((size_t)2 * 9 * K.m * 4 * rows);
     G16Run& RW = g16s().run[kind][lane & 1u];
@@ -446,26 +456,26 @@
     }
     hipStream_t const side = R0.side, side2 = R0.side2;
     hipEvent_t ev_wit = RW.ev[0], ev_ab = RW.ev[1], ev_c = RW.ev[2], ev_cp = RW.ev[3];
-    ReduceView R2{}; R2.rows = rows; R2.ntargets = 1; R2.partial = p2; R2.target_chunk_begin = c2->lay.target_chunk_begin; R2.corr = c2->corr;
+    ReduceView R2{}; R2.rows = rows; R2.ntargets = 1; R2.partial = p2; R2.target_chunk_begin = c2->lay.target_chunk_begin; R2.corr = c2->corr; R2.few_partials = K.merge != 0;
     if (RW.used) HIP_TRY(hipStreamWaitEvent(st, RW.last, 0));
     ZKP_TRACED("k_g16_witness", st, g16_launch_witness(V, st));
     ZKP_TRACED("k_g16_zdigits", st, g16_launch_zdigits(V, st));
     HIP_TRY(hipEventRecord(ev_wit, st));
     HIP_TRY(hipStreamWaitEvent(side, ev_wit, 0));
     { TraceMark tm_("k_g16_qap", side); HIP_TRY(g16_launch_qap(V, K.C, side)); }
-    if ((rc = launch_msm_key(false, K.rx, *c1c, K.table_g1, K.init_g1, rows, V.sdig, p1c, side))) return rc;
-    ReduceView Rc{}; Rc.rows = rows; Rc.ntargets = 1; Rc.partial = p1c; Rc.target_chunk_begin = c1c->lay.target_chunk_begin; Rc.corr = c1c->corr;
+    if ((rc = launch_msm_key(false, K.rx, *c1c, K.table_g1, K.init_g1, rows, V.sdig, p1c, side, K.merge))) return rc;
+    ReduceView Rc{}; Rc.rows = rows; Rc.ntargets = 1; Rc.partial = p1c; Rc.target_chunk_begin = c1c->lay.target_chunk_begin; Rc.corr = c1c->corr; Rc.few_partials = K.merge != 0;
     ZKP_TRACED("k_sum_t<G1Msm>", side, g16_launch_sum(false, Rc, s1 + (size_t)2 * G1_JAC_W * rows, side));
     HIP_TRY(hipEventRecord(ev_c, side));
-    if ((rc = launch_msm_key(false, K.rx, *c1, K.table_g1, K.init_g1, rows, V.sdig, p1, st))) return rc;
-    ReduceView Rab{}; Rab.rows = rows; Rab.ntargets = 2; Rab.partial = p1; Rab.target_chunk_begin = c1->lay.target_chunk_begin; Rab.corr = c1->corr;
+    if ((rc = launch_msm_key(false, K.rx, *c1, K.table_g1, K.init_g1, rows, V.sdig, p1, st, K.merge))) return rc;
+    ReduceView Rab{}; Rab.rows = rows; Rab.ntargets = 2; Rab.partial = p1; Rab.target_chunk_begin = c1->lay.target_chunk_begin; Rab.corr = c1->corr; Rab.few_partials = K.merge != 0;
     if (c1->lay.ntargets == 3) Rab.target_chunk_end = c1->lay.target_chunk_begin + 2;
     HIP_TRY(hipEventRecord(ev_ab, st));
     HIP_TRY(hipStreamWaitEvent(side2, ev_ab, 0));
     ZKP_TRACED("k_sum_t<G1Msm>", side2, g16_launch_sum(false, Rab, s1, side2));
     ZKP_TRACED("k_g16_cparts", side2, g16_launch_cparts(V, s1, t1, side2));
     HIP_TRY(hipEventRecord(ev_cp, side2));
-    if ((rc = launch_msm_key(true, K.rx, *c2, K.table_g2, K.init_g2, rows, V.sdig, p2, st))) return rc;
+    if ((rc = launch_msm_key(true, K.rx, *c2, K.table_g2, K.init_g2, rows, V.sdig, p2, st, K.merge))) return rc;
     ZKP_TRACED("k_sum_t<G2Msm>", st, g16_launch_sum(true, R2, s2, st));
     HIP_TRY(hipStreamWaitEvent(st, ev_c, 0));
     HIP_TRY(hipStreamWaitEvent(st, ev_cp, 0));
diff --git a/libzkp_amd/csrc/g16_kernels.hip b/libzkp_amd/csrc/g16_kernels.hip
--- a/libzkp_amd/csrc/g16_kernels.hip
+++ b/libzkp_amd/csrc/g16_kernels.hip
@@ -8,9 +8,11 @@
     static __device__ __forceinline__ Acc identity() { return jac_infinity<fq>(); }
     static constexpr uint32_t GATHER_WAVES = 3; static constexpr int GATHER_PREFETCH = 2;
     static constexpr uint32_t GATHER_W = 16, GATHER_STRIDE = 16, GATHER_PRIO = 0;
-    using GAcc = g1_xyzz9;
+    using GAcc = g1_xyzz9; using GCoord = fq9;
     static __device__ __forceinline__ GAcc to_gather(const g1_jac& a) { return xyzz9_from_jac(a); }
     static __device__ __forceinline__ g1_jac from_gather(const GAcc& a) { return jac_from_xyzz9(a); }
+    static constexpr uint32_t GATHER_MERGE = 4;
+    template <class Src> static __device__ __forceinline__ GAcc gather_add_from(const GAcc& a, Src&& b) { return g1_add9_from(a, b); }
     static __device__ __forceinline__ GAcc accumulate_entry(const GAcc& acc, int32_t d, const uint32_t* e) {
         g1_aff9 q{fq9_unpack8(e), fq9_unpack8(e + 8)};
         q.y = fq9_select(d < 0, fq9_neg_k<4>(q.y), q.y);
@@ -27,9 +29,11 @@
     static __device__ __forceinline__ Acc identity() { return jac_infinity<fq2>(); }
     static constexpr uint32_t GATHER_WAVES = 2; static constexpr int GATHER_PREFETCH = -1;
     static constexpr uint32_t GATHER_W = 32, GATHER_STRIDE = 32, GATHER_PRIO = 0;
-    using GAcc = g2_xyzz9;
+    using GAcc = g2_xyzz9; using GCoord = fq9;
     static __device__ __forceinline__ GAcc to_gather(const g2_jac& a) { return g2_xyzz9_from_jac(a); }
     static __device__ __forceinline__ g2_jac from_gather(const GAcc& a) { return jac_from_g2_xyzz9(a); }
+    static constexpr uint32_t GATHER_MERGE = 4;
+    template <class Src> static __device__ __forceinline__ GAcc gather_add_from(const GAcc& a, Src&& b) { return g2_add9_from(a, b); }
     static __device__ __forceinline__ GAcc accumulate_entry(const GAcc& acc, int32_t d, const uint32_t* e) {
         const g2_aff9 q{fq2_9{fq9_unpack8(e), fq9_unpack8(e + 8)}, fq2_9{fq9_unpack8(e + 16), fq9_unpack8(e + 24)}};
         return g2_mmadd9(acc, q, d < 0);
@@ -138,8 +142,11 @@
 template __global__ void k_msm_gather<G1Msm>(MsmView, uint32_t, uint32_t);
 template __global__ void k_msm_gather<G2Msm>(MsmView, uint32_t, uint32_t);
 static constexpr uint32_t G16_SUM_ROWS = 8, G16_SUM_TB = 256;
+static constexpr uint32_t G16_SUM_ROWS_FEW = 32;
 template __global__ void k_sum_t<G1Msm, G16_SUM_ROWS, G16_SUM_TB>(ReduceView, uint32_t*);
 template __global__ void k_sum_t<G2Msm, G16_SUM_ROWS, G16_SUM_TB>(ReduceView, uint32_t*);
+template __global__ void k_sum_t<G1Msm, G16_SUM_ROWS_FEW, G16_SUM_TB>(ReduceView, uint32_t*);
+template __global__ void k_sum_t<G2Msm, G16_SUM_ROWS_FEW, G16_SUM_TB>(ReduceView, uint32_t*);
 template __global__ void k_g16_build_table<fq, 20>(const uint32_t*, uint32_t, uint32_t*, uint32_t, G16Radix);
 template __global__ void k_g16_build_table<fq2, 40>(const uint32_t*, uint32_t, uint32_t*, uint32_t, G16Radix);
 
@@ -166,10 +173,11 @@
     else k_g16_build_table<fq2, 40><<<(threads + TW - 1) / TW, TW, 0, st>>>(bases, nslots, table, msm_form ? 1u : 0u, rx);
 }
 uint32_t g16_table_entry_words(bool g2, bool msm_form) { return msm_form ? (g2 ? G2Msm::GATHER_W : G1Msm::GATHER_W) : (g2 ? 40u : 20u); }
-uint32_t g16_msm_rows_per_block(bool) { return 256u; }
+uint32_t g16_msm_rows_per_block(bool, uint32_t merge) { return merge ? 64u : 256u; }
 uint32_t g16_msm_blocks_per_cu(bool g2) { return g2 ? G2Msm::GATHER_WAVES : G1Msm::GATHER_WAVES; }
 void g16_launch_msm(bool g2, const MsmView& m, hipStream_t st) {
-    const uint32_t ngroups = (m.rows + 255u) / 256u, nblocks = m.nchunks * ngroups, grid = ((nblocks + 7) / 8) * 8;
+    const uint32_t tb = g16_msm_rows_per_block(g2, m.merge), ngroups = (m.rows + tb - 1) / tb;
+    const uint32_t nblocks = (m.merge ? m.nchunks / m.merge : m.nchunks) * ngroups, grid = ((nblocks + 7) / 8) * 8;
     if constexpr (gather_lds_bytes<G2Msm>() > 0 || gather_lds_bytes<G1Msm>() > 0) {
         if (gather_lds_bytes<G1Msm>()) (void)hipFuncSetAttribute(reinterpret_cast<const void*>(k_msm_gather<G1Msm>), hipFuncAttributeMaxDynamicSharedMemorySize, (int)gather_lds_bytes<G1Msm>());
         if (gather_lds_bytes<G2Msm>()) (void)hipFuncSetAttribute(reinterpret_cast<const void*>(k_msm_gather<G2Msm>), hipFuncAttributeMaxDynamicSharedMemorySize, (int)gather_lds_bytes<G2Msm>());
@@ -178,6 +186,12 @@
     else k_msm_gather<G2Msm><<<grid, 256, gather_lds_bytes<G2Msm>(), st>>>(m, ngroups, nblocks);
 }
 void g16_launch_sum(bool g2, const ReduceView& R, uint32_t* sums, hipStream_t st) {
+    if (R.few_partials) {
+        const dim3 grid((R.rows + G16_SUM_ROWS_FEW - 1) / G16_SUM_ROWS_FEW, R.ntargets);
+        if (!g2) k_sum_t<G1Msm, G16_SUM_ROWS_FEW, G16_SUM_TB><<<grid, G16_SUM_TB, 0, st>>>(R, sums);
+        else k_sum_t<G2Msm, G16_SUM_ROWS_FEW, G16_SUM_TB><<<grid, G16_SUM_TB, 0, st>>>(R, sums);
+        return;
+    }
     const dim3 grid((R.rows + G16_SUM_ROWS - 1) / G16_SUM_ROWS, R.ntargets);
     if (!g2) k_sum_t<G1Msm, G16_SUM_ROWS, G16_SUM_TB><<<grid, G16_SUM_TB, 0, st>>>(R, sums);
     else k_sum_t<G2Msm, G16_SUM_ROWS, G16_SUM_TB><<<grid, G16_SUM_TB, 0, st>>>(R, sums);
diff --git a/libzkp_amd/csrc/g16_launch.h b/libzkp_amd/csrc/g16_launch.h
--- a/libzkp_amd/csrc/g16_launch.h
+++ b/libzkp_amd/csrc/g16_launch.h
@@ -11,7 +11,7 @@
 void g16_launch_mimc(const uint64_t* values, uint32_t n, const uint32_t* mimc_c, uint8_t* out, hipStream_t st);
 void g16_launch_build_table(bool g2, const uint32_t* bases, uint32_t nslots, uint32_t* table, hipStream_t st, bool msm_form, const zkp::G16Radix& rx);
 uint32_t g16_table_entry_words(bool g2, bool msm_form);
-uint32_t g16_msm_rows_per_block(bool g2);
+uint32_t g16_msm_rows_per_block(bool g2, uint32_t merge = 0);
 uint32_t g16_msm_blocks_per_cu(bool g2);
 void g16_launch_msm(bool g2, const zkp::MsmView& m, hipStream_t st);
 void g16_launch_sum(bool g2, const zkp::ReduceView& R, uint32_t* sums, hipStream_t st);
diff --git a/libzkp_amd/csrc/g16_share.h b/libzkp_amd/csrc/g16_share.h
--- a/libzkp_amd/csrc/g16_share.h
+++ b/libzkp_amd/csrc/g16_share.h
@@ -86,12 +86,16 @@
     if (part == G16_PART_AB) return g16_ab_targets(all[0], all[1], all[2]);
     return std::vector<SlotList>(all.begin() + 3, all.end());
 }
-struct G16Chunks { MsmLayout L; std::vector<uint16_t> scal; std::vector<uint32_t> offsets; };
-inline G16Chunks g16_plan_chunks(const std::vector<SlotList>& targets, const std::vector<uint16_t>& row, int part, uint32_t chunks) {
-    G16Chunks C; C.L = make_layout_even(targets, chunks);
+constexpr uint32_t G16_MERGE = 4, G16_QUAD_OFFSETS = 10;
+struct G16Chunks { MsmLayout L; std::vector<uint16_t> scal; std::vector<uint32_t> offsets; std::vector<uint16_t> reduce_begin; };
+inline uint32_t g16_offset_points(const G16Chunks& C, uint32_t merge, uint32_t t) { return (merge ? G16_QUAD_OFFSETS : 1u) * C.offsets[t]; }
+inline G16Chunks g16_plan_chunks(const std::vector<SlotList>& targets, const std::vector<uint16_t>& row, int part, uint32_t chunks, uint32_t merge = 0) {
+    G16Chunks C; C.L = make_layout_even(targets, chunks, merge ? merge : 1u);
     for (uint16_t b : C.L.slot_base) C.scal.push_back(row[b]);
-    if (part == G16_PART_AB) { const G16AbRanges ab = g16_ab_ranges(C.L); for (int t = 0; t < 2; t++) C.offsets.push_back((uint32_t)ab.end[t] - ab.begin[t]); }
-    else for (uint32_t t = 0; t < C.L.ntargets(); t++) C.offsets.push_back((uint32_t)C.L.target_chunk_begin[t + 1] - C.L.target_chunk_begin[t]);
+    MsmLayout R; for (uint16_t b : C.L.target_chunk_begin) R.target_chunk_begin.push_back((uint16_t)(merge ? b / merge : b));
+    C.reduce_begin = R.target_chunk_begin;
+    if (part == G16_PART_AB) { const G16AbRanges ab = g16_ab_ranges(R); for (int t = 0; t < 2; t++) C.offsets.push_back((uint32_t)ab.end[t] - ab.begin[t]); }
+    else for (uint32_t t = 0; t < R.ntargets(); t++) C.offsets.push_back((uint32_t)R.target_chunk_begin[t + 1] - R.target_chunk_begin[t]);
     return C;
 }
 
diff --git a/libzkp_amd/csrc/msm_kernel.h b/libzkp_amd/csrc/msm_kernel.h
--- a/libzkp_amd/csrc/msm_kernel.h
+++ b/libzkp_amd/csrc/msm_kernel.h
@@ -8,6 +8,8 @@
 
 
 template <class T> constexpr size_t gather_lds_bytes() { return T::GATHER_PREFETCH < 0 ? (size_t)4 * 2 * (T::GATHER_W / 4) * 64 * 16 : 0; }
+template <class T, class = void> struct gather_merge_of { static constexpr uint32_t value = 0; };
+template <class T> struct gather_merge_of<T, decltype((void)T::GATHER_MERGE)> { static constexpr uint32_t value = T::GATHER_MERGE; };
 template <class T>
 __global__ void __launch_bounds__(256, T::GATHER_WAVES) k_msm_gather(MsmView m, uint32_t ngroups, uint32_t nblocks) {
     constexpr uint32_t V4 = T::GATHER_W / 4;
@@ -16,16 +18,63 @@
     const uint32_t per_xcd = (nblocks + 7) / 8;
     const uint32_t linear = (blockIdx.x & 7u) * per_xcd + (blockIdx.x >> 3);
     if (linear >= nblocks) return;
-    const uint32_t chunk = linear / ngroups, group = linear % ngroups;
-    const uint32_t row = group * 256u + tid;
+    constexpr uint32_t MERGE = gather_merge_of<T>::value;
+    static_assert(MERGE == 0 || MERGE == 4, "a merging workgroup is its four waves");
+    uint32_t chunk = linear / ngroups, row = (linear % ngroups) * 256u + tid;
+    if constexpr (MERGE != 0) {
+        const uint32_t sh = m.merge ? 6u : 8u;
+        chunk = (chunk << (8u - sh)) + (uint32_t)__builtin_amdgcn_readfirstlane((int)(tid >> sh));
+        row = ((linear % ngroups) << sh) + (tid & ((1u << sh) - 1u));
+    }
     const bool active = row < m.rows;
     const uint32_t st0 = m.chunk_step0[chunk], left = m.chunk_step0[chunk + 1] - st0;
     const uint2* const steps = reinterpret_cast<const uint2*>(m.steps) + st0;
-    typename T::GAcc acc = T::to_gather(m.acc_init ? T::load(m.acc_init, 0, 0, 1) : T::identity());
+    uint32_t init_idx = 0;
+    if constexpr (MERGE != 0) init_idx = m.merge ? chunk % MERGE : 0u;
+    typename T::GAcc acc = T::to_gather(m.acc_init ? T::load(m.acc_init, init_idx, 0, 1) : T::identity());
     const uint4* const table4 = reinterpret_cast<const uint4*>(m.table);
     auto digit_word = [&](const uint2 ds) -> uint32_t { return active ? m.digits[(size_t)(ds.y >> 1) * m.rows + row] : 0u; };
     auto entry_of = [&](const uint2 ds, int32_t d) -> const uint4* { return table4 + ((uint64_t)ds.x + (uint32_t)((d < 0 ? -d : d) - 1)) * SV4; };
-    if (left == 0) { if (active) T::store(m.partial, chunk, row, m.rows, T::from_gather(acc)); return; }
+    auto finish = [&]() __attribute__((always_inline)) {
+    if constexpr (MERGE != 0) {
+        if (m.merge) {
+            constexpr uint32_t GW = sizeof(typename T::GAcc) / 4;
+            const uint32_t wave = chunk % MERGE, lane = row & 63u;
+            uint32_t* slots;
+            if constexpr (T::GATHER_PREFETCH < 0) {
+                extern __shared__ uint4 gather_lds[];
+                static_assert(gather_lds_bytes<T>() >= 2 * 64 * GW * 4, "the join fits the staging buffers");
+                slots = reinterpret_cast<uint32_t*>(gather_lds);
+                __syncthreads();
+            } else {
+                __shared__ uint32_t merge_lds[2 * 64 * GW];
+                slots = merge_lds;
+            }
+            auto put = [&](uint32_t slot) { const uint32_t* w = reinterpret_cast<const uint32_t*>(&acc); ZKP_UNROLL for (uint32_t k = 0; k < GW; k++) slots[(slot * GW + k) * 64u + lane] = w[k]; };
+            auto add_slot = [&](uint32_t slot) {
+                return T::gather_add_from(acc, [&](int c) {
+                    typename T::GCoord b; constexpr uint32_t CW = sizeof(b) / 4;
+                    uint32_t* w = reinterpret_cast<uint32_t*>(&b);
+#if defined(__HIP_DEVICE_COMPILE__)
+                    __builtin_amdgcn_sched_barrier(0);
+#endif
+                    ZKP_UNROLL for (uint32_t k = 0; k < CW; k++) w[k] = slots[(slot * GW + (uint32_t)c * CW + k) * 64u + lane];
+                    return b;
+                });
+            };
+            if (wave >= 2) put(wave - 2);
+            _Pragma("unroll 1") for (uint32_t level = 0; level < 2; level++) {
+                __syncthreads();
+                if (wave < 2u >> level) acc = add_slot(level ? 1u : wave);
+                if (level == 0 && wave == 1) put(1);
+            }
+            if (wave != 0) return;
+            chunk /= MERGE;
+        }
+    }
+    if (active) T::store(m.partial, chunk, row, m.rows, T::from_gather(acc));
+    };
+    if (left == 0 && (MERGE == 0 || !m.merge)) { if (active) T::store(m.partial, chunk, row, m.rows, T::from_gather(acc)); return; }
     if constexpr (T::GATHER_PREFETCH < 0) {
 #if defined(__HIP_DEVICE_COMPILE__)
         extern __shared__ uint4 gather_lds[];
@@ -37,9 +86,9 @@
             ZKP_UNROLL for (uint32_t k = 0; k < V4; k++) __builtin_amdgcn_global_load_lds(src + k, wbuf + (buf * V4 + k) * 64u, 16, 0, 0);
         };
         uint32_t cb = 0;
-        int32_t d = T::digit(digit_word(steps[0]), steps[0].y & 1u);
+        int32_t d = left ? T::digit(digit_word(steps[0]), steps[0].y & 1u) : 0;
         uint32_t q0 = left > 1 ? digit_word(steps[1]) : 0u, q1 = left > 2 ? digit_word(steps[2]) : 0u;
-        dma(0, steps[0], d);
+        if (left) dma(0, steps[0], d);
         for (uint32_t i = 0; i < left; i++) {
             int32_t dn = 0;
             asm volatile("s_waitcnt vmcnt(0)" ::: "memory");
@@ -50,11 +99,12 @@
             if (d != 0) acc = T::accumulate_entry(acc, d, reinterpret_cast<const uint32_t*>(e));
             cb ^= 1u; d = dn; q0 = q1; q1 = qn;
         }
-        if (active) T::store(m.partial, chunk, row, m.rows, T::from_gather(acc));
+        finish();
         return;
 #endif
     } else {
         constexpr int LEAD = T::GATHER_PREFETCH;
+        if (MERGE == 0 || left != 0) {
         uint4 e[LEAD + 1][V4]; int32_t dd[LEAD + 1];
         auto fetch = [&](uint4* dst, const uint2 ds, int32_t d) {
             if (d == 0) return;
@@ -77,8 +127,9 @@
             ZKP_UNROLL for (int k = 0; k < LEAD; k++) { ZKP_UNROLL for (uint32_t v = 0; v < V4; v++) e[k][v] = e[k + 1][v]; dd[k] = dd[k + 1]; }
             q0 = q1; q1 = qn;
         }
+        }
     }
-    if (active) T::store(m.partial, chunk, row, m.rows, T::from_gather(acc));
+    finish();
 }
 
 template <class T, uint32_t ROWS, uint32_t NTHREADS, uint32_t MIN_WAVES = 1>
```

After: 343,600. About the same (-0.7%).
